# zsc/ARTalk

Hardware: AMD Instinct MI355X
Metric: motion frames/sec (25 fps clips) at batch=32 per GPU (higher is better)
Workload: dtype f32 (operands split into 2 fp16, 3 fp16 MFMA products per fp32 product, fp32 accumulate)

## Files before the change

### artalk_amd/capi.py

```python
from __future__ import annotations

import ctypes as C
import os

from .config import ARTalkConfig

_HERE = os.path.dirname(os.path.abspath(__file__))
LIB_PATH = os.environ.get("ARTALK_LIB") or os.path.join(_HERE, "libartalk_hip.so")

OK, EINVAL, EKEY, EMISSING, EHIP, ESTATE, ECAPACITY, EBUSY = 0, -1, -2, -3, -4, -5, -6, -7
DTYPE_F32, DTYPE_I64 = 0, 1

SYMBOLS = [
    "artalk_create", "artalk_destroy", "artalk_last_error", "artalk_set_tensor", "artalk_finalize_weights",
    "artalk_reserve", "artalk_workspace_bytes", "artalk_weight_bytes", "artalk_infer", "artalk_get_status", "artalk_poll_status", "artalk_last_ticket", "artalk_get_status_of", "artalk_style_encode", "artalk_stream_begin", "artalk_stream_chunk", "artalk_stream_end", "artalk_savgol", "artalk_flame_create", "artalk_flame_verts", "artalk_flame_destroy", "artalk_flame_last_error",
    "artalk_set_profiling", "artalk_get_profile", "artalk_get_kernel_sums", "artalk_set_graphs", "artalk_graph_count", "artalk_set_cu_mask", "artalk_set_audit", "artalk_get_audit", "artalk_calibrate", "artalk_reset_scales", "artalk_get_scales", "artalk_scale_sites", "artalk_get_site_scales", "artalk_set_site_scales", "artalk_set_tap", "artalk_tap_layout", "artalk_set_precision",
    "artalk_op_gemm", "artalk_op_gemm_ex", "artalk_op_gemm_bf16", "artalk_op_gemm_f16s", "artalk_op_pack_split", "artalk_op_gemm_f16s_packed", "artalk_op_release_scratch", "artalk_op_gemm_p8_plan", "artalk_op_create_masked_stream", "artalk_op_destroy_stream", "artalk_op_mfma_f32_peak", "artalk_op_layernorm", "artalk_op_attention", "artalk_op_w2v_front", "artalk_op_resample_mean", "artalk_op_pool_silu",
    "artalk_op_bsq_history",
    "artalk_sessions_reserve", "artalk_session_open", "artalk_session_step", "artalk_session_close", "artalk_session_count",
    "artalk_session_smooth", "artalk_op_savgol_stream", "artalk_op_session_smooth_check",
    "artalk_op_pack_split_ex", "artalk_op_layernorm_ex", "artalk_op_gemm_f16s_packed_ex", "artalk_op_gemm_f16s_ex", "artalk_op_attention_ex", "artalk_op_w2v_front_ex", "artalk_op_pool_silu_ex", "artalk_op_posconv_p8_ex",
    "artalk_op_bsq_history_ex", "artalk_op_ar_bits_next", "artalk_op_vq_embed", "artalk_op_ar_begin", "artalk_op_dec_input", "artalk_op_dec_finish", "artalk_op_enc_input_zero", "artalk_op_style_input", "artalk_op_add_row", "artalk_op_style_finish", "artalk_op_broadcast16", "artalk_op_session_gather", "artalk_op_session_scatter", "artalk_op_absmax",
    "artalk_op_gemm_rows", "artalk_op_layernorm_rows", "artalk_op_attention_rows", "artalk_op_gemm_rows_layout", "artalk_op_rows_dry_run",
    "artalk_op_w2v_front_rows", "artalk_op_pool_silu_rows", "artalk_op_posconv_rows",
    "artalk_op_attention_plan", "artalk_op_attention_rows_cus",
    "artalk_infer_samples", "artalk_set_tail_skip", "artalk_conv_tail_geometry", "artalk_conv_tail_class",
    "artalk_render_create", "artalk_render_mesh", "artalk_render_set_slab", "artalk_render_destroy", "artalk_render_last_error",
    "artalk_splat_create", "artalk_splat_render", "artalk_splat_set_timing", "artalk_splat_get_timing", "artalk_splat_destroy",
    "artalk_splat_last_error",
]

(ATTN_F32_64, ATTN_F32_32, ATTN_SHORT, ATTN_F16, ATTN_F16_P8, ATTN_F16_WIDE, ATTN_F16_PP, ATTN_F16_WIDE_AR,
 ATTN_F16_WIDE_AR_P8) = range(9)
ATTN_KERNELS = {
    ATTN_F32_64: "attention_kernel<64>", ATTN_F32_32: "attention_kernel<32>", ATTN_SHORT: "attention_short_kernel",
    ATTN_F16: "attention_f16_kernel<1>", ATTN_F16_P8: "attention_f16_kernel<1,1>", ATTN_F16_WIDE: "attention_f16_wide_kernel",
    ATTN_F16_PP: "attention_f16_pp_kernel", ATTN_F16_WIDE_AR: "attention_f16_wide_ar_kernel<1>",
    ATTN_F16_WIDE_AR_P8: "attention_f16_wide_ar_kernel<1,1,7,128>",
}


class ArtalkConfigStruct(C.Structure):
    _fields_ = [
        ("ar_depth", C.c_int32), ("ar_heads", C.c_int32),
        ("vae_depth", C.c_int32), ("vae_heads", C.c_int32), ("vae_hidden", C.c_int32),
        ("code_dim", C.c_int32), ("motion_dim", C.c_int32),
        ("n_levels", C.c_int32), ("patch_nums", C.c_int32 * 8),
        ("w2v_layers", C.c_int32), ("w2v_hidden", C.c_int32), ("w2v_heads", C.c_int32), ("w2v_ffn", C.c_int32),
        ("w2v_n_conv", C.c_int32), ("w2v_conv_kernel", C.c_int32 * 8), ("w2v_conv_stride", C.c_int32 * 8),
        ("w2v_conv_dim", C.c_int32),
        ("w2v_pos_kernel", C.c_int32), ("w2v_pos_groups", C.c_int32),
        ("w2v_ln_eps", C.c_float),
        ("style_dim", C.c_int32), ("style_heads", C.c_int32), ("style_layers", C.c_int32), ("style_ffn", C.c_int32),
        ("style_len", C.c_int32),
    ]


ROWMAP_IDENTITY = (2 ** 31 - 1, 0, 0)


class GemmRowsArgs(C.Structure):
    _fields_ = [
        ("mode", C.c_int32), ("M", C.c_int32), ("N", C.c_int32), ("K", C.c_int32), ("act", C.c_int32),
        ("A", C.c_void_p), ("lda", C.c_int64), ("a_elems", C.c_int64), ("a_exp", C.c_int32),
        ("W", C.c_void_p), ("ldw", C.c_int64), ("w_elems", C.c_int64),
        ("bias", C.c_void_p), ("bias_elems", C.c_int64),
        ("C", C.c_void_p), ("ldc", C.c_int64), ("c_elems", C.c_int64), ("cmap", C.c_int32 * 3),
        ("gate", C.c_void_p), ("ldg", C.c_int64), ("gate_elems", C.c_int64), ("gmap", C.c_int32 * 3),
        ("R", C.c_void_p), ("ldr", C.c_int64), ("r_elems", C.c_int64),
        ("c_p8", C.c_int32), ("c_exp", C.c_int32),
        ("force_cfg", C.c_int32), ("splitk", C.c_int32),
        ("ngrp", C.c_int32), ("grpW", C.c_int64), ("grpB", C.c_int64), ("grpC", C.c_int64),
        ("status_dev", C.c_void_p),
        ("ln_Y", C.c_void_p), ("ln_ldy", C.c_int64), ("ln_y_elems", C.c_int64),
        ("ln_scale", C.c_void_p), ("ln_shift", C.c_void_p), ("ln_ldm", C.c_int64), ("ln_mod_elems", C.c_int64), ("ln_mmap", C.c_int32 * 3),
        ("ln_eps", C.c_float), ("ln_out_p8", C.c_int32), ("ln_p8_exp", C.c_int32),
        ("used_cfg", C.POINTER(C.c_int32)), ("used_splitk", C.POINTER(C.c_int32)), ("fused_ln", C.POINTER(C.c_int32)),
        ("cus", C.c_int32),
    ]

    def __init__(self, **kw):
        super().__init__()
        self.a_exp = self.c_exp = self.ln_p8_exp = 4
        self.force_cfg, self.splitk, self.ln_eps = -1, 1, 1e-6
        for name in ("cmap", "gmap", "ln_mmap"):
            setattr(self, name, (C.c_int32 * 3)(*ROWMAP_IDENTITY))
        for k, v in kw.items():
            setattr(self, k, (C.c_int32 * 3)(*v) if k in ("cmap", "gmap", "ln_mmap") else v)


def config_struct(cfg: ARTalkConfig) -> ArtalkConfigStruct:
    w = cfg.w2v
    if w.get("feat_extract_norm", "layer") != "layer" or not w.get("do_stable_layer_norm", True) or not w.get("conv_bias", True):
        raise ValueError("only the XLS-R style wav2vec2 (layer-norm conv stack, stable layer norm, conv bias) is supported")
    if len(set(w["conv_dim"])) != 1:
        raise ValueError("conv_dim must be uniform")
    s = ArtalkConfigStruct()
    s.ar_depth, s.ar_heads = cfg.ar_depth, cfg.ar_heads
    s.vae_depth, s.vae_heads, s.vae_hidden = cfg.vae_depth, cfg.vae_heads, cfg.vae_hidden
    s.code_dim, s.motion_dim = cfg.code_dim, cfg.motion_dim
    s.n_levels = len(cfg.patch_nums)
    for i, p in enumerate(cfg.patch_nums):
        s.patch_nums[i] = p
    s.w2v_layers, s.w2v_hidden = w["num_hidden_layers"], w["hidden_size"]
    s.w2v_heads, s.w2v_ffn = w["num_attention_heads"], w["intermediate_size"]
    s.w2v_n_conv = len(w["conv_kernel"])
    for i, (k, st) in enumerate(zip(w["conv_kernel"], w["conv_stride"])):
        s.w2v_conv_kernel[i], s.w2v_conv_stride[i] = k, st
    s.w2v_conv_dim = w["conv_dim"][0]
    s.w2v_pos_kernel, s.w2v_pos_groups = w["num_conv_pos_embeddings"], w["num_conv_pos_embedding_groups"]
    s.w2v_ln_eps = w["layer_norm_eps"]
    s.style_dim, s.style_heads, s.style_layers = cfg.style_dim, cfg.style_heads, cfg.style_layers
    s.style_ffn, s.style_len = cfg.style_ffn, cfg.style_len
    return s


_lib = None


def lib() -> C.CDLL:
    global _lib
    if _lib is not None:
        return _lib
    if not os.path.exists(LIB_PATH):
        raise RuntimeError(
            f"{LIB_PATH} is missing: the HIP extension has not been built "
            "(run `python -c 'import __graft_entry__ as g; g.build()'`). There is no CPU fallback.")
    L = C.CDLL(LIB_PATH)
    vp, i32, i64, f32 = C.c_void_p, C.c_int, C.c_int64, C.c_float
    L.artalk_create.argtypes = [i32, C.POINTER(ArtalkConfigStruct), C.POINTER(vp)]
    L.artalk_create.restype = i32
    L.artalk_destroy.argtypes = [vp]
    L.artalk_destroy.restype = None
    L.artalk_last_error.argtypes = [vp]
    L.artalk_last_error.restype = C.c_char_p
    L.artalk_set_tensor.argtypes = [vp, C.c_char_p, vp, i32, i32, C.POINTER(i64)]
    L.artalk_set_tensor.restype = i32
    L.artalk_finalize_weights.argtypes = [vp]
    L.artalk_finalize_weights.restype = i32
    L.artalk_reserve.argtypes = [vp, i32, i32]
    L.artalk_reserve.restype = i32
    L.artalk_workspace_bytes.argtypes = [vp]
    L.artalk_workspace_bytes.restype = i64
    L.artalk_weight_bytes.argtypes = [vp]
    L.artalk_weight_bytes.restype = i64
    L.artalk_infer.argtypes = [vp, vp, i64, C.POINTER(i64), i32, vp, vp, vp, i64, vp, vp, vp, vp]
    L.artalk_infer.restype = i32
    if hasattr(L, "artalk_infer_samples"):
        L.artalk_infer_samples.argtypes = [vp, vp, i64, C.POINTER(i64), C.POINTER(i64), i32, vp, vp, vp, i64, vp, vp, vp, vp]
        L.artalk_infer_samples.restype = i32
        L.artalk_set_tail_skip.argtypes = [vp, i32]
        L.artalk_set_tail_skip.restype = i32
        pi = C.POINTER(i32)
        L.artalk_conv_tail_geometry.argtypes = [i64, i32, i32, pi, pi, pi, pi, pi, pi]
        L.artalk_conv_tail_geometry.restype = i32
        L.artalk_conv_tail_class.argtypes = [i64, i32]
        L.artalk_conv_tail_class.restype = i64
    L.artalk_get_status.argtypes = [vp, C.POINTER(C.c_int), vp]
    L.artalk_get_status.restype = i32
    L.artalk_poll_status.argtypes = [vp, C.POINTER(C.c_int)]
    L.artalk_poll_status.restype = i32
    L.artalk_last_ticket.argtypes = [vp]
    L.artalk_last_ticket.restype = C.c_longlong
    L.artalk_get_status_of.argtypes = [vp, C.c_longlong, C.POINTER(C.c_int)]
    L.artalk_get_status_of.restype = i32
    L.artalk_style_encode.argtypes = [vp, vp, i32, vp, vp]
    L.artalk_style_encode.restype = i32
    L.artalk_stream_begin.argtypes = [vp, i32, vp, vp, vp]
    L.artalk_stream_begin.restype = i32
    L.artalk_stream_end.argtypes = [vp]
    L.artalk_stream_end.restype = i32
    L.artalk_stream_chunk.argtypes = [vp, vp, i64, vp, i64, vp]
    L.artalk_stream_chunk.restype = i32
    if hasattr(L, "artalk_session_open"):
        L.artalk_sessions_reserve.argtypes = [vp, i32]
        L.artalk_sessions_reserve.restype = i32
        L.artalk_session_open.argtypes = [vp, i32, vp, vp, C.POINTER(i64), vp]
        L.artalk_session_open.restype = i32
        L.artalk_session_step.argtypes = [vp, C.POINTER(i64), i32, vp, i64, vp, i64, vp, vp, vp]
        L.artalk_session_step.restype = i32
        L.artalk_session_close.argtypes = [vp, C.POINTER(i64), i32]
        L.artalk_session_close.restype = i32
        L.artalk_session_count.argtypes = [vp]
        L.artalk_session_count.restype = i32
    if hasattr(L, "artalk_session_smooth"):
        pi32, pu8 = C.POINTER(i32), C.POINTER(C.c_uint8)
        L.artalk_session_smooth.argtypes = [vp, C.POINTER(i64), i32, vp, i64, pi32, pu8, vp, i64, pi32, pi32, vp]
        L.artalk_session_smooth.restype = i32
        L.artalk_op_savgol_stream.argtypes = [vp, vp, i64, pi32, pi32, pu8, vp, i64, i32, vp]
        L.artalk_op_savgol_stream.restype = i32
        L.artalk_op_session_smooth_check.argtypes = [C.POINTER(i64), C.POINTER(i64), pu8, i32, C.POINTER(i64), i32, C.POINTER(i64), i32, i32, i64,
                                                     pi32, pu8, i64, pi32, pi32, C.c_char_p, i32]
        L.artalk_op_session_smooth_check.restype = i32
    L.artalk_flame_create.argtypes = [i32, i32, i32, i32, vp, vp, vp, vp, vp, vp, f32, C.POINTER(vp)]
    L.artalk_flame_create.restype = i32
    L.artalk_flame_verts.argtypes = [vp, vp, vp, i32, vp, vp]
    L.artalk_flame_verts.restype = i32
    L.artalk_flame_destroy.argtypes = [vp]
    L.artalk_flame_destroy.restype = None
    L.artalk_flame_last_error.argtypes = [vp]
    L.artalk_flame_last_error.restype = C.c_char_p
    if hasattr(L, "artalk_render_create"):
        L.artalk_render_create.argtypes = [i32, i32, i32, vp, i32, f32, C.POINTER(vp)]
        L.artalk_render_create.restype = i32
        L.artalk_render_mesh.argtypes = [vp, vp, i32, vp, f32, vp, vp, vp, vp]
        L.artalk_render_mesh.restype = i32
        L.artalk_render_set_slab.argtypes = [vp, i32]
        L.artalk_render_set_slab.restype = i32
        L.artalk_render_destroy.argtypes = [vp]
        L.artalk_render_destroy.restype = None
        L.artalk_render_last_error.argtypes = [vp]
        L.artalk_render_last_error.restype = C.c_char_p
    if hasattr(L, "artalk_splat_create"):
        L.artalk_splat_create.argtypes = [i32, C.POINTER(vp)]
        L.artalk_splat_create.restype = i32
        L.artalk_splat_render.argtypes = [vp, i32, i32, i32, i32, vp, i64, vp, i64, vp, i64, vp, i64, vp, i64, vp, vp, i32, f32, f32, f32,
                                          vp, vp, vp, vp]
        L.artalk_splat_render.restype = i32
        L.artalk_splat_set_timing.argtypes = [vp, i32]
        L.artalk_splat_set_timing.restype = i32
        L.artalk_splat_get_timing.argtypes = [vp, C.POINTER(C.c_double), i32, C.POINTER(C.c_longlong), C.POINTER(i32)]
        L.artalk_splat_get_timing.restype = i32
        L.artalk_splat_destroy.argtypes = [vp]
        L.artalk_splat_destroy.restype = None
        L.artalk_splat_last_error.argtypes = [vp]
        L.artalk_splat_last_error.restype = C.c_char_p
    L.artalk_savgol.argtypes = [vp, vp, vp, i32, vp]
    L.artalk_savgol.restype = i32
    L.artalk_set_profiling.argtypes = [vp, i32]
    L.artalk_set_profiling.restype = i32
    L.artalk_get_profile.argtypes = [vp, C.POINTER(C.c_double), i32]
    L.artalk_get_profile.restype = i32
    if hasattr(L, "artalk_get_kernel_sums"):
        L.artalk_get_kernel_sums.argtypes = [vp, C.POINTER(C.c_double), i32]
        L.artalk_get_kernel_sums.restype = i32
    L.artalk_set_graphs.argtypes = [vp, i32]
    L.artalk_set_graphs.restype = i32
    if hasattr(L, "artalk_graph_count"):
        L.artalk_graph_count.argtypes = [vp, C.POINTER(C.c_longlong)]
        L.artalk_graph_count.restype = i32
    if hasattr(L, "artalk_set_audit"):
        L.artalk_set_audit.argtypes = [vp, i32]
        L.artalk_set_audit.restype = i32
        L.artalk_get_audit.argtypes = [vp, C.c_char_p, i32, C.POINTER(C.c_float), i32]
        L.artalk_get_audit.restype = i32
    if hasattr(L, "artalk_calibrate"):
        L.artalk_calibrate.argtypes = [vp, f32]
        L.artalk_calibrate.restype = i32
        L.artalk_reset_scales.argtypes = [vp]
        L.artalk_reset_scales.restype = i32
        L.artalk_get_scales.argtypes = [vp, C.POINTER(C.c_int), i32]
        L.artalk_get_scales.restype = i32
    if hasattr(L, "artalk_set_site_scales"):
        L.artalk_scale_sites.argtypes = [vp, C.c_char_p, i32]
        L.artalk_scale_sites.restype = i32
        L.artalk_get_site_scales.argtypes = [vp, C.POINTER(C.c_int), i32]
        L.artalk_get_site_scales.restype = i32
        L.artalk_set_site_scales.argtypes = [vp, C.POINTER(C.c_int), i32]
        L.artalk_set_site_scales.restype = i32
    L.artalk_op_gemm.argtypes = [vp, i64, vp, vp, vp, vp, vp, i32, i32, i32, i32, vp]
    L.artalk_op_gemm.restype = i32
    L.artalk_set_precision.argtypes = [vp, i32]
    L.artalk_set_precision.restype = i32
    if hasattr(L, "artalk_op_gemm_bf16"):
        L.artalk_op_gemm_bf16.argtypes = [vp, i64, vp, vp, vp, vp, vp, i32, i32, i32, i32, i32, vp]
        L.artalk_op_gemm_bf16.restype = i32
    L.artalk_op_gemm_f16s.argtypes = [vp, i64, vp, vp, vp, i32, i32, i32, i32, i32, vp]
    L.artalk_op_gemm_f16s.restype = i32
    L.artalk_op_pack_split.argtypes = [vp, vp, i64, i32, vp]
    L.artalk_op_pack_split.restype = i32
    L.artalk_op_gemm_f16s_packed.argtypes = [vp, i32, i64, vp, vp, vp, i32, i32, i32, i32, i32, vp]
    L.artalk_op_gemm_f16s_packed.restype = i32
    if hasattr(L, "artalk_set_tap"):
        L.artalk_set_tap.argtypes = [vp, vp, i32, i32]
        L.artalk_set_tap.restype = i32
        L.artalk_tap_layout.argtypes = [C.POINTER(C.c_int64), i32]
        L.artalk_tap_layout.restype = i32
        L.artalk_op_release_scratch.argtypes = []
        L.artalk_op_release_scratch.restype = i32
    L.artalk_set_cu_mask.argtypes = [vp, vp, i32]
    L.artalk_set_cu_mask.restype = i32
    L.artalk_op_create_masked_stream.argtypes = [vp, i32, C.POINTER(vp)]
    L.artalk_op_create_masked_stream.restype = i32
    L.artalk_op_destroy_stream.argtypes = [vp]
    L.artalk_op_destroy_stream.restype = i32
    L.artalk_op_gemm_p8_plan.argtypes = [i32, i32, i32, i32]
    L.artalk_op_gemm_p8_plan.restype = i32
    L.artalk_op_gemm_ex.argtypes = [vp, i64, vp, vp, vp, i32, i32, i32, i32, i32, vp]
    L.artalk_op_gemm_ex.restype = i32
    L.artalk_op_mfma_f32_peak.argtypes = [vp, i32, i32, i32, C.POINTER(C.c_double), vp]
    L.artalk_op_mfma_f32_peak.restype = i32
    L.artalk_op_layernorm.argtypes = [vp, vp, vp, vp, vp, vp, i32, i32, f32, i32, vp]
    L.artalk_op_layernorm.restype = i32
    L.artalk_op_attention.argtypes = [vp, vp, vp, vp, i32, i32, i32, i32, i32, f32, i32, vp, i32, vp]
    L.artalk_op_attention.restype = i32
    L.artalk_op_w2v_front.argtypes = [vp, i32, i32, vp, vp, vp, vp, vp, vp, vp]
    L.artalk_op_w2v_front.restype = i32
    L.artalk_op_resample_mean.argtypes = [vp, i32, i32, vp, i32, i32, i32, vp, i32, vp]
    L.artalk_op_resample_mean.restype = i32
    L.artalk_op_pool_silu.argtypes = [vp, i32, i32, i32, vp, vp]
    L.artalk_op_pool_silu.restype = i32
    L.artalk_op_bsq_history.argtypes = [vp, vp, vp, vp, i32, vp]
    L.artalk_op_bsq_history.restype = i32
    if hasattr(L, "artalk_op_pack_split_ex"):
        L.artalk_op_pack_split_ex.argtypes = [vp, vp, i64, i32, i32, vp, vp]
        L.artalk_op_pack_split_ex.restype = i32
        L.artalk_op_layernorm_ex.argtypes = [vp, vp, vp, vp, vp, vp, i32, i32, f32, i32, i32, i32, i32, vp, vp]
        L.artalk_op_layernorm_ex.restype = i32
        L.artalk_op_gemm_f16s_packed_ex.argtypes = [vp, i32, i64, vp, vp, vp, i32, i32, i32, i32, i32, i32, i32, vp, vp, vp]
        L.artalk_op_gemm_f16s_packed_ex.restype = i32
# ... 85 lines not shown
```

### artalk_amd/csrc/ar_glue.hip

```cpp
#include "common.h"
#include <cmath>
#include <mutex>
#include <set>

namespace artalk {

constexpr int T100 = 100;
constexpr int CD = 32;
constexpr int NLV = 5;
__constant__ int c_pn[NLV];
__constant__ int c_off[NLV + 1];
__constant__ int c_up_i0[4][T100];
__constant__ int c_up_i1[4][T100];
__constant__ float c_up_w1[4][T100];
__constant__ float c_hq;

static const int h_pn[NLV] = {1, 5, 25, 50, 100};

int init_ms_tables() {
    static std::mutex mu;
    static std::set<int> ready;
    int dev = -1;
    if (hipGetDevice(&dev) != hipSuccess) return -1;
    std::lock_guard<std::mutex> lock(mu);
// ... 79 lines not shown
}
void launch_ar_begin(const float* style_cond, const float* lvlpos, float* x0, float* fhat, int B, hipStream_t s) {
    ARTALK_LAUNCH(ar_begin_kernel, dim3(B), dim3(256), 0, s, style_cond, lvlpos, x0, fhat, 768);
}

constexpr int BITS_NT = 1024;
__global__ __launch_bounds__(BITS_NT) void ar_bits_kernel(const float* __restrict__ logits, uint8_t* __restrict__ bits,
                                                      float* __restrict__ fhat, float* __restrict__ nextfeat, int p, int* __restrict__ status) {
    __shared__ float hs[T100 * CD];
    __shared__ float fs[T100 * CD];
    const int b = blockIdx.x, tid = threadIdx.x;
    const int pn = c_pn[p], off = c_off[p];
    for (int idx = tid; idx < pn * CD; idx += BITS_NT) {
        const int i = idx / CD, c = idx % CD;
        const float* l = logits + ((long)b * pn + i) * (2 * CD) + 2 * c;
        const int bit = l[1] > l[0];
        if (status && !(isfinite(l[0]) && isfinite(l[1]))) atomicOr(status, 1);
        bits[((long)b * 181 + off + i) * CD + c] = (uint8_t)bit;
        hs[idx] = bit ? c_hq : -c_hq;
    }
    if (p >= NLV - 1) return;
    __syncthreads();
    float* fg = fhat + (long)b * T100 * CD;
    for (int idx = tid; idx < T100 * CD; idx += BITS_NT) {
        const int t = idx / CD, c = idx % CD;
        const float v = fg[idx] + up_lin(hs, p, t, c);
        fg[idx] = v;
        fs[idx] = v;
    }
    __syncthreads();
    const int pn2 = c_pn[p + 1];
    for (int idx = tid; idx < pn2 * CD; idx += BITS_NT)
        nextfeat[(long)b * pn2 * CD + idx] = area_pool(fs, pn2, idx / CD, idx % CD);
}
void launch_ar_bits_next(const float* logits, uint8_t* bits, float* fhat, float* nextfeat, int B, int level, hipStream_t s, int* status) {
    ARTALK_LAUNCH(ar_bits_kernel, dim3(B), dim3(BITS_NT), 0, s, logits, bits, fhat, nextfeat, level, status);
}

constexpr int VQ_TOK = 16;
__global__ __launch_bounds__(256) void vq_embed_kernel(const float* __restrict__ feat, int n, const float* __restrict__ We,
                                                       const float* __restrict__ be, const float* __restrict__ pos,
                                                       float* __restrict__ X, int xrows, int xoff,
                                                       const float* __restrict__ style_cond, const float* __restrict__ pos0, int E) {
    __shared__ float f[VQ_TOK][CD];
    const int i0 = blockIdx.x * VQ_TOK, b = blockIdx.y, tid = threadIdx.x;
    if (blockIdx.x == 0 && style_cond) {
        for (int e = tid; e < E; e += 256) X[((long)b * xrows) * E + e] = style_cond[(long)b * E + e] + pos0[e];
    }
    const int nt = min(VQ_TOK, n - i0);
    for (int idx = tid; idx < VQ_TOK * CD; idx += 256) f[idx / CD][idx % CD] = idx < nt * CD ? feat[((long)b * n + i0) * CD + idx] : 0.f;
    constexpr int EPT = 3;
    float w[EPT][CD], bias[EPT], pv[EPT][VQ_TOK];
#pragma unroll
    for (int k = 0; k < EPT; ++k) {
        const int e = tid + k * 256;
        const bool ok = e < E;
#pragma unroll
        for (int c4 = 0; c4 < CD / 4; ++c4) {
            f32x4 t = {0.f, 0.f, 0.f, 0.f};
            if (ok) t = *reinterpret_cast<const f32x4*>(We + (long)e * CD + 4 * c4);
            w[k][4 * c4] = t[0]; w[k][4 * c4 + 1] = t[1]; w[k][4 * c4 + 2] = t[2]; w[k][4 * c4 + 3] = t[3];
        }
        bias[k] = ok ? be[e] : 0.f;
#pragma unroll
        for (int t = 0; t < VQ_TOK; ++t) pv[k][t] = (ok && t < nt) ? pos[(long)(i0 + t) * E + e] : 0.f;
    }
    __syncthreads();
#pragma unroll
    for (int k = 0; k < EPT; ++k) {
        const int e = tid + k * 256;
        if (e >= E) break;
#pragma unroll
        for (int t0 = 0; t0 < VQ_TOK; t0 += 4) {
            float acc[4] = {0.f, 0.f, 0.f, 0.f};
#pragma unroll
            for (int c = 0; c < CD; ++c)
#pragma unroll
                for (int u = 0; u < 4; ++u) acc[u] = fmaf(w[k][c], f[t0 + u][c], acc[u]);
#pragma unroll
            for (int u = 0; u < 4; ++u)
                if (t0 + u < nt) X[((long)b * xrows + xoff + i0 + t0 + u) * E + e] = (acc[u] + bias[k]) + pv[k][t0 + u];
        }
    }
}
void launch_vq_embed(const float* feat, int n, const float* We, const float* be, const float* pos, float* X, int xrows,
                     int xoff, const float* style_cond, const float* pos0, int B, hipStream_t s) {
    ARTALK_LAUNCH(vq_embed_kernel, dim3((n + VQ_TOK - 1) / VQ_TOK, B), dim3(256), 0, s, feat, n, We, be, pos, X, xrows, xoff,
                       style_cond, pos0, 768);
}

__global__ __launch_bounds__(256) void dec_input_kernel(const float* __restrict__ prev_fdec, const float* __restrict__ fhat,
                                                        const uint8_t* __restrict__ bits, const float* __restrict__ dpos,
                                                        float* __restrict__ X) {
    const int b = blockIdx.x;
    for (int idx = blockIdx.y * 256 + threadIdx.x; idx < 2 * T100 * CD; idx += gridDim.y * 256) {
        const int t = idx / CD, c = idx % CD;
        float v;
        if (t < T100) {
            v = prev_fdec[(long)b * T100 * CD + idx];
        } else {
            const int tt = t - T100;
            const float h = bits[((long)b * 181 + 81 + tt) * CD + c] ? c_hq : -c_hq;
            v = fhat[(long)b * T100 * CD + tt * CD + c] + h;
        }
        X[(long)b * 2 * T100 * CD + idx] = v + dpos[idx];
    }
}
void launch_dec_input(const float* prev_fdec, const float* fhat, const uint8_t* bits, const float* dpos, float* X, int B,
                      hipStream_t s) {
    ARTALK_LAUNCH(dec_input_kernel, dim3(B, 8), dim3(256), 0, s, prev_fdec, fhat, bits, dpos, X);
}

__global__ __launch_bounds__(256) void dec_finish_kernel(const float* __restrict__ dec, const float* __restrict__ mean,
                                                         const float* __restrict__ stdv, const float* __restrict__ epos,
                                                         float* __restrict__ out, long out_bstride, int chunk,
                                                         float* __restrict__ E, int MD, int EK, int* __restrict__ status) {
    const int b = blockIdx.x;
    for (int idx = blockIdx.y * 256 + threadIdx.x; idx < T100 * EK; idx += gridDim.y * 256) {
        const int t = idx / EK, j = idx % EK;
        float e = 0.f;
        if (j < MD) {
            const float d = dec[((long)b * 2 * T100 + T100 + t) * MD + j];
            const float m = d * stdv[j] + mean[j];
            if (status && !isfinite(m)) atomicOr(status, 4);
            out[(long)b * out_bstride + ((long)chunk * T100 + t) * MD + j] = m;
            e = (m - mean[j]) / stdv[j] + epos[t * MD + j];
        }
        E[((long)b * T100 + t) * EK + j] = e;
    }
}
void launch_dec_finish(const float* dec, const float* mean, const float* stdv, const float* epos, float* out,
                       long out_bstride, int chunk, float* E, int B, hipStream_t s, int* status) {
    ARTALK_LAUNCH(dec_finish_kernel, dim3(B, 10), dim3(256), 0, s, dec, mean, stdv, epos, out, out_bstride, chunk, E, 106, 128, status);
}

__global__ __launch_bounds__(256) void enc_input_zero_kernel(const float* __restrict__ mean, const float* __restrict__ stdv,
                                                             const float* __restrict__ epos, float* __restrict__ E, int MD, int EK) {
    const int b = blockIdx.x;
    for (int idx = threadIdx.x; idx < T100 * EK; idx += 256) {
        const int t = idx / EK, j = idx % EK;
        E[((long)b * T100 + t) * EK + j] = (j < MD) ? ((0.f - mean[j]) / stdv[j] + epos[t * MD + j]) : 0.f;
    }
}
__global__ __launch_bounds__(256) void broadcast16_kernel(const uint4* __restrict__ src, uint4* __restrict__ dst, int n16) {
    uint4* d = dst + (long)blockIdx.y * n16;
    for (int i = blockIdx.x * 256 + threadIdx.x; i < n16; i += gridDim.x * 256) d[i] = src[i];
}
void launch_broadcast16(const void* src, void* dst, long bytes, int B, hipStream_t s) {
    if (B <= 0 || bytes <= 0) return;
    const int n16 = (int)(bytes / 16);
    ARTALK_LAUNCH(broadcast16_kernel, dim3((n16 + 255) / 256 < 8 ? (n16 + 255) / 256 : 8, B), dim3(256), 0, s,
                       reinterpret_cast<const uint4*>(src), reinterpret_cast<uint4*>(dst), n16);
}

void launch_enc_input_zero(const float* mean, const float* stdv, const float* epos, float* E, int B, hipStream_t s) {
    ARTALK_LAUNCH(enc_input_zero_kernel, dim3(B), dim3(256), 0, s, mean, stdv, epos, E, 106, 128);
}

__global__ __launch_bounds__(256) void session_gather_kernel(const uint4* const* __restrict__ slots, SessionRows w) {
    const uint4* __restrict__ src = slots[blockIdx.y];
    const long row = blockIdx.y;
    const int p0 = w.s16, f0 = w.s16 + w.p16, n16 = f0 + w.f16;
    for (int i = blockIdx.x * 256 + threadIdx.x; i < n16; i += gridDim.x * 256) {
        const uint4 v = src[i];
        if (i < p0) w.style[row * w.s16 + i] = v;
        else if (i < f0) w.prev_in[row * w.p16 + (i - p0)] = v;
        else w.prev_fdec[row * w.f16 + (i - f0)] = v;
    }
}
__global__ __launch_bounds__(256) void session_scatter_kernel(uint4* const* __restrict__ slots, SessionRows w, int with_style) {
    uint4* __restrict__ dst = slots[blockIdx.y];
    const long row = blockIdx.y;
    const int p0 = w.s16, f0 = w.s16 + w.p16, n16 = f0 + w.f16;
    for (int i = (with_style ? 0 : p0) + blockIdx.x * 256 + threadIdx.x; i < n16; i += gridDim.x * 256) {
        uint4 v;
        if (i < p0) v = w.style[row * w.s16 + i];
        else if (i < f0) v = w.prev_in[row * w.p16 + (i - p0)];
        else v = w.prev_fdec[row * w.f16 + (i - f0)];
        dst[i] = v;
    }
}
static inline unsigned session_pieces(const SessionRows& w) { return (unsigned)((w.s16 + w.p16 + w.f16 + 1023) / 1024); }
void launch_session_gather(const float* const* slots, const SessionRows& w, int n, hipStream_t s) {
    if (n <= 0) return;
    ARTALK_LAUNCH(session_gather_kernel, dim3(session_pieces(w), n), dim3(256), 0, s, reinterpret_cast<const uint4* const*>(slots), w);
}
void launch_session_scatter(float* const* slots, const SessionRows& w, int n, bool with_style, hipStream_t s) {
    if (n <= 0) return;
    ARTALK_LAUNCH(session_scatter_kernel, dim3(session_pieces(w), n), dim3(256), 0, s, reinterpret_cast<uint4* const*>(slots), w,
                  with_style ? 1 : 0);
}

constexpr int BSQ_NT = 1024;
__global__ __launch_bounds__(BSQ_NT) void bsq_history_kernel(const float* __restrict__ enc_out, uint8_t* __restrict__ hist_bits,
                                                          float* __restrict__ prev_fdec, float* __restrict__ msfeat, int* __restrict__ status) {
    __shared__ float resid[T100 * CD];
    __shared__ float fms[T100 * CD];
    __shared__ float qs[T100 * CD];
    __shared__ float hs[T100 * CD];
    const int b = blockIdx.x, tid = threadIdx.x;
    for (int idx = tid; idx < T100 * CD; idx += BSQ_NT) {
        resid[idx] = enc_out[(long)b * T100 * CD + idx];
        if (status && !isfinite(resid[idx])) atomicOr(status, 2);
        fms[idx] = 0.f;
    }
    __syncthreads();
    int msoff = 0;
    for (int p = 0; p < NLV; ++p) {
        const int pn = c_pn[p], off = c_off[p];
        for (int base = 0; base < pn * CD; base += BSQ_NT) {
            const int idx = base + tid;
            const bool ok = idx < pn * CD;
            const int i = ok ? idx / CD : 0, c = idx % CD;
            float x = 0.f;
            if (ok) x = (pn == T100) ? resid[idx] : area_pool(resid, pn, i, c);
            float ss = x * x;
            ss = group_sum<32>(ss);
            const float z = x / fmaxf(sqrtf(ss), 1e-12f);
            const float zhat = (z > 0.f) ? c_hq : -c_hq;
            const float q = z + (zhat - z);
            const int bit = q > 0.f;
            if (ok) {
                qs[idx] = q;
                hs[idx] = bit ? c_hq : -c_hq;
                hist_bits[((long)b * 181 + off + i) * CD + c] = (uint8_t)bit;
            }
        }
        __syncthreads();
        if (p < NLV - 1) {
            for (int idx = tid; idx < T100 * CD; idx += BSQ_NT) {
                const int t = idx / CD, c = idx % CD;
                resid[idx] -= up_lin(qs, p, t, c);
                fms[idx] += up_lin(hs, p, t, c);
            }
            __syncthreads();
            const int pn2 = c_pn[p + 1];
            for (int idx = tid; idx < pn2 * CD; idx += BSQ_NT)
                msfeat[((long)b * 180 + msoff) * CD + idx] = area_pool(fms, pn2, idx / CD, idx % CD);
            msoff += pn2;
        } else {
            for (int idx = tid; idx < T100 * CD; idx += BSQ_NT) prev_fdec[(long)b * T100 * CD + idx] = fms[idx] + hs[idx];
        }
        __syncthreads();
    }
}
void launch_bsq_history(const float* enc_out, uint8_t* hist_bits, float* prev_fdec, float* msfeat, int B, hipStream_t s, int* status) {
    ARTALK_LAUNCH(bsq_history_kernel, dim3(B), dim3(BSQ_NT), 0, s, enc_out, hist_bits, prev_fdec, msfeat, status);
}

__global__ __launch_bounds__(256) void style_input_kernel(const float* __restrict__ motion, const float* __restrict__ mean,
                                                          const float* __restrict__ stdv, float* __restrict__ X, int rows, int MD, int EK) {
    const long n = (long)rows * EK;
    for (long idx = (long)blockIdx.x * 256 + threadIdx.x; idx < n; idx += (long)gridDim.x * 256) {
        const long row = idx / EK; const int j = idx % EK;
        X[idx] = (j < MD) ? (motion[row * MD + j] - mean[j]) / stdv[j] : 0.f;
    }
}
void launch_style_input(const float* motion, const float* mean, const float* stdv, float* X, int B, hipStream_t s) {
    const int rows = B * 50;
    ARTALK_LAUNCH(style_input_kernel, dim3((rows * 128 + 255) / 256), dim3(256), 0, s, motion, mean, stdv, X, rows, 106, 128);
}

__global__ __launch_bounds__(256) void add_row_kernel(float* __restrict__ X, const float* __restrict__ v, long n, int D) {
    for (long idx = (long)blockIdx.x * 256 + threadIdx.x; idx < n; idx += (long)gridDim.x * 256) X[idx] += v[idx % D];
}
void launch_add_row(float* X, const float* v, int M, int D, hipStream_t s) {
    const long n = (long)M * D;
    ARTALK_LAUNCH(add_row_kernel, dim3((unsigned)((n + 255) / 256)), dim3(256), 0, s, X, v, n, D);
}

__global__ __launch_bounds__(256) void style_finish_kernel(const float* __restrict__ feat, const float* __restrict__ Ws,
                                                           const float* __restrict__ bs, const float* __restrict__ null_cond,
                                                           const uint8_t* __restrict__ has_style, float* __restrict__ style_cond,
                                                           int L, int S, int E, const float* __restrict__ cached, long cached_stride) {
    __shared__ float m[128];
    const int b = blockIdx.x, tid = threadIdx.x;
    const int has = has_style ? has_style[b] : 0;
    if (has != 1 && has != 2) {
        for (int e = tid; e < E; e += 256) style_cond[(long)b * E + e] = null_cond[e];
        return;
    }
    if (has == 2) {
        for (int e = tid; e < E; e += 256) style_cond[(long)b * E + e] = cached[(long)b * cached_stride + e];
        return;
    }
    if (tid < S) {
        float s = 0.f;
        for (int t = 0; t < L; ++t) s += feat[((long)b * L + t) * S + tid];
        m[tid] = s / (float)L;
    }
    __syncthreads();
    for (int e = tid; e < E; e += 256) {
        const float* w = Ws + (long)e * S;
        float acc = 0.f;
        for (int c = 0; c < S; ++c) acc = fmaf(w[c], m[c], acc);
        style_cond[(long)b * E + e] = (acc + bs[e]) * 1.1f - null_cond[e] * 0.1f;
    }
}
void launch_style_finish(const float* feat, const float* Ws, const float* bs, const float* null_cond,
                         const uint8_t* has_style, float* style_cond, int B, hipStream_t s, const float* cached, long cached_stride) {
    ARTALK_LAUNCH(style_finish_kernel, dim3(B), dim3(256), 0, s, feat, Ws, bs, null_cond, has_style, style_cond, 50, 128, 768,
                       cached, cached_stride);
}

struct SavgolCoef {
    double fir5[5], edge5[2][5];
// ... 104 lines not shown
```

### artalk_amd/csrc/calls.hip

```cpp
#include "model.h"

#include <algorithm>
#include <climits>
#include <cstring>
#include <set>
#include <string>
#include <vector>

using namespace artalk;

namespace {
int call_stream(artalk_model* m, void* stream, hipStream_t* s) {
    (void)hipSetDevice(m->device);
    if (!stream && !m->own_stream) HIPCHK(m, hipStreamCreate(&m->own_stream));
    *s = stream ? (hipStream_t)stream : m->own_stream;
    return ARTALK_OK;
}
int check_has_style(artalk_model* m, const float* style_motion_dev, const uint8_t* has_style, int B, bool* encode) {
    *encode = false;
    for (int b = 0; style_motion_dev && has_style && b < B; ++b) {
        if (has_style[b] > 2) return fail(m, ARTALK_EINVAL, "has_style entries must be 0, 1 or 2");
        *encode |= has_style[b] == 1;
    }
    return ARTALK_OK;
// ... 37 lines not shown
            *err = std::string(fn) + ": " + std::to_string(ids[i]) + " is not an open session";
            return ARTALK_EINVAL;
        }
        if (!listed.insert(ids[i]).second) { *err = std::string(fn) + ": session " + std::to_string(ids[i]) + " is listed twice"; return ARTALK_EINVAL; }
        (*st)[i] = &it->second;
    }
    return ARTALK_OK;
}

}

namespace artalk {
void smooth_span(int64_t seen, int nf, bool last, int* first, int* count) {
    const int64_t f = seen > kSavgolLag ? seen - kSavgolLag : 0;
    *first = (int)f;
    *count = (int)((last ? seen + nf : seen + nf - kSavgolLag) - f);
}
int smooth_row_range(const std::string& who, int nf, bool last, std::string* err) {
    if (nf < 0 || nf > 100) { *err = who + ": n_frames " + std::to_string(nf) + " is outside 0..100"; return ARTALK_EINVAL; }
    if (nf < 100 && !last) { *err = who + ": fewer than 100 frames (" + std::to_string(nf) + ") without `last`"; return ARTALK_EINVAL; }
    return ARTALK_OK;
}
int smooth_row_length(const std::string& who, int64_t seen, int nf, bool last, std::string* err) {
    if (seen < 0 || seen > INT_MAX - 2 * kSavgolMaxOut) { *err = who + ": frame count out of range"; return ARTALK_EINVAL; }
    if (last && seen + nf < kSavgolCarry) { *err = who + ": savgol (mode='interp') needs window_length <= T (T >= 9)"; return ARTALK_EINVAL; }
    return ARTALK_OK;
}
int smooth_stride_check(const char* fn, bool have_raw, bool need_raw, int64_t raw_stride, int64_t out_stride, int D, std::string* err) {
    if (need_raw && !have_raw) { *err = std::string(fn) + ": no raw frames given"; return ARTALK_EINVAL; }
    if (need_raw && raw_stride < 100LL * D) { *err = std::string(fn) + ": raw_stride is below 100 x " + std::to_string(D); return ARTALK_EINVAL; }
    if (out_stride < (int64_t)kSavgolMaxOut * D) { *err = std::string(fn) + ": out_stride is below 104 x " + std::to_string(D); return ARTALK_EINVAL; }
    return ARTALK_OK;
}
int smooth_check(artalk_model::Sessions& ss, const int64_t* ids, int n, bool have_raw, int64_t raw_stride, const int* n_frames,
                 const uint8_t* last, int64_t out_stride, int D, std::vector<artalk_model::Sessions::Open*>* st, std::string* err) {
    if (int rc = resolve_sessions(ss, "artalk_session_smooth", ids, n, st, err)) return rc;
    bool need_raw = false;
    for (int i = 0; i < n; ++i) {
        const int nf = n_frames ? n_frames[i] : 100;
        const bool lst = last && last[i];
        const std::string who = "artalk_session_smooth: session " + std::to_string(ids[i]);
        if (int rc = smooth_row_range(who, nf, lst, err)) return rc;
        if ((*st)[i]->smooth_done) { *err = who + " has been smoothed to its end (a `last` call was made)"; return ARTALK_ESTATE; }
        if (int rc = smooth_row_length(who, (*st)[i]->seen, nf, lst, err)) return rc;
        need_raw |= nf > 0;
    }
    return smooth_stride_check("artalk_session_smooth", have_raw, need_raw, raw_stride, out_stride, D, err);
}
}

namespace {
int stage_session_slots(artalk_model* m, hipStream_t s, artalk_model::Stage* stg, const int* slot, int n) {
    for (int i = 0; i < n; ++i) stg->slots[i] = m->sess_slot(slot[i]);
    HIPCHK(m, hipMemcpyAsync(m->ws.sess_slots, stg->slots, (size_t)n * sizeof(float*), hipMemcpyHostToDevice, s));
    return ARTALK_OK;
}

}

extern "C" {

int artalk_infer(artalk_model* m, const float* audio_dev, int64_t audio_clip_stride, const int64_t* n_chunks, int B,
                 const float* style_motion_dev, const uint8_t* has_style, float* out_motion_dev, int64_t out_clip_stride,
                 uint8_t* out_bits_dev, uint8_t* out_hist_bits_dev, float* out_w2v_dev, void* stream) {
    return artalk_infer_samples(m, audio_dev, audio_clip_stride, n_chunks, nullptr, B, style_motion_dev, has_style, out_motion_dev, out_clip_stride,
                                out_bits_dev, out_hist_bits_dev, out_w2v_dev, stream);
}

int artalk_infer_samples(artalk_model* m, const float* audio_dev, int64_t audio_clip_stride, const int64_t* n_chunks, const int64_t* n_samples,
                         int B, const float* style_motion_dev, const uint8_t* has_style, float* out_motion_dev, int64_t out_clip_stride,
                         uint8_t* out_bits_dev, uint8_t* out_hist_bits_dev, float* out_w2v_dev, void* stream) {
    if (!m || !audio_dev || !n_chunks || !out_motion_dev || B <= 0) return ARTALK_EINVAL;
    if (!m->finalized) return fail(m, ARTALK_ESTATE, "artalk_infer before artalk_finalize_weights");
    for (int b = 0; n_samples && b < B; ++b)
        if (n_chunks[b] > 0 && (n_samples[b] < 1 || n_samples[b] > n_chunks[b] * kSamplesPerChunk))
            return fail(m, ARTALK_EINVAL, "n_samples[" + std::to_string(b) + "] must be in 1 .. n_chunks * " + std::to_string(kSamplesPerChunk));
    hipStream_t s;
    if (int rc = call_stream(m, stream, &s)) return rc;
    const artalk_config& c = m->cfg;
    int64_t C = 0, maxch = n_chunks[0];
    for (int b = 0; b < B; ++b) {
        if (n_chunks[b] <= 0 || (b > 0 && n_chunks[b] > n_chunks[b - 1])) return fail(m, ARTALK_EINVAL, "n_chunks must be positive and non-increasing");
        C += n_chunks[b];
    }
    bool encode_style;
    if (int rc = check_has_style(m, style_motion_dev, has_style, B, &encode_style)) return rc;
    if (m->tap && (B > m->tap_B || maxch > m->tap_maxch)) return fail(m, ARTALK_EINVAL, "the tap buffer (artalk_set_tap) is smaller than this call");
    if (B > m->ws.maxB || C > m->ws.maxC) { if (int rc = reserve(m, B, (int)C)) return rc; }
    Workspace& w = m->ws;
    artalk_model::Stage* stg = nullptr;
    if (int rc = next_stage(m, &stg)) return rc;
    long* src = stg->src;
    std::vector<int> base((size_t)maxch + 1, 0), Bj((size_t)maxch, 0);
    {
        int idx = 0;
        for (int64_t j = 0; j < maxch; ++j) {
            base[j] = idx;
            for (int b = 0; b < B && n_chunks[b] > j; ++b) { src[idx++] = (long)b * audio_clip_stride + (long)j * kSamplesPerChunk; Bj[j]++; }
        }
        base[maxch] = idx;
    }
    std::vector<ConvPasses> passes;
    bool any_tail = false;
    if (n_samples && m->tail_skip) {
        std::vector<int> cls((size_t)C, 3);
        for (int64_t j = 0, idx = 0; j < maxch; ++j)
            for (int b = 0; b < B && n_chunks[b] > j; ++b, ++idx) {
                const int64_t v = std::min<int64_t>(n_samples[b] - j * kSamplesPerChunk, kSamplesPerChunk);
                const int64_t bound = v >= 1 ? artalk_conv_tail_class(v, kSamplesPerChunk) : 0;
                const int q = bound >= 1 && kSamplesPerChunk % 4 == 0 ? (int)(bound / (kSamplesPerChunk / 4)) : 4;
                cls[idx] = m->tail_geo[q - 1].partial ? q - 1 : 3;
            }
        const int last = m->n_conv - 1;
        for (int c0 = 0; c0 < C; c0 += w.G) {
            const int n = (int)std::min<int64_t>(w.G, C - c0);
            ConvPasses cp;
            static const int order[4] = {3, 0, 1, 2};
            int pos = 0;
            long row0 = 0;
            for (int k = 0; k < 4; ++k) {
                const int cl = order[k], off = pos;
                const artalk_model::TailGeo& tg = m->tail_geo[cl];
                const long rows = cl == 3 ? m->Ts : tg.S[last], tc = cl == 3 ? m->Tw - 1 : tg.tc;
                for (int i = 0; i < n; ++i)
                    if (cls[c0 + i] == cl) {
                        src[C + c0 + pos] = src[c0 + i];
                        src[2 * C + c0 + i] = (row0 + (pos - off) * rows) | (tc << 32);
                        ++pos;
                    }
                if (pos > off) { cp.off[cp.np] = off; cp.n[cp.np] = pos - off; cp.cls[cp.np] = cl; ++cp.np; row0 += (pos - off) * rows; }
            }
            if (cp.np == 1 && cp.cls[0] == 3) cp.np = 0;
            else { cp.perm = w.src_off + C + c0; cp.tab = w.src_off + 2 * C + c0; any_tail = true; }
            passes.push_back(cp);
        }
    }
    HIPCHK(m, hipMemcpyAsync(w.src_off, src, (any_tail ? 3 : 1) * C * sizeof(long), hipMemcpyHostToDevice, s));
    m->stream_B = 0; m->stream_scales_ended = false;
    m->ev_used = 0; m->dom_events.clear(); m->marks.clear(); m->prof_stream = s;
    struct TimerScope { bool on; TimerScope(artalk_model* x) : on(x->profiling == 3) { if (on) { x->ktimer.used = 0; x->ktimer.recs.clear(); x->ktimer.bucket = KB_OTHER; g_ktimer = &x->ktimer; } }
                        ~TimerScope() { if (on) g_ktimer = nullptr; } } timer_scope(m);
    if (int rc = begin_clips(m, s, B, style_motion_dev, has_style, encode_style, stg)) return rc;
    for (int c0 = 0, gi = 0; c0 < C; c0 += w.G, ++gi)
        run_wav2vec(m, audio_dev, c0, (int)std::min<int64_t>(w.G, C - c0), out_w2v_dev, s, !passes.empty() && passes[gi].np ? &passes[gi] : nullptr);
    if (int rc = run_init_history(m, B, s)) return rc;
    const size_t bits_row = (size_t)kNTok * c.code_dim;
    if (out_hist_bits_dev)
        HIPCHK(m, hipMemcpy2DAsync(out_hist_bits_dev, (size_t)(maxch + 1) * bits_row, w.hist_bits, bits_row, bits_row, B,
                                   hipMemcpyDeviceToDevice, s));
    stage_mark(m, s, PB_VAE);
    for (int64_t j = 0; j < maxch; ++j) {
        const int Bn = Bj[j];
        const int n_next = out_hist_bits_dev ? Bn : (j + 1 < maxch ? Bj[j + 1] : 0);
        if (int rc = chunk_step(m, s, base[j], Bn, n_next, (int)j, out_motion_dev + j * 100 * c.motion_dim, out_clip_stride)) return rc;
        if (out_bits_dev)
            HIPCHK(m, hipMemcpy2DAsync(out_bits_dev + j * bits_row, (size_t)maxch * bits_row, w.bits, bits_row, bits_row, Bn,
                                       hipMemcpyDeviceToDevice, s));
        if (out_hist_bits_dev)
            HIPCHK(m, hipMemcpy2DAsync(out_hist_bits_dev + (j + 1) * bits_row, (size_t)(maxch + 1) * bits_row, w.hist_bits, bits_row,
                                       bits_row, Bn, hipMemcpyDeviceToDevice, s));
    }
    stage_mark(m, s, PB_OTHER);
    if (int rc = publish_status(m, s)) return rc;
    if (m->sticky_error) { m->sticky_error = false; return ARTALK_ESTATE; }
    return ARTALK_OK;
}

int artalk_style_encode(artalk_model* m, const float* style_motion_dev, int n, float* out_cond_dev, void* stream) {
    if (!m || !style_motion_dev || !out_cond_dev || n <= 0) return ARTALK_EINVAL;
    if (!m->finalized) return fail(m, ARTALK_ESTATE, "artalk_style_encode before artalk_finalize_weights");
    hipStream_t s;
    if (int rc = call_stream(m, stream, &s)) return rc;
    if (m->stream_B > 0) return fail(m, ARTALK_ESTATE, "artalk_style_encode during a streaming session (it shares the workspace)");
    if (n > m->ws.maxB) { if (int rc = reserve(m, n, std::max(n, m->ws.maxC))) return rc; }
    Workspace& w = m->ws;
    HIPCHK(m, hipMemsetAsync(w.has_style, 1, n, s));
    {
        ProfilingOff quiet(m);
        run_style(m, style_motion_dev, n, s, true);
    }
    HIPCHK(m, hipMemcpyAsync(out_cond_dev, w.style_cond, (size_t)n * kE * sizeof(float), hipMemcpyDeviceToDevice, s));
    HIPCHK(m, hipGetLastError());
    return ARTALK_OK;
}

int artalk_stream_begin(artalk_model* m, int B, const float* style_motion_dev, const uint8_t* has_style, void* stream) {
    if (!m || B <= 0) return ARTALK_EINVAL;
    if (!m->finalized) return fail(m, ARTALK_ESTATE, "artalk_stream_begin before artalk_finalize_weights");
    bool encode_style;
    if (int rc = check_has_style(m, style_motion_dev, has_style, B, &encode_style)) return rc;
    hipStream_t s;
    if (int rc = call_stream(m, stream, &s)) return rc;
    if (B > m->ws.maxB || B > m->ws.maxC) { if (int rc = reserve(m, B, B)) return rc; }
    if (int rc = ensure_stage(m, m->ws.maxB, m->ws.maxC)) return rc;
    artalk_model::Stage* stg = nullptr;
    if (int rc = next_stage(m, &stg)) return rc;
    {
        ProfilingOff quiet(m);
        if (int rc = begin_clips(m, s, B, style_motion_dev, has_style, encode_style, stg)) return rc;
        if (int rc = run_init_history(m, B, s)) return rc;
    }
    m->stream_B = B; m->stream_scales_ended = false;
    if (int rc = publish_status(m, s)) return rc;
    return ARTALK_OK;
}

int artalk_stream_chunk(artalk_model* m, const float* audio_dev, int64_t chunk_stride, float* out_motion_dev, int64_t out_stride,
                        void* stream) {
    if (!m || !audio_dev || !out_motion_dev) return ARTALK_EINVAL;
    if (m->stream_B <= 0)
        return fail(m, ARTALK_ESTATE, m->stream_scales_ended ? "the site scales changed since artalk_stream_begin; begin again"
                                                             : "artalk_stream_chunk before artalk_stream_begin");
    hipStream_t s;
    if (int rc = call_stream(m, stream, &s)) return rc;
    const int B = m->stream_B;
    Workspace& w = m->ws;
    if (B > w.maxB) return fail(m, ARTALK_ESTATE, "workspace was re-reserved since artalk_stream_begin; begin again");
    artalk_model::Stage* stg = nullptr;
    if (int rc = next_stage(m, &stg)) return rc;
    for (int b = 0; b < B; ++b) stg->src[b] = (long)b * chunk_stride;
    HIPCHK(m, hipMemcpyAsync(w.src_off, stg->src, B * sizeof(long), hipMemcpyHostToDevice, s));
    HIPCHK(m, hipEventRecord(stg->done, s));
    stg->used = true;
    ProfilingOff quiet(m);
    for (int c0 = 0; c0 < B; c0 += w.G) run_wav2vec(m, audio_dev, c0, std::min(w.G, B - c0), nullptr, s);
    if (int rc = chunk_step(m, s, 0, B, B, m->tap_maxch, out_motion_dev, out_stride)) return rc;
    if (int rc = publish_status(m, s)) return rc;
    return ARTALK_OK;
}

int artalk_stream_end(artalk_model* m) {
    if (!m) return ARTALK_EINVAL;
    m->stream_B = 0; m->stream_scales_ended = false;
    return ARTALK_OK;
}

int artalk_sessions_reserve(artalk_model* m, int max_sessions) {
    if (!m || max_sessions <= 0) return ARTALK_EINVAL;
    (void)hipSetDevice(m->device);
    return grow_sessions(m, max_sessions);
}

int artalk_session_count(const artalk_model* m) { return m ? (int)m->sess.open.size() : ARTALK_EINVAL; }

int artalk_session_open(artalk_model* m, int n, const float* style_motion_dev, const uint8_t* has_style, int64_t* ids_out, void* stream) {
    if (!m || n <= 0 || !ids_out) return ARTALK_EINVAL;
    if (!m->finalized) return fail(m, ARTALK_ESTATE, "artalk_session_open before artalk_finalize_weights");
    bool encode_style;
    if (int rc = check_has_style(m, style_motion_dev, has_style, n, &encode_style)) return rc;
    hipStream_t s;
    if (int rc = call_stream(m, stream, &s)) return rc;
    artalk_model::Sessions& ss = m->sess;
    if (int rc = grow_sessions(m, (int64_t)ss.open.size() + n)) return rc;
    if (n > m->ws.maxB || n > m->ws.maxC) { if (int rc = reserve(m, n, n)) return rc; }
    if (int rc = ensure_stage(m, m->ws.maxB, m->ws.maxC)) return rc;
    std::vector<int> slot;
    for (int i = 0; i < (int)ss.owner.size() && (int)slot.size() < n; ++i)
        if (!ss.owner[i]) slot.push_back(i);
    artalk_model::Stage* stg = nullptr;
    if (int rc = next_stage(m, &stg)) return rc;
    if (int rc = stage_session_slots(m, s, stg, slot.data(), n)) return rc;
    m->stream_B = 0; m->stream_scales_ended = false;
    {
        ProfilingOff quiet(m);
        if (int rc = begin_clips(m, s, n, style_motion_dev, has_style, encode_style, stg)) return rc;
        if (int rc = run_init_history(m, n, s)) return rc;
    }
    launch_session_scatter(m->ws.sess_slots, session_rows(m), n, true, s);
    if (int rc = publish_status(m, s)) return rc;
    for (int i = 0; i < n; ++i) {
        ids_out[i] = ss.next_id++;
        ss.owner[slot[i]] = ids_out[i];
        ss.open.emplace(ids_out[i], artalk_model::Sessions::Open{slot[i]});
    }
    return ARTALK_OK;
}

int artalk_session_step(artalk_model* m, const int64_t* ids, int n, const float* audio_dev, int64_t chunk_stride, float* out_motion_dev,
                        int64_t out_stride, uint8_t* out_bits_dev, uint8_t* out_hist_bits_dev, void* stream) {
    if (!m || !ids || n <= 0 || !audio_dev || !out_motion_dev) return ARTALK_EINVAL;
    artalk_model::Sessions& ss = m->sess;
    std::vector<artalk_model::Sessions::Open*> st;
    std::string err;
    if (int rc = resolve_sessions(ss, "artalk_session_step", ids, n, &st, &err)) return fail(m, rc, err);
    std::vector<int> slot((size_t)n);
    for (int i = 0; i < n; ++i) slot[i] = st[i]->slot;
    hipStream_t s;
    if (int rc = call_stream(m, stream, &s)) return rc;
    if (n > m->ws.maxB || n > m->ws.maxC) { if (int rc = reserve(m, n, n)) return rc; }
    Workspace& w = m->ws;
    artalk_model::Stage* stg = nullptr;
    if (int rc = next_stage(m, &stg)) return rc;
    for (int b = 0; b < n; ++b) stg->src[b] = (long)b * chunk_stride;
    HIPCHK(m, hipMemcpyAsync(w.src_off, stg->src, n * sizeof(long), hipMemcpyHostToDevice, s));
    if (int rc = stage_session_slots(m, s, stg, slot.data(), n)) return rc;
    HIPCHK(m, hipEventRecord(stg->done, s));
    stg->used = true;
    m->stream_B = 0; m->stream_scales_ended = false;
    HIPCHK(m, hipMemsetAsync(w.status, 0, 4 * sizeof(int), s));
    const SessionRows rows = session_rows(m);
    ProfilingOff quiet(m);
    launch_session_gather(w.sess_slots, rows, n, s);
    for (int c0 = 0; c0 < n; c0 += w.G) run_wav2vec(m, audio_dev, c0, std::min(w.G, n - c0), nullptr, s);
    if (int rc = chunk_step(m, s, 0, n, n, m->tap_maxch, out_motion_dev, out_stride)) return rc;
    launch_session_scatter(w.sess_slots, rows, n, false, s);
    const size_t bits_n = (size_t)n * kNTok * m->cfg.code_dim;
    if (out_bits_dev) HIPCHK(m, hipMemcpyAsync(out_bits_dev, w.bits, bits_n, hipMemcpyDeviceToDevice, s));
    if (out_hist_bits_dev) HIPCHK(m, hipMemcpyAsync(out_hist_bits_dev, w.hist_bits, bits_n, hipMemcpyDeviceToDevice, s));
    if (int rc = publish_status(m, s)) return rc;
    return ARTALK_OK;
}

int artalk_session_close(artalk_model* m, const int64_t* ids, int n) {
    if (!m || !ids || n <= 0) return ARTALK_EINVAL;
    artalk_model::Sessions& ss = m->sess;
    std::set<int64_t> seen;
    for (int i = 0; i < n; ++i)
        if ((!ss.open.count(ids[i]) && !ss.ended_by_scales.count(ids[i])) || !seen.insert(ids[i]).second)
            return fail(m, ARTALK_EINVAL, "artalk_session_close: " + std::to_string(ids[i]) + " is not an open session (or is listed twice)");
    for (int i = 0; i < n; ++i) {
        const auto it = ss.open.find(ids[i]);
        if (it != ss.open.end()) { ss.owner[it->second.slot] = 0; ss.open.erase(it); }
        ss.ended_by_scales.erase(ids[i]);
    }
    return ARTALK_OK;
}

int artalk_session_smooth(artalk_model* m, const int64_t* ids, int n, const float* raw_dev, int64_t raw_stride, const int* n_frames,
                          const uint8_t* last, float* out_dev, int64_t out_stride, int* first_out, int* count_out, void* stream) {
    if (!m || !ids || n <= 0 || !out_dev || !first_out || !count_out) return ARTALK_EINVAL;
    artalk_model::Sessions& ss = m->sess;
    std::vector<artalk_model::Sessions::Open*> st;
    std::string err;
    if (int rc = smooth_check(ss, ids, n, raw_dev != nullptr, raw_stride, n_frames, last, out_stride, m->cfg.motion_dim, &st, &err)) return fail(m, rc, err);
    hipStream_t s;
    if (int rc = call_stream(m, stream, &s)) return rc;
    if (n > m->stage_cap_b) { if (int rc = ensure_stage(m, n, m->stage_cap_c)) return rc; }
    artalk_model::Stage* stg = nullptr;
    if (int rc = next_stage(m, &stg)) return rc;
    for (int i = 0; i < n; ++i) {
        stg->slots[i] = m->sess_slot(st[i]->slot);
        stg->smooth[i] = make_int4((int)st[i]->seen, n_frames ? n_frames[i] : 100, last && last[i] ? 1 : 0, 0);
    }
    float** slots_dev = static_cast<float**>(ss.smooth_tab);
    int4* meta_dev = reinterpret_cast<int4*>(slots_dev + ss.smooth_cap);
    HIPCHK(m, hipMemcpyAsync(slots_dev, stg->slots, (size_t)n * sizeof(float*), hipMemcpyHostToDevice, s));
    HIPCHK(m, hipMemcpyAsync(meta_dev, stg->smooth, (size_t)n * sizeof(int4), hipMemcpyHostToDevice, s));
    HIPCHK(m, hipEventRecord(stg->done, s));
    stg->used = true;
    launch_savgol_stream(slots_dev, meta_dev, (long)m->sess_carry_off(), raw_dev, (long)raw_stride, out_dev, (long)out_stride, n,
                         m->cfg.motion_dim, s);
    HIPCHK(m, hipGetLastError());
    for (int i = 0; i < n; ++i) {
        const int nf = n_frames ? n_frames[i] : 100;
        const bool lst = last && last[i];
        smooth_span(st[i]->seen, nf, lst, &first_out[i], &count_out[i]);
        st[i]->seen += nf;
        st[i]->smooth_done = lst;
    }
    return ARTALK_OK;
}

int artalk_savgol(artalk_model* m, const float* in_dev, float* out_dev, int T, void* stream) {
    if (!m || !in_dev || !out_dev) return ARTALK_EINVAL;
    if (T < 9) return fail(m, ARTALK_EINVAL, "savgol (mode='interp') needs window_length <= T (T >= 9)");
    (void)hipSetDevice(m->device);
    launch_savgol(in_dev, out_dev, T, m->cfg.motion_dim, (hipStream_t)stream);
    return ARTALK_OK;
}

}
```

### artalk_amd/csrc/engine.hip

```cpp
#include "model.h"

#include <hip/hip_ext.h>

#include <algorithm>
#include <cmath>
#include <cstring>
#include <string>
#include <vector>

using namespace artalk;

namespace artalk {
thread_local KernelTimer* g_ktimer = nullptr;
bool ktimer_events(hipEvent_t* e0, hipEvent_t* e1) {
    KernelTimer* t = g_ktimer;
    if (!t) return false;
    while (t->pool.size() < t->used + 2) {
        hipEvent_t e = nullptr;
        if (hipEventCreate(&e) != hipSuccess) return false;
        t->pool.push_back(e);
    }
    *e0 = t->pool[t->used]; *e1 = t->pool[t->used + 1];
    t->recs.emplace_back(t->bucket, t->used);
    t->used += 2;
    return true;
}
}

namespace {
hipEvent_t next_event(artalk_model* m, hipStream_t s, size_t* idx) {
    if (m->ev_used == m->ev_pool.size()) {
        hipEvent_t e;
        (void)hipEventCreate(&e);
        m->ev_pool.push_back(e);
    }
    *idx = m->ev_used++;
    (void)hipEventRecord(m->ev_pool[*idx], s);
    return m->ev_pool[*idx];
}
void kbucket(artalk_model* m, int b) { m->ktimer.bucket = b; }
}

namespace artalk {
void stage_mark(artalk_model* m, hipStream_t s, int bucket) {
    if (!m->profiling || m->in_graph_body) return;
    size_t i;
    next_event(m, s, &i);
    m->marks.emplace_back(bucket, i);
}
}

namespace {
void audit(artalk_model* m, const float* buf, int rows, int cols, long ld, bool is_p8, hipStream_t s, int* ex, int junk_period = 0,
           int junk_from = 0) {
    if (!m->audit || !m->audit_vals) return;
    auto st = m->site_of.find(ex);
    if (st == m->site_of.end()) { m->err = "internal: audited exponent is not in the site table"; m->sticky_error = true; return; }
    const std::string& name = m->sites[st->second].name;
    auto it = m->audit_index.find(name);
    int idx;
    if (it == m->audit_index.end()) {
        if ((int)m->audit_names.size() >= kAuditSlots) return;
        idx = (int)m->audit_names.size();
        m->audit_names.push_back(name);
        m->audit_exp.push_back(ex);
        m->audit_index.emplace(name, idx);
    } else idx = it->second;
    launch_absmax(buf, rows, cols & ~7, ld, is_p8 ? 1 : 0, m->audit_vals + idx, s, junk_period, junk_from, ex ? *ex : kActExp);
}

bool gemm(artalk_model* m, const GemmArgs& g0, hipStream_t s, const LnArgs* fuse_ln = nullptr, int plan_M = 0) {
    GemmArgs g = g0;
    const int run_M = g.M;
    if (plan_M > 0) g.M = plan_M;
    g.graph_tag = m->in_body ? 1 : 0;
    g.cus = m->n_cus;
    g.status = m->precision == 1 ? (m->view ? m->view->status : m->ws.status) : nullptr;
    if (m->precision == 1 && !g.exact) g.Wp = packed_of(m, g.W);
    if (m->precision == 2 && !g.exact) {
        g.Wb = bf16_of(m, g.W);
        if (!g.Wb || ((unsigned long long)g.Wb & 15) || (g.ldw & 7)) {
            m->err = "internal: bf16 GEMM without an aligned bf16 weight copy"; m->sticky_error = true; return false;
        }
        if (g.a_packed) { m->err = "internal: P8 activation handed to a bf16 GEMM"; m->sticky_error = true; return false; }
    }
    const Workspace& cw = m->view ? *m->view : m->ws;
    const GemmPolicy pol{m->precision, false, cw.splitk, cw.splitk_floats, m->splitk_tiles, m->splitk_target};
    GemmPlan plan = plan_gemm(g, pol, fuse_ln);
    if (plan_M > 0) {
        g.M = run_M;
        if (plan.path != GEMM_P8) g.force_cfg = plan.cfg;
        else if (gemm_p8_class(plan.cfg) == P8_BIG) {
            GemmArgs h = g;
            h.force_cfg = g0.force_cfg; h.splitk = g0.splitk; h.partial = g0.partial;
            const GemmPlan alt = plan_gemm(h, pol, fuse_ln);
            if (alt.path == GEMM_P8 && gemm_p8_class(alt.cfg) == P8_BIG && h.splitk == g.splitk) { g.force_cfg = alt.cfg; plan.cfg = alt.cfg; }
        }
    }
    if (g.a_packed && plan.path == GEMM_F32) { m->err = "internal: P8 activation handed to an fp32 GEMM"; m->sticky_error = true; return false; }
    const bool timed = m->profiling && plan.dominant && !m->in_body;
    size_t i0 = 0, i1 = 0;
    if (timed) next_event(m, s, &i0);
    run_gemm(g, plan, fuse_ln, s);
    if (timed) {
        next_event(m, s, &i1);
        m->dom_events.emplace_back(i0, gemm_flops(g));
    }
    return plan.fused_ln;
}

void tap_copy(artalk_model* m, int field, int row0, const float* src, int rows, int cols, int B, hipStream_t s) {
    if (!m->tap || m->in_graph_body || m->tap_chunk >= m->tap_maxch || B > m->tap_B) return;
    float* dst = m->tap + ((long)m->tap_chunk * m->tap_B) * TAP_SLOT + field + (long)row0 * cols;
    (void)hipMemcpy2DAsync(dst, (size_t)TAP_SLOT * 4, src, (size_t)rows * cols * 4, (size_t)rows * cols * 4, B, hipMemcpyDeviceToDevice, s);
}

enum { LF_EXACT = 1, LF_A_P8 = 2, LF_C_P8 = 4 };
void linear(artalk_model* m, const float* A, long lda, const float* W, const float* bias, float* C, long ldc, int M, int N, int K,
            int act, const float* R, hipStream_t s, int flags = 0, float* c2 = nullptr, int a_exp = kActExp, int c_exp = kActExp,
            int plan_M = 0) {
    GemmArgs g;
    g.c2 = c2; g.a_exp = a_exp; g.c_exp = c_exp;
    g.exact = flags & LF_EXACT; g.a_packed = (flags & LF_A_P8) ? 1 : 0; g.c_p8 = (flags & LF_C_P8) ? 1 : 0;
    g.A = A; g.lda = lda; g.W = W; g.ldw = K; g.bias = bias; g.C = C; g.ldc = ldc; g.M = M; g.N = N; g.K = K; g.act = act;
    g.R = R; g.ldr = ldc;
    gemm(m, g, s, nullptr, plan_M);
}

void layernorm(const float* X, float* Y, const float* w, const float* b, int M, int D, float eps, int act, hipStream_t s, int out_p8 = 0,
               int* status = nullptr, int junk_period = 0, int junk_from = 0, int p8_exp = kActExp) {
    LnArgs a;
    a.out_p8 = out_p8; a.p8_exp = p8_exp; a.status = out_p8 ? status : nullptr; a.junk_period = junk_period; a.junk_from = junk_from;
    a.X = X; a.ldx = D; a.Y = Y; a.ldy = D; a.w = w; a.b = b; a.M = M; a.D = D; a.eps = eps; a.act = act;
    launch_layernorm(a, s);
}

}

namespace artalk {

void run_wav2vec(artalk_model* m, const float* audio, int c0, int n, float* out_w2v, hipStream_t s, const ConvPasses* tail) {
    const artalk_config& c = m->cfg;
    Workspace& w = m->ws;
    const int CD = c.w2v_conv_dim, Hs = c.w2v_hidden;
    const int p8 = m->precision == 1 ? 1 : 0;
    const int AP = p8 ? LF_A_P8 : 0;
    Range r_w2v("artalk.wav2vec2");
    roctxRangePushA("artalk.wav2vec2.conv_stack");
    kbucket(m, KB_CONV);
    launch_audio_normalize(audio, tail ? tail->perm : w.src_off + c0, w.xnorm, n, kSamplesPerChunk, s);
    SiteExps& ex = m->ex;
    ConvPasses one;
    one.np = 1; one.n[0] = n; one.cls[0] = 3;
    const ConvPasses& ps = tail ? *tail : one;
    auto geo_T = [&](int p) { const artalk_model::TailGeo& tg = m->tail_geo[ps.cls[p]]; return ps.cls[p] != 3 && tg.partial ? tg.T : m->conv_T; };
    auto geo_S = [&](int p) { const artalk_model::TailGeo& tg = m->tail_geo[ps.cls[p]]; return ps.cls[p] != 3 && tg.partial ? tg.S : m->conv_S; };
    auto row0 = [&](int p, int i) { long r = 0; for (int q = 0; q < p; ++q) r += (long)ps.n[q] * geo_S(q)[i]; return r; };
    float* src = w.convA; float* dst = w.convB;
    for (int p = 0; p < ps.np; ++p) {
        const int *T = geo_T(p), *S = geo_S(p);
        float* y = src + row0(p, 0) * CD;
        launch_conv0(w.xnorm + (long)ps.off[p] * kSamplesPerChunk, kSamplesPerChunk, m->conv0_w, m->conv_b[0], m->conv_lnw[0], m->conv_lnb[0], y, ps.n[p],
                     T[0], S[0], s, p8, w.status, ex.conv[0]);
        audit(m, y, ps.n[p] * S[0], CD, CD, p8, s, &ex.conv[0], S[0], T[0]);
    }
    for (int i = 1; i < c.w2v_n_conv; ++i) {
        const int M = (int)row0(ps.np, i), plan_M = M == n * m->conv_S[i] ? 0 : n * m->conv_S[i];
        linear(m, src, (long)c.w2v_conv_stride[i] * CD, m->conv_w[i], m->conv_b[i], dst, CD, M, CD, c.w2v_conv_kernel[i] * CD,
               ACT_NONE, nullptr, s, AP, nullptr, ex.conv[i - 1], kActExp, plan_M);
        for (int p = 0; p < ps.np; p += 2) {
            const int *T = geo_T(p), *S = geo_S(p);
            float* y = dst + row0(p, i) * CD;
            const int Mp = ps.n[p] * S[i], Mq = p + 1 < ps.np ? ps.n[p + 1] * geo_S(p + 1)[i] : 0;
            LnArgs a;
            a.plan_M = plan_M;
            a.out_p8 = (p8 && i + 1 < c.w2v_n_conv) ? 1 : 0; a.p8_exp = ex.conv[i]; a.status = a.out_p8 ? w.status : nullptr;
            a.junk_period = S[i]; a.junk_from = T[i];
            if (Mq) { a.junk_row2 = Mp; a.junk_period2 = geo_S(p + 1)[i]; a.junk_from2 = geo_T(p + 1)[i]; }
            a.X = y; a.ldx = CD; a.Y = y; a.ldy = CD; a.w = m->conv_lnw[i]; a.b = m->conv_lnb[i]; a.M = Mp + Mq; a.D = CD; a.eps = 1e-5f; a.act = ACT_GELU_ERF;
            launch_layernorm(a, s);
            if (i + 1 < c.w2v_n_conv) {
                audit(m, y, Mp, CD, CD, p8, s, &ex.conv[i], S[i], T[i]);
                if (Mq) audit(m, y + (long)Mp * CD, Mq, CD, CD, p8, s, &ex.conv[i], a.junk_period2, a.junk_from2);
            }
        }
        std::swap(src, dst);
    }
    if (tail) {
        launch_conv_tail_gather(src, tail->tab, dst, n, m->Tw, m->Ts, CD, s);
        std::swap(src, dst);
    }
    stage_mark(m, s, PB_CONV);
    roctxRangePop();
    Range r_enc("artalk.wav2vec2.encoder");
    kbucket(m, KB_ENC);
    const int M = n * m->Ts;
    const int JP = m->Ts, JF = m->Tw;
    layernorm(src, dst, m->fp_lnw, m->fp_lnb, M, CD, c.w2v_ln_eps, ACT_NONE, s, p8, w.status, JP, JF, ex.fp_ln);
    audit(m, dst, M, CD, CD, p8, s, &ex.fp_ln, JP, JF);
    linear(m, dst, CD, m->fp_w, m->fp_b, w.h0, Hs, M, Hs, CD, ACT_NONE, nullptr, s, AP, nullptr, ex.fp_ln);
    audit(m, w.h0, M, Hs, Hs, false, s, &ex.posconv_in, JP, JF);
    {
        const int cg = Hs / c.w2v_pos_groups;
        GemmArgs g;
        g.A = w.h0; g.lda = Hs; g.W = m->pos_w; g.ldw = (long)cg * c.w2v_pos_kernel; g.bias = m->pos_b; g.C = w.h1; g.ldc = Hs; g.R = w.h0; g.ldr = Hs;
        g.M = M; g.act = ACT_GELU_ERF; g.a_exp = ex.posconv_in;
        if (p8 && cg == 64 && c.w2v_pos_kernel == 128 && c.w2v_pos_groups == 16 && m->Ts <= 256) {
            g.N = Hs; g.K = cg * c.w2v_pos_kernel; g.Wp = packed_of(m, m->pos_w); g.status = w.status;
            launch_posconv_p8(g, n, m->Tw, m->Ts, s);
        } else {
            g.amode = 1; g.pc_T = m->Tw; g.pc_tstride = m->Ts; g.pc_pad = c.w2v_pos_kernel / 2; g.pc_cin = cg;
            g.N = cg; g.K = cg * c.w2v_pos_kernel;
            g.batch = c.w2v_pos_groups; g.sA = cg; g.sW = (long)cg * cg * c.w2v_pos_kernel; g.sBias = cg; g.sC = cg; g.sR = cg;
            gemm(m, g, s);
        }
    }
    float* h = w.h1;
    const int nh = c.w2v_heads, hd = Hs / nh;
    for (int i = 0; i < c.w2v_layers; ++i) {
        const W2VLayer& L = m->w2v[i];
        SiteExps::W2V& E = ex.w2v[i];
        layernorm(h, w.xln, L.ln1w, L.ln1b, M, Hs, c.w2v_ln_eps, ACT_NONE, s, p8, w.status, JP, JF, E.ln1);
        audit(m, w.xln, M, Hs, Hs, p8, s, &E.ln1, JP, JF);
        linear(m, w.xln, Hs, L.qkv_w, L.qkv_b, w.qkv, 3 * Hs, M, 3 * Hs, Hs, ACT_NONE, nullptr, s, AP | (p8 ? LF_C_P8 : 0), nullptr, E.ln1, E.qkv);
        AttnArgs a;
        a.qkv_p8 = p8; a.qkv_exp = E.qkv; a.o_exp = E.attn;
        a.Q = w.qkv; a.K = w.qkv + Hs; a.V = w.qkv + 2 * Hs;
        a.ldq = a.ldk = a.ldv = 3 * Hs; a.q_bstride = a.k_bstride = a.v_bstride = (long)m->Ts * 3 * Hs;
        a.O = w.att; a.ldo = Hs; a.o_bstride = (long)m->Ts * Hs;
        a.B = n; a.H = nh; a.HD = hd; a.Lq = m->Tw; a.Lk = m->Tw; a.scale = 1.0f / std::sqrt((float)hd);
        audit(m, w.qkv, M, 3 * Hs, 3 * Hs, p8, s, &E.qkv, JP, JF);
        a.out_p8 = p8; a.split16 = p8; a.status = p8 ? w.status : nullptr; a.cus = m->n_cus;
        launch_attention(a, s);
        audit(m, w.att, M, Hs, Hs, p8, s, &E.attn, JP, JF);
        linear(m, w.att, Hs, L.out_w, L.out_b, h, Hs, M, Hs, Hs, ACT_NONE, h, s, AP, nullptr, E.attn);
        layernorm(h, w.xln, L.ln2w, L.ln2b, M, Hs, c.w2v_ln_eps, ACT_NONE, s, p8, w.status, JP, JF, E.ln2);
        audit(m, w.xln, M, Hs, Hs, p8, s, &E.ln2, JP, JF);
        linear(m, w.xln, Hs, L.ff1_w, L.ff1_b, w.ffn, c.w2v_ffn, M, c.w2v_ffn, Hs, ACT_GELU_ERF, nullptr, s, AP | (p8 ? LF_C_P8 : 0), nullptr, E.ln2, E.ffn);
        audit(m, w.ffn, M, c.w2v_ffn, c.w2v_ffn, p8, s, &E.ffn, JP, JF);
        linear(m, w.ffn, c.w2v_ffn, L.ff2_w, L.ff2_b, h, Hs, M, Hs, c.w2v_ffn, ACT_NONE, h, s, AP, nullptr, E.ffn);
    }
    layernorm(h, w.xln, m->enc_lnw, m->enc_lnb, M, Hs, c.w2v_ln_eps, ACT_NONE, s);
    if (out_w2v)
        (void)hipMemcpy2DAsync(out_w2v + (long)c0 * m->Tw * Hs, (size_t)m->Tw * Hs * 4, w.xln, (size_t)m->Ts * Hs * 4,
                               (size_t)m->Tw * Hs * 4, n, hipMemcpyDeviceToDevice, s);
    launch_pool_silu(w.xln, m->Ts, m->Tw, w.silu_cond + (long)c0 * kNTok * kCond, n, m->pn, c.n_levels, kCond, s, p8, w.status, ex.silu_cond);
    audit(m, w.silu_cond + (long)c0 * kNTok * kCond, n * kNTok, kCond, kCond, p8, s, &ex.silu_cond);
    stage_mark(m, s, PB_ENC);
}

void run_style(artalk_model* m, const float* style_motion, int B, hipStream_t s, bool encode) {
    const artalk_config& c = m->cfg;
    Workspace& w = m->ws;
    const int S = c.style_dim, L = c.style_len, M = B * L;
    Range r_style("artalk.style_encoder");
    kbucket(m, KB_STYLE);
    if (style_motion && encode) {
        launch_style_input(style_motion, m->st_mean, m->st_std, w.s_in, B, s);
        SiteExps& ex = m->ex;
        audit(m, w.s_in, M, 128, 128, false, s, &ex.style_in);
        linear(m, w.s_in, 128, m->st_proj_w, m->st_proj_b, w.s_h, S, M, S, 128, ACT_NONE, nullptr, s, 0, nullptr, ex.style_in);
        launch_add_row(w.s_h, m->st_pe, M, S, s);
        for (int i = 0; i < c.style_layers; ++i) {
            const StyleLayer& Ly = m->style[i];
            SiteExps::ST& E = ex.style[i];
            audit(m, w.s_h, M, S, S, false, s, &E.h);
            linear(m, w.s_h, S, Ly.in_w, Ly.in_b, w.s_qkv, 3 * S, M, 3 * S, S, ACT_NONE, nullptr, s, 0, nullptr, E.h);
            AttnArgs a;
            a.Q = w.s_qkv; a.K = w.s_qkv + S; a.V = w.s_qkv + 2 * S; a.ldq = a.ldk = a.ldv = 3 * S;
            a.q_bstride = a.k_bstride = a.v_bstride = (long)L * 3 * S;
            a.O = w.s_att; a.ldo = S; a.o_bstride = (long)L * S;
            a.B = B; a.H = c.style_heads; a.HD = S / c.style_heads; a.Lq = L; a.Lk = L;
            a.scale = 1.0f / std::sqrt((float)(S / c.style_heads));
            launch_attention(a, s);
            audit(m, w.s_att, M, S, S, false, s, &E.attn);
            linear(m, w.s_att, S, Ly.out_w, Ly.out_b, w.s_tmp, S, M, S, S, ACT_NONE, w.s_h, s, 0, nullptr, E.attn);
            layernorm(w.s_tmp, w.s_h, Ly.n1w, Ly.n1b, M, S, 1e-5f, ACT_NONE, s);
            audit(m, w.s_h, M, S, S, false, s, &E.h1);
            linear(m, w.s_h, S, Ly.l1_w, Ly.l1_b, w.s_ffn, c.style_ffn, M, c.style_ffn, S, ACT_GELU_ERF, nullptr, s, 0, nullptr, E.h1);
            audit(m, w.s_ffn, M, c.style_ffn, c.style_ffn, false, s, &E.ffn);
            linear(m, w.s_ffn, c.style_ffn, Ly.l2_w, Ly.l2_b, w.s_tmp, S, M, S, c.style_ffn, ACT_NONE, w.s_h, s, 0, nullptr, E.ffn);
            layernorm(w.s_tmp, w.s_h, Ly.n2w, Ly.n2b, M, S, 1e-5f, ACT_NONE, s);
        }
    }
    launch_style_finish(w.s_h, m->sc_w, m->sc_b, m->null_style, style_motion ? w.has_style : nullptr, w.style_cond, B, s,
                        style_motion, (long)L * c.motion_dim);
}

}

namespace {
void run_vae_stack(artalk_model* m, const VAESide& S, int B, int T, int split, hipStream_t s) {
    const artalk_config& c = m->cfg;
    Workspace& w = m->view ? *m->view : m->ws;
    const int H = c.vae_hidden, M = B * T, F = H * 3 / 2;
    const int p8 = m->precision == 1 ? 1 : 0;
    const int AP = p8 ? LF_A_P8 : 0;
    const int sd = &S == &m->enc ? 0 : 1;
    for (int i = 0; i < c.vae_depth; ++i) {
        const VAELayer& L = S.layers[i];
        SiteExps::VAE& E = m->ex.vae[sd][i];
        layernorm(w.vh, w.vln, L.lnw, L.lnb, M, H, 1e-5f, ACT_NONE, s, p8, w.status, 0, 0, E.ln);
        audit(m, w.vln, M, H, H, p8, s, &E.ln);
        linear(m, w.vln, H, L.qkv_w, nullptr, w.vqkv, 3 * H, M, 3 * H, H, ACT_NONE, nullptr, s, AP | (p8 ? LF_C_P8 : 0), nullptr, E.ln, E.qkv);
        AttnArgs a;
        a.qkv_p8 = p8; a.qkv_exp = E.qkv; a.o_exp = E.attn;
        a.Q = w.vqkv; a.K = w.vqkv + H; a.V = w.vqkv + 2 * H; a.ldq = a.ldk = a.ldv = 3 * H;
        a.q_bstride = a.k_bstride = a.v_bstride = (long)T * 3 * H;
        a.O = w.vatt; a.ldo = H; a.o_bstride = (long)T * H;
        a.B = B; a.H = c.vae_heads; a.HD = H / c.vae_heads; a.Lq = T; a.Lk = T;
        a.scale = 1.0f / std::sqrt((float)H);
        audit(m, w.vqkv, M, 3 * H, 3 * H, p8, s, &E.qkv);
        a.split_q = split; a.split_k = split; a.out_p8 = p8; a.split16 = p8; a.status = p8 ? w.status : nullptr; a.cus = m->n_cus;
        launch_attention(a, s);
        audit(m, w.vatt, M, H, H, p8, s, &E.attn);
        linear(m, w.vatt, H, L.out_w, L.out_b, w.vh, H, M, H, H, ACT_NONE, w.vh, s, AP, p8 ? w.vln : nullptr, E.attn, E.resid);
        audit(m, p8 ? w.vln : w.vh, M, H, H, p8, s, &E.resid);
        linear(m, p8 ? w.vln : w.vh, H, L.m1_w, L.m1_b, w.vmlp, F, M, F, H, ACT_GELU_TANH, nullptr, s, p8 ? (LF_A_P8 | LF_C_P8) : 0, nullptr, E.resid, E.mlp);
        audit(m, w.vmlp, M, F, F, p8, s, &E.mlp);
        linear(m, w.vmlp, F, L.m2_w, L.m2_b, w.vh, H, M, H, F, ACT_NONE, w.vh, s, AP, nullptr, E.mlp);
    }
}

void run_reencode(artalk_model* m, int B, hipStream_t s) {
    const artalk_config& c = m->cfg;
    Workspace& w = m->view ? *m->view : m->ws;
    const int H = c.vae_hidden, T = 100;
    Range r_re("artalk.vae.reencode_bsq");
    kbucket(m, KB_REENC);
    audit(m, w.enc_in, B * T, 128, 128, false, s, &m->ex.vae_enc_in);
    linear(m, w.enc_in, 128, m->enc.in_w, m->enc.in_b, w.vh, H, B * T, H, 128, ACT_LEAKY02, nullptr, s, 0, nullptr, m->ex.vae_enc_in);
    run_vae_stack(m, m->enc, B, T, 0, s);
    linear(m, w.vh, H, m->enc.out_w, m->enc.out_b, w.enc_out, c.code_dim, B * T, c.code_dim, H, ACT_NONE, nullptr, s, LF_EXACT);
    launch_bsq_history(w.enc_out, w.hist_bits, w.prev_fdec, w.msfeat, B, s, w.status);
    launch_vq_embed(w.msfeat, kNTok - 1, m->vq_w, m->vq_b, m->prev_lvl_pos + kE, w.prev_in, kNTok, 1, w.style_cond,
                    m->prev_lvl_pos, B, s);
}

}

namespace artalk {
int run_init_history(artalk_model* m, int B, hipStream_t s) {
    const artalk_config& c = m->cfg;
    struct Restore { artalk_model* m; ~Restore() { kbucket(m, KB_OTHER); } } restore{m};
    Workspace& w = m->ws;
    artalk_model::InitHistory& ih = m->init_hist[m->precision];
    const long nb = (long)kNTok * c.code_dim, nf = 100L * c.code_dim * 4, nm = 180L * c.code_dim * 4;
    if (!ih.valid) {
        if (!ih.bits) {
            ih.bits = dalloc<uint8_t>(m, nb); ih.fdec = dalloc<float>(m, nf / 4); ih.msfeat = dalloc<float>(m, nm / 4);
            if (!ih.bits || !ih.fdec || !ih.msfeat) return fail(m, ARTALK_EHIP, "hipMalloc failed for the initial-history cache");
            HIPCHK(m, hipDeviceSynchronize());
        }
        launch_enc_input_zero(m->vae_mean, m->vae_std, m->enc_pos, w.enc_in, 1, s);
        run_reencode(m, 1, s);
        HIPCHK(m, hipMemcpyAsync(ih.bits, w.hist_bits, nb, hipMemcpyDeviceToDevice, s));
        HIPCHK(m, hipMemcpyAsync(ih.fdec, w.prev_fdec, nf, hipMemcpyDeviceToDevice, s));
        HIPCHK(m, hipMemcpyAsync(ih.msfeat, w.msfeat, nm, hipMemcpyDeviceToDevice, s));
        int flags[4] = {0, 0, 0, 0};
        HIPCHK(m, hipMemcpyAsync(flags, w.status, sizeof(int), hipMemcpyDeviceToHost, s));
        HIPCHK(m, hipStreamSynchronize(s));
        ih.valid = flags[0] == 0;
    }
    launch_broadcast16(ih.bits, w.hist_bits, nb, B, s);
    launch_broadcast16(ih.fdec, w.prev_fdec, nf, B, s);
    launch_broadcast16(ih.msfeat, w.msfeat, nm, B, s);
    launch_vq_embed(w.msfeat, kNTok - 1, m->vq_w, m->vq_b, m->prev_lvl_pos + kE, w.prev_in, kNTok, 1, w.style_cond, m->prev_lvl_pos, B, s);
    return ARTALK_OK;
}

}

namespace {
void run_chunk_body(artalk_model* m, int B, hipStream_t s, int n_reencode = -1) {
    struct BodyScope { artalk_model* m; BodyScope(artalk_model* x) : m(x) { m->in_body = true; } ~BodyScope() { m->in_body = false; } } scope(m);
    const artalk_config& c = m->cfg;
    Workspace& w = m->view ? *m->view : m->ws;
    const long ldada = m->ada_n;
    const long cache_l = (long)w.maxB * 2 * kNTok * 3 * kE;
    const int p8 = m->precision == 1 ? 1 : 0;
    kbucket(m, KB_AR_MISC);
    tap_copy(m, TAP_PREV_IN, 0, w.prev_in, kNTok, kE, B, s);
    roctxRangePushA("artalk.ar.history_kv");
    SiteExps& ex = m->ex;
    if (p8) launch_pack_split(w.prev_in, reinterpret_cast<unsigned int*>(w.prev_in_p8), (long)B * kNTok * kE, false, s, w.status, ex.hist_tok);
    audit(m, p8 ? w.prev_in_p8 : w.prev_in, B * kNTok, kE, kE, p8, s, &ex.hist_tok);
    {
        GemmArgs g;
        g.A = p8 ? w.prev_in_p8 : w.prev_in; g.a_packed = p8; g.a_exp = ex.hist_tok;
        g.lda = kE; g.W = m->ar_qkv_w + (long)kE * kE; g.ldw = kE; g.bias = m->ar_qkv_b + kE;
        g.C = w.cache + kE; g.ldc = 3 * kE; g.cmap = rowmap(kNTok, 2 * kNTok, 0);
        g.M = B * kNTok; g.N = c.ar_depth * 2 * kE; g.K = kE;
        g.ngrp = 2 * kE; g.grpW = (long)3 * kE * kE; g.grpB = 3 * kE; g.grpC = cache_l;
        g.Wp = packed_of(m, g.W);
        if (p8 && gemm_p8_eligible(g)) {
            gemm(m, g, s);
        } else {
            for (int l = 0; l < c.ar_depth; ++l) {
                const ARLayer& L = m->ar[l];
                GemmArgs q = g;
                q.Wp = nullptr; q.ngrp = 0; q.grpW = q.grpB = q.grpC = 0;
                q.W = L.qkv_w + (long)kE * kE; q.bias = L.qkv_b + kE; q.C = w.cache + l * cache_l + kE; q.N = 2 * kE;
                gemm(m, q, s);
            }
        }
    }
    roctxRangePop();
    launch_ar_begin(w.style_cond, m->lvl_pos, w.x, w.fhat, B, s);
    static const char* const kLevelName[kMaxLv] = {"artalk.ar.scale_step0", "artalk.ar.scale_step1", "artalk.ar.scale_step2",
                                                   "artalk.ar.scale_step3", "artalk.ar.scale_step4"};
    for (int p = 0; p < c.n_levels; ++p) {
        Range r_lv(kLevelName[p]);
        kbucket(m, KB_LEVEL0 + p);
        const int pn = m->pn[p], off = m->off[p], M = B * pn;
        const RowMap amap = rowmap(pn, kNTok, off);
        auto ln_args = [&](int l, int which) {
            LnArgs n;
            n.X = w.x; n.ldx = kE; n.Y = w.xmod; n.ldy = kE; n.ldm = ldada; n.mmap = amap; n.M = M; n.D = kE; n.eps = 1e-6f;
            n.status = p8 ? w.status : nullptr;
            if (l < c.ar_depth) {
                const float* ada = w.ada + (long)l * 6 * kE;
                n.scale = ada + (2 + which) * kE; n.shift = ada + (4 + which) * kE; n.out_p8 = p8;
                n.p8_exp = which == 0 ? ex.ar[l].ln1 : ex.ar[l].ln2;
            } else {
                const float* hada = w.ada + (long)c.ar_depth * 6 * kE;
                n.scale = hada; n.shift = hada + kE; n.out_p8 = 0;
            }
            return n;
        };
        bool have_ln = false;
        for (int l = 0; l < c.ar_depth; ++l) {
            const ARLayer& L = m->ar[l];
            const float* ada = w.ada + (long)l * 6 * kE;
            float* cache = w.cache + l * cache_l;
            SiteExps::AR& E = ex.ar[l];
            if (l == 0) tap_copy(m, TAP_BLK0_IN, off, w.x, pn, kE, B, s);
            if (!have_ln) launch_layernorm(ln_args(l, 0), s);
            audit(m, w.xmod, M, kE, kE, p8, s, &E.ln1);
            GemmArgs q;
            q.A = w.xmod; q.lda = kE; q.W = L.qkv_w; q.ldw = kE; q.bias = L.qkv_b; q.C = cache; q.ldc = 3 * kE;
            q.cmap = rowmap(pn, 2 * kNTok, kNTok + off); q.M = M; q.N = 3 * kE; q.K = kE; q.a_packed = p8; q.a_exp = E.ln1;
            gemm(m, q, s);
            AttnArgs a;
            a.Q = cache + (long)(kNTok + off) * 3 * kE; a.K = cache + kE; a.V = cache + 2 * kE;
            a.ldq = a.ldk = a.ldv = 3 * kE; a.q_bstride = a.k_bstride = a.v_bstride = (long)2 * kNTok * 3 * kE;
            a.O = w.attn_out; a.ldo = kE; a.o_bstride = (long)pn * kE;
            a.B = B; a.H = c.ar_heads; a.HD = kE / c.ar_heads; a.Lq = pn; a.Lk = kNTok + off + pn; a.scale = 1.0f;
            a.l2norm = 1; a.qscale = L.qscale; a.out_p8 = p8; a.split16 = p8; a.status = p8 ? w.status : nullptr; a.o_exp = E.attn;
            launch_attention(a, s);
            audit(m, w.attn_out, M, kE, kE, p8, s, &E.attn);
            GemmArgs pj;
            pj.A = w.attn_out; pj.lda = kE; pj.W = L.proj_w; pj.ldw = kE; pj.bias = L.proj_b; pj.C = w.x; pj.ldc = kE;
            pj.gate = ada; pj.ldg = ldada; pj.gmap = amap; pj.R = w.x; pj.ldr = kE; pj.M = M; pj.N = kE; pj.K = kE; pj.a_packed = p8; pj.a_exp = E.attn;
            const LnArgs n2 = ln_args(l, 1);
            if (!gemm(m, pj, s, &n2)) launch_layernorm(n2, s);
            audit(m, w.xmod, M, kE, kE, p8, s, &E.ln2);
            linear(m, w.xmod, kE, L.ffn1_w, L.ffn1_b, w.ffn_h, 4 * kE, M, 4 * kE, kE, ACT_GELU_TANH, nullptr, s, p8 ? (LF_A_P8 | LF_C_P8) : 0, nullptr, E.ln2, E.ffn);
            audit(m, w.ffn_h, M, 4 * kE, 4 * kE, p8, s, &E.ffn);
            GemmArgs f2;
            f2.A = w.ffn_h; f2.lda = 4 * kE; f2.W = L.ffn2_w; f2.ldw = 4 * kE; f2.bias = L.ffn2_b; f2.C = w.x; f2.ldc = kE;
            f2.gate = ada + kE; f2.ldg = ldada; f2.gmap = amap; f2.R = w.x; f2.ldr = kE; f2.M = M; f2.N = kE; f2.K = 4 * kE; f2.a_packed = p8; f2.a_exp = E.ffn;
            const LnArgs nn = ln_args(l + 1, 0);
            have_ln = gemm(m, f2, s, &nn);
            if (l == 0) tap_copy(m, TAP_BLK0_OUT, off, w.x, pn, kE, B, s);
            if (l == c.ar_depth - 1) tap_copy(m, TAP_BLKL_OUT, off, w.x, pn, kE, B, s);
        }
        if (!have_ln) launch_layernorm(ln_args(c.ar_depth, 0), s);
        linear(m, w.xmod, kE, m->logits_w, m->logits_b, w.logits, 2 * c.code_dim, M, 2 * c.code_dim, kE, ACT_NONE, nullptr, s, LF_EXACT);
        tap_copy(m, TAP_LOGITS, off, w.logits, pn, 2 * c.code_dim, B, s);
        launch_ar_bits_next(w.logits, w.bits, w.fhat, w.nextfeat, B, p, s, w.status);
        if (p + 1 < c.n_levels)
            launch_vq_embed(w.nextfeat, m->pn[p + 1], m->vq_w, m->vq_b, m->lvl_pos + (long)m->off[p + 1] * kE, w.x, m->pn[p + 1], 0,
                            nullptr, nullptr, B, s);
    }
    stage_mark(m, s, PB_AR);
    const int H = c.vae_hidden;
    roctxRangePushA("artalk.vae.decode");
    kbucket(m, KB_VAE_DEC);
    launch_dec_input(w.prev_fdec, w.fhat, w.bits, m->dec_pos, w.dec_x, B, s);
    audit(m, w.dec_x, B * 200, c.code_dim, c.code_dim, false, s, &ex.vae_dec_in);
    linear(m, w.dec_x, c.code_dim, m->dec.in_w, m->dec.in_b, w.vh, H, B * 200, H, c.code_dim, ACT_LEAKY02, nullptr, s, 0, nullptr, ex.vae_dec_in);
    run_vae_stack(m, m->dec, B, 200, 100, s);
    audit(m, w.vh, B * 200, H, H, false, s, &ex.vae_dec_head);
    linear(m, w.vh, H, m->dec.out_w, m->dec.out_b, w.dec_out, c.motion_dim, B * 200, c.motion_dim, H, ACT_NONE, nullptr, s, 0, nullptr, ex.vae_dec_head);
    tap_copy(m, TAP_DEC_OUT, 0, w.dec_out, 200, c.motion_dim, B, s);
    launch_dec_finish(w.dec_out, m->vae_mean, m->vae_std, m->enc_pos, w.motion_chunk, 100L * c.motion_dim, 0, w.enc_in, B, s, w.status);
    roctxRangePop();
    if (n_reencode < 0 || n_reencode > B) n_reencode = B;
    if (n_reencode > 0) run_reencode(m, n_reencode, s);
    stage_mark(m, s, PB_VAE);
}

Workspace clip_view(const artalk_model* m, int b0, int branch) {
    Workspace v = m->ws;
    for (const ClipBuf& cb : clip_buffers(m)) {
        if (cb.f) v.*cb.f += b0 * cb.n; else v.*cb.u8 += b0 * cb.n;
    }
    v.splitk = m->ws.splitk_b[branch];
    return v;
}

int ensure_side_streams(artalk_model* m, int n) {
    if (!m->fork_ev) HIPCHK(m, hipEventCreateWithFlags(&m->fork_ev, hipEventDisableTiming));
    for (int i = 0; i < n && i < 3; ++i) {
        if (m->side_stream[i]) continue;
        if (m->cu_mask.empty()) HIPCHK(m, hipStreamCreateWithFlags(&m->side_stream[i], hipStreamNonBlocking));
        else HIPCHK(m, hipExtStreamCreateWithCUMask(&m->side_stream[i], (uint32_t)m->cu_mask.size(), m->cu_mask.data()));
        HIPCHK(m, hipEventCreateWithFlags(&m->join_ev[i], hipEventDisableTiming));
    }
    return ARTALK_OK;
}
int body_branches(const artalk_model* m, int B) {
    const int want = m->branches > 0 ? m->branches : (B >= 8 ? 2 : 1);
    return B >= 2 * want ? want : (B >= 8 ? 2 : 1);
}
bool body_uses_graphs(const artalk_model* m) { return m->use_graphs && m->profiling < 2 && !m->audit && !m->tap; }
constexpr size_t kMaxGraphs = 96;
int evict_graphs(artalk_model* m, const long long* keep, int n_keep) {
    while (m->graphs.size() >= kMaxGraphs) {
        auto victim = m->graphs.end();
        for (auto it = m->graphs.begin(); it != m->graphs.end(); ++it) {
            bool pinned = false;
            for (int i = 0; i < n_keep; ++i) pinned |= it->first == keep[i];
            if (!pinned && (victim == m->graphs.end() || it->second.last_use < victim->second.last_use)) victim = it;
        }
        if (victim == m->graphs.end()) break;
        HIPCHK(m, hipDeviceSynchronize());
        (void)hipGraphExecDestroy(victim->second.exec);
        m->graphs.erase(victim);
    }
    return ARTALK_OK;
}
struct BodyGroups { bool graphs; int n; int b0[5]; int nre[4]; long long key[4]; };
BodyGroups plan_body(const artalk_model* m, int B, int n_next) {
    BodyGroups g;
    if (n_next < 0 || n_next > B) n_next = B;
    g.graphs = body_uses_graphs(m) && B <= 4095;
    const bool whole = m->audit || m->tap || m->profiling == 2 || (body_uses_graphs(m) && !g.graphs);
    g.n = whole ? 1 : body_branches(m, B);
    for (int h = 0; h <= g.n; ++h) g.b0[h] = (int)((long)B * h / g.n);
    for (int h = 0; h < g.n; ++h) {
        const int gsz = g.b0[h + 1] - g.b0[h];
        const int need = std::max(0, std::min(n_next - g.b0[h], gsz));
        g.nre[h] = g.graphs ? std::min(gsz, (need + 7) / 8 * 8) : need;
        g.key[h] = ((long long)(((B * 8 + g.n) * 4 + h) * 3 + m->precision)) * 4096 + g.nre[h];
    }
    return g;
}
int run_body(artalk_model* m, int B, hipStream_t s, int n_next) {
    const BodyGroups g = plan_body(m, B, n_next);
    const bool fork = g.n > 1 && m->profiling != 3;
    if (fork) { if (int rc = ensure_side_streams(m, g.n - 1)) return rc; }
    hipStream_t st[4] = {s, s, s, s};
    for (int h = 1; fork && h < g.n; ++h) st[h] = m->side_stream[h - 1];
    Workspace views[4];
    for (int h = 0; h < g.n; ++h) views[h] = clip_view(m, g.b0[h], h);
    auto launch_group = [&](int h) { m->view = &views[h]; run_chunk_body(m, g.b0[h + 1] - g.b0[h], st[h], g.nre[h]); m->view = nullptr; };
    for (int h = 0; g.graphs && h < g.n; ++h) {
        auto hit = m->graphs.find(g.key[h]);
        if (hit != m->graphs.end()) { hit->second.last_use = ++m->graph_clock; continue; }
        if (int rc = evict_graphs(m, g.key, g.n)) return rc;
        hipGraph_t graph = nullptr;
        hipGraphExec_t exec = nullptr;
        HIPCHK(m, hipStreamBeginCapture(st[h], hipStreamCaptureModeThreadLocal));
        m->in_graph_body = true;
        launch_group(h);
        m->in_graph_body = false;
        HIPCHK(m, hipStreamEndCapture(st[h], &graph));
        HIPCHK(m, hipGraphInstantiate(&exec, graph, nullptr, nullptr, 0));
        (void)hipGraphDestroy(graph);
        m->graphs.emplace(g.key[h], artalk_model::GraphEntry{exec, ++m->graph_clock});
        ++m->graph_captures;
    }
    if (fork) {
        HIPCHK(m, hipEventRecord(m->fork_ev, s));
        for (int h = 1; h < g.n; ++h) HIPCHK(m, hipStreamWaitEvent(st[h], m->fork_ev, 0));
    }
    for (int h = 0; h < g.n; ++h) {
        if (g.graphs) HIPCHK(m, hipGraphLaunch(m->graphs[g.key[h]].exec, st[h]));
        else launch_group(h);
    }
    for (int h = 1; fork && h < g.n; ++h) {
        HIPCHK(m, hipEventRecord(m->join_ev[h - 1], st[h]));
        HIPCHK(m, hipStreamWaitEvent(s, m->join_ev[h - 1], 0));
    }
    return ARTALK_OK;
}

}

namespace artalk {
int begin_clips(artalk_model* m, hipStream_t s, int B, const float* style_motion_dev, const uint8_t* has_style, bool encode_style,
                artalk_model::Stage* stg) {
    Workspace& w = m->ws;
    if (!has_style) style_motion_dev = nullptr;
    if (style_motion_dev) {
        std::memcpy(stg->has, has_style, (size_t)B);
        HIPCHK(m, hipMemcpyAsync(w.has_style, stg->has, B, hipMemcpyHostToDevice, s));
    }
    HIPCHK(m, hipEventRecord(stg->done, s));
    stg->used = true;
    HIPCHK(m, hipMemsetAsync(w.status, 0, 4 * sizeof(int), s));
    stage_mark(m, s, PB_OTHER);
    run_style(m, style_motion_dev, B, s, encode_style);
    stage_mark(m, s, PB_STYLE);
    return ARTALK_OK;
}
int chunk_step(artalk_model* m, hipStream_t s, int cond_row0, int Bn, int n_next, int tap_chunk, float* out_motion_dev, int64_t out_stride) {
    Workspace& w = m->ws;
    m->tap_chunk = tap_chunk;
    roctxRangePushA("artalk.ar.adaln_table");
    kbucket(m, KB_ADA);
    linear(m, w.silu_cond + (long)cond_row0 * kNTok * kCond, kCond, m->ada_w, m->ada_b, w.ada, m->ada_n, Bn * kNTok, m->ada_n, kCond,
           ACT_NONE, nullptr, s, m->precision == 1 ? LF_A_P8 : 0, nullptr, m->ex.silu_cond);
    roctxRangePop();
    stage_mark(m, s, PB_ADA);
    if (body_uses_graphs(m)) {
        Range r_body("artalk.body.graph");
        if (int rc = run_body(m, Bn, s, n_next)) return rc;
        stage_mark(m, s, PB_AR);
    } else {
        if (int rc = run_body(m, Bn, s, n_next)) return rc;
    }
    const size_t mrow = (size_t)100 * m->cfg.motion_dim * 4;
    HIPCHK(m, hipMemcpy2DAsync(out_motion_dev, (size_t)out_stride * 4, w.motion_chunk, mrow, mrow, Bn, hipMemcpyDeviceToDevice, s));
    return ARTALK_OK;
}

}
```

### artalk_amd/csrc/gemm_f16s.hip

```cpp
#include <algorithm>
#include <cmath>
#include <cstdlib>
#include <type_traits>
#include "common.h"
#include "gemm_tile.h"

namespace artalk {

typedef _Float16 f16x4 __attribute__((ext_vector_type(4)));
typedef unsigned int u32x4 __attribute__((ext_vector_type(4)));
typedef unsigned int u32x2 __attribute__((ext_vector_type(2)));

__device__ __forceinline__ void split_f32x4(const f32x4 x, const float scale, u32x2& hi, u32x2& lo) {
    f16x4 h, l;
#pragma unroll
    for (int e = 0; e < 4; ++e) { _Float16 a, b; split_f16(x[e] * scale, a, b); h[e] = a; l[e] = b; }
    hi = __builtin_bit_cast(u32x2, h);
    lo = __builtin_bit_cast(u32x2, l);
}
__device__ __forceinline__ int p8_lds_offset(int c) { return (c & 1) * 64 + (c >> 1) * 16; }

__global__ __launch_bounds__(256) void pack_split_kernel(const float* __restrict__ w, unsigned int* __restrict__ out, long n, float scale,
                                                         int* __restrict__ status, unsigned int maxbits) {
    for (long i = ((long)blockIdx.x * 256 + threadIdx.x) * 8; i < n; i += (long)gridDim.x * 2048) {
        const f32x4 a = *reinterpret_cast<const f32x4*>(w + i), b = *reinterpret_cast<const f32x4*>(w + i + 4);
        if (status) {
            p8_guard(status, a[0], a[1], a[2], a[3], maxbits);
            p8_guard(status, b[0], b[1], b[2], b[3], maxbits);
        }
        u32x2 h0, l0, h1, l1;
        split_f32x4(a, scale, h0, l0);
        split_f32x4(b, scale, h1, l1);
        u32x4 hi = {h0[0], h0[1], h1[0], h1[1]}, lo = {l0[0], l0[1], l1[0], l1[1]};
        *reinterpret_cast<u32x4*>(out + i) = hi;
        *reinterpret_cast<u32x4*>(out + i + 4) = lo;
    }
}
void launch_pack_split(const float* w, unsigned int* out, long n, bool is_weight, hipStream_t s, int* status, int p8_exp) {
    if (n <= 0) return;
    if (is_weight) status = nullptr;
    const long blocks = (n / 8 + 255) / 256;
    ARTALK_LAUNCH(pack_split_kernel, dim3((unsigned)(blocks < 8192 ? blocks : 8192)), dim3(256), 0, s, w, out, n, is_weight ? kWScale : p8_scale_of(p8_exp), status, p8_maxbits_of(p8_exp));
}

template <int BM, int BN, int WM, int WN, int APK, int TAG, int AMODE = 0>
__global__ __launch_bounds__(256, 2) void gemm_f16s_kernel(const GemmArgs g) {
    constexpr int BK = 32;
    constexpr int ROWB = 144;
    constexpr int TM = BM / WM / 32, TN = BN / WN / 32;
    constexpr int A_LD = BM / 32, B_LD = BN / 32;
    extern __shared__ __attribute__((aligned(16))) unsigned char smem_h[];
    unsigned char* As = smem_h;
    unsigned char* Bs = smem_h + 2 * BM * ROWB;

    const int tid = threadIdx.x;
    const int tiles_n = (g.N + BN - 1) / BN, tiles_m = (g.M + BM - 1) / BM;
    int tm, tn;
    tile_order(gridDim.x, blockIdx.x, tiles_m, tiles_n, (BM >= 128) ? 4 : 8, tm, tn);
    const int m0 = tm * BM, n0 = tn * BN;
    const int z = blockIdx.z;
    const float* __restrict__ A = g.A + z * g.sA;
    const unsigned int* __restrict__ Wp = g.Wp + z * g.sW;

    u32x4 ra[A_LD];
    u32x4 rb[B_LD];
    const int lrow = tid >> 3, lc4 = (tid & 7) * 4;

    auto gload = [&](int kt) {
        const int k = kt * BK + lc4;
#pragma unroll
        for (int i = 0; i < A_LD; ++i) {
            const int gm = m0 + lrow + i * 32;
            u32x4 v = {0u, 0u, 0u, 0u};
            if (gm < g.M) {
                if (AMODE == 0) {
                    v = *reinterpret_cast<const u32x4*>(A + (long)gm * g.lda + k);
                } else {
                    long off;
                    if (window_src(g, gm, k, off)) v = *reinterpret_cast<const u32x4*>(A + off);
                }
            }
            ra[i] = v;
        }
#pragma unroll
        for (int i = 0; i < B_LD; ++i) {
            const int gn = n0 + lrow + i * 32;
            u32x4 v = {0u, 0u, 0u, 0u};
            if (gn < g.N) v = *reinterpret_cast<const u32x4*>(Wp + (long)gn * g.ldw + k);
            rb[i] = v;
        }
    };
    auto lstore = [&](int buf) {
#pragma unroll
        for (int i = 0; i < A_LD; ++i) {
            unsigned char* p = As + (buf * BM + lrow + i * 32) * ROWB;
            if (APK) {
                *reinterpret_cast<u32x4*>(p + p8_lds_offset(tid & 7)) = ra[i];
            } else {
                u32x2 hi, lo;
                {
                    const f32x4 av = __builtin_bit_cast(f32x4, ra[i]);
                    p8_guard(g.status, av[0], av[1], av[2], av[3], p8_maxbits_of(g.a_exp));
                }
                split_f32x4(__builtin_bit_cast(f32x4, ra[i]), p8_scale_of(g.a_exp), hi, lo);
                *reinterpret_cast<u32x2*>(p + lc4 * 2) = hi;
                *reinterpret_cast<u32x2*>(p + lc4 * 2 + 64) = lo;
            }
        }
#pragma unroll
        for (int i = 0; i < B_LD; ++i) {
            *reinterpret_cast<u32x4*>(Bs + (buf * BN + lrow + i * 32) * ROWB + p8_lds_offset(tid & 7)) = rb[i];
        }
    };

    const int wave = tid >> 6, lane = tid & 63;
    const int wm = wave / WN, wn = wave % WN;
    const int r = lane & 31, h = lane >> 5;

    f32x16 acc[TM][TN];
    zero_acc(acc);

    int kt0, nkt;
    k_range(g.K / BK, blockIdx.y, g.splitk, kt0, nkt);
    const int nk = kt0 + nkt;
    gload(kt0);
    lstore(0);
    __syncthreads();
    for (int kt = kt0; kt < nk; ++kt) {
        const int buf = (kt - kt0) & 1;
        if (kt + 1 < nk) gload(kt + 1);
        const unsigned char* as = As + (buf * BM + wm * (BM / WM) + r) * ROWB + h * 16;
        const unsigned char* bs = Bs + (buf * BN + wn * (BN / WN) + r) * ROWB + h * 16;
#pragma unroll
        for (int kb = 0; kb < 2; ++kb) {
            f16x8 ah[TM], al[TM], bh[TN], bl[TN];
#pragma unroll
            for (int i = 0; i < TM; ++i) {
                ah[i] = *reinterpret_cast<const f16x8*>(as + i * 32 * ROWB + kb * 32);
                al[i] = *reinterpret_cast<const f16x8*>(as + i * 32 * ROWB + kb * 32 + 64);
            }
#pragma unroll
            for (int j = 0; j < TN; ++j) {
                bh[j] = *reinterpret_cast<const f16x8*>(bs + j * 32 * ROWB + kb * 32);
                bl[j] = *reinterpret_cast<const f16x8*>(bs + j * 32 * ROWB + kb * 32 + 64);
            }
#pragma unroll
            for (int i = 0; i < TM; ++i)
#pragma unroll
                for (int j = 0; j < TN; ++j) {
                    acc[i][j] = __builtin_amdgcn_mfma_f32_32x32x16_f16(bh[j], ah[i], acc[i][j], 0, 0, 0);
                    acc[i][j] = __builtin_amdgcn_mfma_f32_32x32x16_f16(bl[j], ah[i], acc[i][j], 0, 0, 0);
                    acc[i][j] = __builtin_amdgcn_mfma_f32_32x32x16_f16(bh[j], al[i], acc[i][j], 0, 0, 0);
                }
        }
        if (kt + 1 < nk) lstore(buf ^ 1);
        __syncthreads();
    }

    if (g.splitk > 1) {
        scale_acc(acc, p8_out_scale_of(g.a_exp));
        float* __restrict__ P = g.partial + (long)blockIdx.y * g.M * g.N;
#pragma unroll
        for (int i = 0; i < TM; ++i)
#pragma unroll
            for (int j = 0; j < TN; ++j) partial_tile32(g, P, m0 + wm * (BM / WM) + i * 32 + r, n0 + wn * (BN / WN) + j * 32, h, acc[i][j]);
        return;
    }
    const EpiCtx epi = make_epi(g, g.bias ? g.bias + z * g.sBias : nullptr, g.C + z * g.sC, g.R ? g.R + z * g.sR : nullptr);
    epilogue_tiles<true, true, TM, TN>(g, epi, m0 + wm * (BM / WM) + r, n0 + wn * (BN / WN), h, acc, p8_out_scale_of(g.a_exp));
}

template <int U, int N, class F>
__device__ __forceinline__ void static_for(F&& f) {
    if constexpr (U < N) {
        f(std::integral_constant<int, U>{});
        static_for<U + 1, N>(f);
    }
}
template <int TM, bool RES, int TAG = 0>
__global__ __launch_bounds__(512, 1) void gemm_p8_big_kernel(const GemmArgs g) {
    constexpr int BM = 64 * TM, BN = 256, BK = 32;
    constexpr int STAGE_BYTES = (BM + BN) * 128;
    constexpr int NDMA = TM + 4;
    constexpr int NSUB = 2 * TM;
    constexpr int BIAS_OFF = 2 * STAGE_BYTES;
    extern __shared__ __attribute__((aligned(16))) unsigned char smem_p8[];

    const int tid = threadIdx.x;
    const int wave = __builtin_amdgcn_readfirstlane(tid >> 6);
    const int tiles_n = (g.N + BN - 1) / BN, tiles_m = (g.M + BM - 1) / BM;
    const int ntiles = tiles_n * tiles_m;
    const int wm = wave >> 2, wn = wave & 3;
    const int nk = g.K / BK;
    int lane = tid & 63, r, h, prow, pchunk;
    unsigned a_off[2], w_off[2];
// ... 1162 lines not shown
```

### artalk_amd/csrc/kernels.h

```cpp
#pragma once
#include <hip/hip_runtime.h>
#include <climits>
#include <cstdint>

#include <hip/hip_ext.h>
#include <utility>
#include <vector>

namespace artalk {

struct KernelTimer {
    int bucket = 0;
    std::vector<hipEvent_t> pool; size_t used = 0;
    std::vector<std::pair<int, size_t>> recs;
};
extern thread_local KernelTimer* g_ktimer;
bool ktimer_events(hipEvent_t* e0, hipEvent_t* e1);
#define ARTALK_LAUNCH(kernel, grid, block, lds, stream, ...)                                                          \
    do {                                                                                                              \
        hipEvent_t kt_e0_ = nullptr, kt_e1_ = nullptr;                                                                \
        if (artalk::g_ktimer && artalk::ktimer_events(&kt_e0_, &kt_e1_))                                              \
            hipExtLaunchKernelGGL(kernel, grid, block, lds, stream, kt_e0_, kt_e1_, 0, __VA_ARGS__);                  \
        else                                                                                                          \
            hipLaunchKernelGGL(kernel, grid, block, lds, stream, __VA_ARGS__);                                        \
    } while (0)

struct RowMap {
    int rpb;
    int bstride;
    int off;
};
static inline RowMap rowmap_identity() { return RowMap{INT_MAX, 0, 0}; }
static inline RowMap rowmap(int rows_per_batch, int batch_stride_rows, int row_off) {
    return RowMap{rows_per_batch, batch_stride_rows, row_off};
}

enum Act { ACT_NONE = 0, ACT_GELU_ERF = 1, ACT_GELU_TANH = 2, ACT_LEAKY02 = 3 };
constexpr int kActExp = 4;

struct GemmArgs {
    const float* A = nullptr; long lda = 0;
    const float* W = nullptr; long ldw = 0;
    const unsigned int* Wp = nullptr;
    const void* Wb = nullptr;
    int c_p8 = 0;
    int a_packed = 0;
    int a_exp = 4, c_exp = 4;
    int exact = 0;
    const float* bias = nullptr;
    float* C = nullptr; long ldc = 0; RowMap cmap = {INT_MAX, 0, 0};
    float* c2 = nullptr;
    const float* gate = nullptr; long ldg = 0; RowMap gmap = {INT_MAX, 0, 0};
    const float* R = nullptr; long ldr = 0;
    int M = 0, N = 0, K = 0;
    int act = ACT_NONE;
    int batch = 1; long sA = 0, sW = 0, sBias = 0, sC = 0, sR = 0;
    int amode = 0; int pc_T = 0, pc_tstride = 0, pc_pad = 0, pc_cin = 0;
    int splitk = 1; float* partial = nullptr;
    int ngrp = 0; long grpW = 0, grpB = 0, grpC = 0;
    int res_lds = 0;
    int w_nt = 0;
    int cus = 0;
    int force_cfg = -1;
    int graph_tag = 0;
    int* status = nullptr;
};
void launch_gemm(const GemmArgs& g, hipStream_t s);
void launch_splitk_reduce(const GemmArgs& g, hipStream_t s);
struct LnArgs;
bool splitk_reduce_ln_eligible(const GemmArgs& g, const LnArgs& ln);
void launch_splitk_reduce_ln(const GemmArgs& g, const LnArgs& ln, hipStream_t s);
int gemm_config(const GemmArgs& g);
int gemm_tile_count(const GemmArgs& g);
void launch_pack_split(const float* w, unsigned int* out, long n, bool is_weight, hipStream_t s, int* status = nullptr, int p8_exp = kActExp);
bool gemm_p8_eligible(const GemmArgs& g);
void gemm_p8_prepare();
void launch_gemm_bf16(const GemmArgs& g, hipStream_t s);
int gemm_bf16_config(const GemmArgs& g);
int gemm_bf16_tile_count(const GemmArgs& g);
void launch_pack_bf16(const float* in, void* out, long n, hipStream_t s);

struct GemmPolicy {
    int precision = 0;
    bool reg_staged = false;
    float* slabs = nullptr; int64_t slab_floats = 0;
    int splitk_tiles = 0, splitk_target = 0;
};
enum GemmPath { GEMM_F32 = 0, GEMM_F16S = 1, GEMM_P8 = 2, GEMM_BF16 = 3 };
enum P8Class { P8_NONE = 0, P8_BIG, P8_GROUPS, P8_SMALL };
int gemm_p8_class(int cfg);
struct GemmPlan {
    int path = GEMM_F32;
    int cfg = -1;
    bool c2_fused = false;
    bool dominant = false;
    bool fused_ln = false;
};
GemmPlan plan_gemm(GemmArgs& g, const GemmPolicy& p, const LnArgs* fuse_ln);
void run_gemm(const GemmArgs& g, const GemmPlan& plan, const LnArgs* fuse_ln, hipStream_t s);
void launch_posconv_p8(const GemmArgs& g, int n_chunks, int T, int Ts, hipStream_t s);
static inline double gemm_flops(const GemmArgs& g) { return 2.0 * g.M * (double)g.N * g.K * g.batch; }

struct LnArgs {
    const float* X = nullptr; long ldx = 0;
    float* Y = nullptr; long ldy = 0;
    const float* w = nullptr; const float* b = nullptr;
    const float* scale = nullptr; const float* shift = nullptr;
    long ldm = 0; RowMap mmap = {INT_MAX, 0, 0};
    int M = 0, D = 0; float eps = 1e-5f; int act = ACT_NONE;
    int out_p8 = 0;
    int p8_exp = 4;
    int* status = nullptr;
    int junk_period = 0, junk_from = 0;
    int junk_row2 = 0, junk_period2 = 0, junk_from2 = 0;
    int plan_M = 0;
};
void launch_layernorm(const LnArgs& a, hipStream_t s);
struct AttnArgs {
    const float* Q = nullptr; long ldq = 0, q_bstride = 0;
    const float* K = nullptr; long ldk = 0, k_bstride = 0;
    const float* V = nullptr; long ldv = 0, v_bstride = 0;
    float* O = nullptr; long ldo = 0, o_bstride = 0;
    int B = 0, H = 0, HD = 64, Lq = 0, Lk = 0;
    float scale = 1.f;
    int l2norm = 0; const float* qscale = nullptr;
    int split_q = 0, split_k = 0;
    int out_p8 = 0;
    int split16 = 0;
    int qkv_p8 = 0;
    int qkv_exp = 4, o_exp = 4;
    int* status = nullptr;
    int cus = 0;
};
enum AttnKernel {
    ATTN_NONE = -1,
    ATTN_F32_64 = 0,
    ATTN_F32_32 = 1,
    ATTN_SHORT = 2,
    ATTN_F16 = 3,
    ATTN_F16_P8 = 4,
    ATTN_F16_WIDE = 5,
    ATTN_F16_PP = 6,
    ATTN_F16_WIDE_AR = 7,
    ATTN_F16_WIDE_AR_P8 = 8,
};
AttnKernel plan_attention(const AttnArgs& a, int n_cu);
AttnKernel launch_attention(const AttnArgs& a, hipStream_t s);
void attention_prepare();

void launch_audio_normalize(const float* audio, const long* src_off, float* xnorm, int n_chunks, int n, hipStream_t s);
void launch_conv0(const float* xnorm, int n, const float* w , const float* bias, const float* lnw,
                  const float* lnb, float* Y, int n_chunks, int T, int row_stride, hipStream_t s, int out_p8 = 0, int* status = nullptr, int p8_exp = kActExp);
void launch_conv_tail_gather(const float* X, const long* tab, float* Y, int n_chunks, int Tw, int Ts, int D, hipStream_t s);
void launch_pool_silu(const float* X, int x_tstride, int T, float* Y, int n_chunks, const int* patch_nums, int n_lvls,
                      int D, hipStream_t s, int out_p8 = 0, int* status = nullptr, int p8_exp = kActExp);

void launch_ar_bits_next(const float* logits, uint8_t* bits, float* fhat, float* nextfeat, int B, int level, hipStream_t s,
                         int* status = nullptr);
void launch_vq_embed(const float* feat, int n, const float* We, const float* be, const float* pos, float* X, int xrows,
                     int xoff, const float* style_cond, const float* pos0, int B, hipStream_t s);
void launch_ar_begin(const float* style_cond, const float* lvlpos, float* x0, float* fhat, int B, hipStream_t s);
void launch_dec_input(const float* prev_fdec, const float* fhat, const uint8_t* bits, const float* dpos, float* X,
                      int B, hipStream_t s);
void launch_dec_finish(const float* dec , const float* mean, const float* stdv, const float* epos,
                       float* out, long out_bstride, int chunk, float* E, int B, hipStream_t s, int* status = nullptr);
void launch_enc_input_zero(const float* mean, const float* stdv, const float* epos, float* E, int B, hipStream_t s);
void launch_broadcast16(const void* src, void* dst, long bytes, int B, hipStream_t s);
struct SessionRows {
    uint4* style; uint4* prev_in; uint4* prev_fdec;
    int s16, p16, f16;
};
void launch_session_gather(const float* const* slots, const SessionRows& w, int n, hipStream_t s);
void launch_session_scatter(float* const* slots, const SessionRows& w, int n, bool with_style, hipStream_t s);
void launch_bsq_history(const float* enc_out, uint8_t* hist_bits, float* prev_fdec, float* msfeat, int B, hipStream_t s,
                        int* status = nullptr);
void launch_style_input(const float* motion, const float* mean, const float* stdv, float* X, int B, hipStream_t s);
void launch_style_finish(const float* feat , const float* Ws, const float* bs, const float* null_cond,
                         const uint8_t* has_style, float* style_cond, int B, hipStream_t s, const float* cached = nullptr,
                         long cached_stride = 0);
void launch_add_row(float* X, const float* v, int M, int D, hipStream_t s);
void launch_savgol(const float* in, float* out, int T, int D, hipStream_t s);
constexpr int kSavgolLag = 4, kSavgolCarry = 9, kSavgolMaxOut = 104;
void launch_savgol_stream(float* const* slots, const int4* meta, long carry_off, const float* raw, long raw_stride, float* out,
                          long out_stride, int n, int D, hipStream_t s);

double launch_mfma_f32_peak(float* out, int blocks, int iters, int nacc, hipStream_t s);
void launch_resample_mean(const float* x, int nch, int n, const float* taps, int orig, int nw, int width, float* out, int n_out,
                          hipStream_t s);
void launch_flame_pose(const float* pose, float* rot, float* feat, int T, int ldf, hipStream_t s);
void launch_flame_joints(const float* vs, const float* jreg, float* J, int T, int V, hipStream_t s);
void launch_flame_skin(const float* vposed, const float* rot, const float* J, const int* parents, const float* weights, float* out,
                       int T, int V, float scale, hipStream_t s);
void launch_absmax(const float* buf, int rows, int cols, long ld, int is_p8, unsigned int* slot, hipStream_t s, int junk_period = 0,
                   int junk_from = 0, int p8_exp = kActExp);
int init_ms_tables();

}
```

### artalk_amd/csrc/model.h

```cpp
#pragma once
#include "kernels.h"
#include "../../include/artalk_hip.h"

#include <rocprofiler-sdk-roctx/roctx.h>

#include <cstdint>
#include <map>
#include <set>
#include <string>
#include <vector>

namespace artalk {

enum { KB_STYLE = 0, KB_CONV = 1, KB_ENC = 2, KB_ADA = 3, KB_AR_MISC = 4, KB_LEVEL0 = 5, KB_VAE_DEC = 10, KB_REENC = 11, KB_OTHER = 12, KB_N = 13 };
enum { PB_STYLE = 0, PB_CONV = 1, PB_ENC = 2, PB_ADA = 3, PB_AR = 4, PB_VAE = 5, PB_OTHER = 6 };

constexpr int kSamplesPerChunk = 64000;
constexpr int kE = 768;
constexpr int kCond = 1024;
constexpr int kNTok = 181;
constexpr int kMaxLv = 5;
constexpr int kAuditSlots = 1024;

struct Range {
    explicit Range(const char* name) { roctxRangePushA(name); }
    ~Range() { roctxRangePop(); }
    Range(const Range&) = delete;
    Range& operator=(const Range&) = delete;
};

enum SlotKind { SK_DIRECT, SK_PADK, SK_CONV, SK_HOST, SK_IGNORE };

struct Slot {
    std::vector<int64_t> shape;
    int dtype = ARTALK_DTYPE_F32;
    SlotKind kind = SK_DIRECT;
    float* dst = nullptr;
    int64_t pad_to = 0;
    bool set = false;
    std::vector<float> host;
    std::vector<int64_t> host_i64;
    int64_t numel() const { int64_t n = 1; for (auto d : shape) n *= d; return n; }
};

struct W2VLayer { float *qkv_w, *qkv_b, *out_w, *out_b, *ln1w, *ln1b, *ln2w, *ln2b, *ff1_w, *ff1_b, *ff2_w, *ff2_b; };
struct ARLayer { float *qkv_w, *qkv_b, *proj_w, *proj_b, *ffn1_w, *ffn1_b, *ffn2_w, *ffn2_b, *qscale; };
struct VAELayer { float *lnw, *lnb, *qkv_w, *out_w, *out_b, *m1_w, *m1_b, *m2_w, *m2_b; };
struct VAESide { float *in_w, *in_b, *out_w, *out_b; std::vector<VAELayer> layers; };
struct StyleLayer { float *in_w, *in_b, *out_w, *out_b, *l1_w, *l1_b, *l2_w, *l2_b, *n1w, *n1b, *n2w, *n2b; };

struct SiteExps {
    int conv[8]; int fp_ln, posconv_in;
    struct W2V { int ln1, qkv, attn, ln2, ffn; } w2v[64];
    int silu_cond, hist_tok;
    struct AR { int ln1, attn, ln2, ffn; } ar[32];
    struct VAE { int ln, qkv, attn, resid, mlp; } vae[2][16];
    int vae_enc_in, vae_dec_in, vae_dec_head;
    int style_in; struct ST { int h, attn, h1, ffn; } style[8];
    SiteExps() { int* p = reinterpret_cast<int*>(this); for (size_t i = 0; i < sizeof(SiteExps) / sizeof(int); ++i) p[i] = kActExp; }
};

struct Workspace {
    int maxB = 0, maxC = 0, G = 0;
    long* src_off = nullptr; float *xnorm = nullptr, *convA = nullptr, *convB = nullptr;
    float *h0 = nullptr, *h1 = nullptr, *xln = nullptr, *qkv = nullptr, *att = nullptr, *ffn = nullptr;
    float* silu_cond = nullptr;
    float *ada = nullptr, *style_cond = nullptr, *prev_in = nullptr, *prev_in_p8 = nullptr, *cache = nullptr;
    float *x = nullptr, *xmod = nullptr, *attn_out = nullptr, *ffn_h = nullptr, *logits = nullptr;
    float *fhat = nullptr, *nextfeat = nullptr;
    float* splitk = nullptr; int64_t splitk_floats = 0;
    float* splitk_b[4] = {nullptr, nullptr, nullptr, nullptr};
    uint8_t *bits = nullptr, *hist_bits = nullptr, *has_style = nullptr;
    int* status = nullptr;
    float** sess_slots = nullptr;
    float *prev_fdec = nullptr, *msfeat = nullptr, *dec_x = nullptr, *vh = nullptr, *vln = nullptr, *vqkv = nullptr;
    float *vatt = nullptr, *vmlp = nullptr, *dec_out = nullptr, *enc_in = nullptr, *enc_out = nullptr, *motion_chunk = nullptr;
    float *s_in = nullptr, *s_h = nullptr, *s_qkv = nullptr, *s_att = nullptr, *s_ffn = nullptr, *s_tmp = nullptr;
    int64_t bytes = 0;
};

struct ClipBuf { float* Workspace::*f; uint8_t* Workspace::*u8; int64_t n; };

struct ConvPasses { int np = 0; int off[4]{}, n[4]{}, cls[4]{}; const long* perm = nullptr; const long* tab = nullptr; };

enum { TAP_BLK0_IN = 0, TAP_BLK0_OUT = kNTok * kE, TAP_BLKL_OUT = 2 * kNTok * kE, TAP_PREV_IN = 3 * kNTok * kE,
       TAP_LOGITS = 4 * kNTok * kE, TAP_DEC_OUT = 4 * kNTok * kE + kNTok * 64, TAP_SLOT = 4 * kNTok * kE + kNTok * 64 + 200 * 106 };

constexpr int64_t slot_carry_off(int code_dim) { return kE + (int64_t)kNTok * kE + 100LL * code_dim; }
constexpr int kOpCodeDim = 32, kOpMotionDim = 106;

}

using namespace artalk;

struct artalk_model {
    artalk_config cfg{};
    int device = 0;
    std::string err;
    bool finalized = false;
    std::map<std::string, Slot> slots;
    std::vector<void*> allocs;
    std::vector<void*> ws_allocs;
    int64_t weight_bytes = 0;
    struct PackRange { const float* base; int64_t n; unsigned int* packed; uint16_t* bf16; };
    std::vector<PackRange> wranges;
    int precision = 0;
    bool have_bf16 = false;
    int splitk_tiles = 192, splitk_target = 384;
    bool audit = false;
    unsigned int* audit_vals = nullptr;
    std::vector<std::string> audit_names;
    std::map<std::string, int> audit_index;
    std::vector<int*> audit_exp;
    SiteExps ex;
    int scales_changed = 0;
    struct Site { std::string name; int* ex; };
    std::vector<Site> sites;
    std::map<const int*, int> site_of;
    bool stream_scales_ended = false;
    struct InitHistory { uint8_t* bits = nullptr; float *fdec = nullptr, *msfeat = nullptr; bool valid = false; } init_hist[3];
    void invalidate_init_hist() { for (auto& ih : init_hist) ih.valid = false; }
    float* tap = nullptr; int tap_B = 0, tap_maxch = 0, tap_chunk = 0;
    std::vector<uint32_t> cu_mask;
    int n_cus = 0;
    int stream_B = 0;
    static constexpr int kSessBlock = 32;
    struct Sessions {
        std::vector<float*> blocks;
        std::vector<int64_t> owner;
        struct Open { int slot = 0; int64_t seen = 0; bool smooth_done = false; };
        std::map<int64_t, Open> open;
        std::set<int64_t> ended_by_scales;
        int64_t next_id = 1;
        void* smooth_tab = nullptr; int64_t smooth_cap = 0;
    } sess;
    int64_t sess_carry_off() const { return slot_carry_off(cfg.code_dim); }
    int64_t sess_slot_floats() const { return sess_carry_off() + (kSavgolCarry * (int64_t)cfg.motion_dim + 3) / 4 * 4; }
    float* sess_slot(int i) const { return sess.blocks[i / kSessBlock] + (int64_t)(i % kSessBlock) * sess_slot_floats(); }
    Workspace* view = nullptr;
    bool sticky_error = false;
    int n_conv = 0; int conv_T[8]{}; int conv_S[8]{};
    int Tw = 0, Ts = 0;
    struct TailGeo { bool partial = false; int tc = 0; int T[8]{}, S[8]{}; } tail_geo[4];
    bool tail_skip = true;
    int ada_n = 0;
    int pn[kMaxLv]{}, off[kMaxLv + 1]{};
    float *conv0_w = nullptr, *conv_b[8]{}, *conv_lnw[8]{}, *conv_lnb[8]{}, *conv_w[8]{};
    float *fp_lnw = nullptr, *fp_lnb = nullptr, *fp_w = nullptr, *fp_b = nullptr;
    float *pos_w = nullptr, *pos_b = nullptr, *enc_lnw = nullptr, *enc_lnb = nullptr;
    std::vector<W2VLayer> w2v;
    float *ada_w = nullptr, *ada_b = nullptr;
    float *ar_qkv_w = nullptr, *ar_qkv_b = nullptr;
    std::vector<ARLayer> ar;
    float *logits_w = nullptr, *logits_b = nullptr, *vq_w = nullptr, *vq_b = nullptr, *sc_w = nullptr, *sc_b = nullptr;
    float *null_style = nullptr, *lvl_pos = nullptr, *prev_lvl_pos = nullptr;
    float *enc_pos = nullptr, *dec_pos = nullptr, *vae_mean = nullptr, *vae_std = nullptr;
    VAESide enc, dec;
    float *st_mean = nullptr, *st_std = nullptr, *st_pe = nullptr, *st_proj_w = nullptr, *st_proj_b = nullptr;
    std::vector<StyleLayer> style;
    Workspace ws;
    int profiling = 0;
    KernelTimer ktimer;
    bool use_graphs = true;
    bool in_graph_body = false;
    bool in_body = false;
    std::vector<hipEvent_t> ev_pool; size_t ev_used = 0;
    std::vector<std::pair<size_t, double>> dom_events;
    std::vector<std::pair<int, size_t>> marks;
    hipStream_t prof_stream = nullptr;
    hipStream_t side_stream[3] = {nullptr, nullptr, nullptr};
    hipEvent_t fork_ev = nullptr, join_ev[3] = {nullptr, nullptr, nullptr};
    int branches = 0;
    hipStream_t own_stream = nullptr;
    struct GraphEntry { hipGraphExec_t exec = nullptr; long long last_use = 0; };
    std::map<long long, GraphEntry> graphs;
    long long graph_clock = 0, graph_captures = 0;
    static constexpr int kStageSlots = 4;
    struct Stage { long* src = nullptr; uint8_t* has = nullptr; float** slots = nullptr; int4* smooth = nullptr; hipEvent_t done = nullptr; bool used = false; };
    Stage stage[kStageSlots];
    int stage_cap_c = 0, stage_cap_b = 0, stage_next = 0;
    static constexpr int kStatusSlots = 4;
    int* h_status = nullptr; hipEvent_t status_ev[kStatusSlots] = {nullptr, nullptr, nullptr, nullptr}; bool status_pending = false;
    long long ticket = 0;
};

#define HIPCHK(m, call)                                                                         \
    do {                                                                                        \
        hipError_t e_ = (call);                                                                 \
        if (e_ != hipSuccess) {                                                                 \
            (m)->err = std::string(#call) + ": " + hipGetErrorString(e_);                       \
            return ARTALK_EHIP;                                                                 \
        }                                                                                       \
    } while (0)

namespace artalk {

inline int fail(artalk_model* m, int code, const std::string& msg) { m->err = msg; return code; }
struct ProfilingOff {
    artalk_model* m; int saved;
    explicit ProfilingOff(artalk_model* x) : m(x), saved(x->profiling) { m->profiling = 0; }
    ~ProfilingOff() { m->profiling = saved; }
    ProfilingOff(const ProfilingOff&) = delete;
    ProfilingOff& operator=(const ProfilingOff&) = delete;
};

template <typename T>
T* dalloc_in(std::vector<void*>& pool, int64_t n) {
    void* p = nullptr;
    if (n <= 0) n = 1;
    if (hipMalloc(&p, n * sizeof(T)) != hipSuccess) { pool.push_back(nullptr); return nullptr; }
    (void)hipMemset(p, 0, n * sizeof(T));
    pool.push_back(p);
    return reinterpret_cast<T*>(p);
}
template <typename T>
T* dalloc(artalk_model* m, int64_t n) { return dalloc_in<T>(m->allocs, n); }


void stage_mark(artalk_model* m, hipStream_t s, int bucket);
void run_wav2vec(artalk_model* m, const float* audio, int c0, int n, float* out_w2v, hipStream_t s, const ConvPasses* tail = nullptr);
void run_style(artalk_model* m, const float* style_motion, int B, hipStream_t s, bool encode = true);
int run_init_history(artalk_model* m, int B, hipStream_t s);
int begin_clips(artalk_model* m, hipStream_t s, int B, const float* style_motion_dev, const uint8_t* has_style, bool encode_style,
                artalk_model::Stage* stg);
int chunk_step(artalk_model* m, hipStream_t s, int cond_row0, int Bn, int n_next, int tap_chunk, float* out_motion_dev, int64_t out_stride);
const unsigned int* packed_of(const artalk_model* m, const float* w);
const void* bf16_of(const artalk_model* m, const float* w);
int ensure_stage(artalk_model* m, int maxB, int maxC);
int next_stage(artalk_model* m, artalk_model::Stage** out);
int publish_status(artalk_model* m, hipStream_t s);
std::vector<ClipBuf> clip_buffers(const artalk_model* m);
int reserve(artalk_model* m, int maxB, int maxC);
void smooth_span(int64_t seen, int nf, bool last, int* first, int* count);
int smooth_row_range(const std::string& who, int nf, bool last, std::string* err);
int smooth_row_length(const std::string& who, int64_t seen, int nf, bool last, std::string* err);
int smooth_stride_check(const char* fn, bool have_raw, bool need_raw, int64_t raw_stride, int64_t out_stride, int D, std::string* err);
int smooth_check(artalk_model::Sessions& ss, const int64_t* ids, int n, bool have_raw, int64_t raw_stride, const int* n_frames,
                 const uint8_t* last, int64_t out_stride, int D, std::vector<artalk_model::Sessions::Open*>* st, std::string* err);

}
```

### artalk_amd/csrc/model.hip

```cpp
#include "model.h"

#include <algorithm>
#include <cmath>
#include <cstring>
#include <string>
#include <vector>

using namespace artalk;

namespace {
thread_local std::string g_create_error;

float* walloc(artalk_model* m, int64_t n) {
    m->weight_bytes += n * 4;
    float* p = dalloc<float>(m, n);
    m->wranges.push_back({p, n, nullptr, nullptr});
    return p;
}

}

namespace artalk {
const unsigned int* packed_of(const artalk_model* m, const float* w) {
    for (const auto& r : m->wranges)
// ... 459 lines not shown
    if (m->fork_ev) (void)hipEventDestroy(m->fork_ev);
    free_stage(m);
    for (auto& st : m->stage) if (st.done) (void)hipEventDestroy(st.done);
    if (m->h_status) (void)hipHostFree(m->h_status);
    for (auto& e : m->status_ev) if (e) (void)hipEventDestroy(e);
    for (void* p : m->allocs) if (p) (void)hipFree(p);
    for (void* p : m->ws_allocs) if (p) (void)hipFree(p);
    for (float* p : m->sess.blocks) if (p) (void)hipFree(p);
    if (m->sess.smooth_tab) (void)hipFree(m->sess.smooth_tab);
    delete m;
}

int artalk_set_tensor(artalk_model* m, const char* key, const void* host_ptr, int dtype, int ndim, const int64_t* shape) {
    if (!m || !key || !host_ptr || !shape) return ARTALK_EINVAL;
    if (m->finalized) return fail(m, ARTALK_ESTATE, "weights are final after artalk_finalize_weights (derived layouts and packed copies exist); create a new model");
    auto it = m->slots.find(key);
    if (it == m->slots.end()) return fail(m, ARTALK_EKEY, std::string("Unexpected key in state_dict: ") + key);
    Slot& s = it->second;
    bool same = (int)s.shape.size() == ndim && dtype == s.dtype;
    for (int i = 0; same && i < ndim; ++i) same = s.shape[i] == shape[i];
    if (!same) return fail(m, ARTALK_EINVAL, std::string("size mismatch for ") + key);
    (void)hipSetDevice(m->device);
    const int64_t n = s.numel();
    if (dtype == ARTALK_DTYPE_I64) {
        s.host_i64.assign((const int64_t*)host_ptr, (const int64_t*)host_ptr + n);
        s.set = true;
        return ARTALK_OK;
    }
    const float* src = (const float*)host_ptr;
    if (s.kind == SK_HOST || n <= 4096) s.host.assign(src, src + n);
    int rc = ARTALK_OK;
    switch (s.kind) {
        case SK_DIRECT: rc = upload(m, s.dst, src, n); break;
        case SK_PADK: {
            const int64_t o = s.shape[0], in = s.shape[1];
            std::vector<float> t((size_t)o * s.pad_to, 0.f);
            for (int64_t r = 0; r < o; ++r) std::memcpy(&t[r * s.pad_to], src + r * in, in * sizeof(float));
            rc = upload(m, s.dst, t.data(), (int64_t)t.size());
            break;
        }
        case SK_CONV: {
            const int64_t o = s.shape[0], ci = s.shape[1], k = s.shape[2];
            std::vector<float> t((size_t)n);
            for (int64_t a = 0; a < o; ++a)
                for (int64_t b = 0; b < ci; ++b)
                    for (int64_t d = 0; d < k; ++d) t[(a * k + d) * ci + b] = src[(a * ci + b) * k + d];
            rc = upload(m, s.dst, t.data(), n);
            break;
        }
        default: break;
    }
    if (rc == ARTALK_OK) s.set = true;
    return rc;
}

int artalk_finalize_weights(artalk_model* m) {
    if (!m) return ARTALK_EINVAL;
    (void)hipSetDevice(m->device);
    std::string missing;
    int nmiss = 0;
    for (auto& kv : m->slots)
        if (!kv.second.set) { if (nmiss++ < 8) missing += (missing.empty() ? "" : ", ") + kv.first; }
    if (nmiss) return fail(m, ARTALK_EMISSING, "Missing key(s) in state_dict: " + missing + (nmiss > 8 ? ", ..." : ""));
    const artalk_config& c = m->cfg;
    {
        const Slot& li = m->slots["lvl_idx"]; const Slot& le = m->slots["lvl_embed.weight"];
        const Slot& pe = m->slots["pos_embed"]; const Slot& ppe = m->slots["prev_pos_embed"];
        std::vector<float> a((size_t)kNTok * kE), b((size_t)kNTok * kE);
        int tok = 0;
        for (int p = 0; p < c.n_levels; ++p)
            for (int i = 0; i < c.patch_nums[p]; ++i, ++tok)
                if (li.host_i64[tok] != p) return fail(m, ARTALK_EINVAL, "lvl_idx does not match V_PATCH_NUMS");
        for (int t = 0; t < kNTok; ++t)
            for (int e = 0; e < kE; ++e) {
                const float lv = le.host[(size_t)li.host_i64[t] * kE + e];
                a[(size_t)t * kE + e] = lv + pe.host[(size_t)t * kE + e];
                b[(size_t)t * kE + e] = lv + ppe.host[(size_t)t * kE + e];
            }
        if (int rc = upload(m, m->lvl_pos, a.data(), (int64_t)a.size())) return rc;
        if (int rc = upload(m, m->prev_lvl_pos, b.data(), (int64_t)b.size())) return rc;
        const Slot& mk = m->slots["attn_bias_for_masking"];
        for (int q = 0; q < kNTok; ++q)
            for (int k = 0; k < 2 * kNTok; ++k) {
                const float v = mk.host[(size_t)q * 2 * kNTok + k];
                const bool vis = k < kNTok || li.host_i64[q] >= li.host_i64[k - kNTok];
                if (vis ? (v != 0.f) : !(std::isinf(v) && v < 0)) return fail(m, ARTALK_EINVAL, "attn_bias_for_masking is not the level-causal mask");
            }
        const Slot& vm = m->slots["basic_vae.attn_mask"];
        for (int q = 0; q < 200; ++q)
            for (int k = 0; k < 200; ++k) {
                const float v = vm.host[(size_t)q * 200 + k];
                const bool vis = !(q < 100 && k >= 100);
                if (vis ? (v != 0.f) : !(std::isinf(v) && v < 0)) return fail(m, ARTALK_EINVAL, "basic_vae.attn_mask is not the expected mask");
            }
    }
    for (int i = 0; i < c.ar_depth; ++i) {
        const Slot& sm = m->slots["attn_blocks." + std::to_string(i) + ".attn.scale_mul_1H11"];
        std::vector<float> q(c.ar_heads);
        for (int h = 0; h < c.ar_heads; ++h) q[h] = std::exp(std::min(sm.host[h], (float)std::log(100.0)));
        if (int rc = upload(m, m->ar[i].qscale, q.data(), c.ar_heads)) return rc;
    }
    {
        const Slot& pe = m->slots["style_encoder.PE.pe"];
        if (int rc = upload(m, m->st_pe, pe.host.data() + (size_t)c.style_len * c.style_dim, c.style_dim)) return rc;
    }
    {
        const std::string pc = "audio_encoder.encoder.pos_conv_embed.conv.parametrizations.weight.";
        const Slot& g = m->slots[pc + "original0"]; const Slot& v = m->slots[pc + "original1"];
        const int64_t O = v.shape[0], I = v.shape[1], K = v.shape[2];
        std::vector<double> nrm(K, 0.0);
        for (int64_t o = 0; o < O; ++o)
            for (int64_t i = 0; i < I; ++i)
                for (int64_t k = 0; k < K; ++k) { const double x = v.host[(o * I + i) * K + k]; nrm[k] += x * x; }
        std::vector<float> t((size_t)O * I * K);
        for (int64_t k = 0; k < K; ++k) {
            const float nk = (float)std::sqrt(nrm[k]);
            for (int64_t o = 0; o < O; ++o)
                for (int64_t i = 0; i < I; ++i) t[(o * K + k) * I + i] = v.host[(o * I + i) * K + k] * (g.host[k] / nk);
        }
        if (int rc = upload(m, m->pos_w, t.data(), (int64_t)t.size())) return rc;
    }
    for (auto& kv : m->slots) { std::vector<float>().swap(kv.second.host); }
    for (auto& r : m->wranges) {
        if (r.n < 1024 || r.packed) continue;
        r.packed = dalloc<unsigned int>(m, r.n);
        if (!r.packed) return fail(m, ARTALK_EHIP, "hipMalloc failed for packed weights");
        launch_pack_split(r.base, r.packed, r.n, true, nullptr);
    }
    HIPCHK(m, hipDeviceSynchronize());
    if (m->precision == 2) { if (int rc = ensure_bf16_copy(m)) return rc; }
    m->finalized = true;
    return ARTALK_OK;
}

int artalk_reserve(artalk_model* m, int max_batch, int max_total_chunks) {
    if (!m || max_batch <= 0 || max_total_chunks < max_batch) return ARTALK_EINVAL;
    (void)hipSetDevice(m->device);
    return reserve(m, max_batch, max_total_chunks);
}
int64_t artalk_workspace_bytes(const artalk_model* m) { return m ? m->ws.bytes : 0; }
int64_t artalk_weight_bytes(const artalk_model* m) { return m ? m->weight_bytes : 0; }

int artalk_set_profiling(artalk_model* m, int level) { if (!m || level < 0 || level > 3) return ARTALK_EINVAL; m->profiling = level; return ARTALK_OK; }
int artalk_set_precision(artalk_model* m, int mode) {
    if (!m || mode < 0 || mode > 2) return ARTALK_EINVAL;
    if (mode == 2 && m->finalized) {
        (void)hipSetDevice(m->device);
        if (int rc = ensure_bf16_copy(m)) return rc;
    }
    m->precision = mode;
    return ARTALK_OK;
}
int artalk_set_tail_skip(artalk_model* m, int on) { if (!m) return ARTALK_EINVAL; m->tail_skip = on != 0; return ARTALK_OK; }
int artalk_set_graphs(artalk_model* m, int enable) {
    if (!m) return ARTALK_EINVAL;
    m->use_graphs = (enable & 0xff) != 0;
    const int br = (enable >> 8) & 0xff;
    if (br >= 0 && br <= 4) m->branches = br; else return ARTALK_EINVAL;
    if ((enable >> 16) & 0xffff) {
        m->splitk_tiles = ((enable >> 16) & 0xff) * 16; m->splitk_target = ((enable >> 24) & 0xff) * 16;
    }
    (void)hipSetDevice(m->device); (void)hipDeviceSynchronize();
    drop_graphs(m);
    m->invalidate_init_hist();
    return ARTALK_OK;
}
int artalk_graph_count(const artalk_model* m, long long* captures) {
    if (!m) return ARTALK_EINVAL;
    if (captures) *captures = m->graph_captures;
    return (int)m->graphs.size();
}

int artalk_set_audit(artalk_model* m, int enable) {
    if (!m) return ARTALK_EINVAL;
    (void)hipSetDevice(m->device);
    if (enable && !m->audit_vals) {
        HIPCHK(m, hipMalloc(reinterpret_cast<void**>(&m->audit_vals), kAuditSlots * sizeof(unsigned int)));
        m->allocs.push_back(m->audit_vals);
    }
    if (enable) {
        HIPCHK(m, hipDeviceSynchronize());
        HIPCHK(m, hipMemset(m->audit_vals, 0, kAuditSlots * sizeof(unsigned int)));
        m->audit_names.clear(); m->audit_index.clear(); m->audit_exp.clear();
    }
    m->audit = enable != 0;
    return ARTALK_OK;
}
int artalk_calibrate(artalk_model* m, float headroom) {
    if (!m || !(headroom >= 1.0f)) return ARTALK_EINVAL;
    if (!m->audit_vals || m->audit_names.empty()) { m->err = "artalk_calibrate: no audit data (artalk_set_audit(1), then artalk_infer in f32 mode)"; return ARTALK_ESTATE; }
    (void)hipSetDevice(m->device);
    if (hipDeviceSynchronize() != hipSuccess) return ARTALK_EHIP;
    const int n = (int)m->audit_names.size();
    std::vector<unsigned int> bits((size_t)n);
    if (hipMemcpy(bits.data(), m->audit_vals, n * sizeof(unsigned int), hipMemcpyDeviceToHost) != hipSuccess) return ARTALK_EHIP;
    SiteExps next = m->ex;
    int* const base = reinterpret_cast<int*>(&m->ex);
    int* const nbase = reinterpret_cast<int*>(&next);
    for (int i = 0; i < n; ++i) {
        if (!m->audit_exp[i]) continue;
        int* ex = nbase + (m->audit_exp[i] - base);
        float mx;
        std::memcpy(&mx, &bits[i], sizeof(float));
        if (!std::isfinite(mx)) { m->err = "artalk_calibrate: site " + m->audit_names[i] + " is not finite (calibrate in f32 mode)"; return ARTALK_EINVAL; }
        if (mx <= 0.f) continue;
        int e = *ex;
        while (e > -8 && (double)mx * std::ldexp(1.0, e) * headroom > 65504.0) --e;
        if ((double)mx * std::ldexp(1.0, e) > 65504.0) { m->err = "artalk_calibrate: site " + m->audit_names[i] + " exceeds every supported scale"; return ARTALK_EINVAL; }
        *ex = e;
    }
    return commit_scales(m, next);
}
int artalk_reset_scales(artalk_model* m) {
    if (!m) return ARTALK_EINVAL;
    (void)hipSetDevice(m->device); (void)hipDeviceSynchronize();
    if (m->scales_changed) end_sessions_by_scales(m);
    m->ex = SiteExps();
    m->scales_changed = 0;
    drop_graphs(m);
    m->invalidate_init_hist();
    return ARTALK_OK;
}
int artalk_get_scales(artalk_model* m, int* exps, int max_n) {
    if (!m || !exps || max_n <= 0) return ARTALK_EINVAL;
    const int n = std::min<int>((int)m->audit_names.size(), max_n);
    for (int i = 0; i < n; ++i) exps[i] = m->audit_exp[i] ? *m->audit_exp[i] : kActExp;
    return n;
}
int artalk_scale_sites(const artalk_model* m, char* names_buf, int buf_len) {
    if (!m) return ARTALK_EINVAL;
    const int n = (int)m->sites.size();
    if (!names_buf) return n;
    int need = 0;
    for (const auto& st : m->sites) need += (int)st.name.size() + 1;
    if (buf_len < need) { const_cast<artalk_model*>(m)->err = "artalk_scale_sites: names need " + std::to_string(need) + " bytes"; return ARTALK_EINVAL; }
    int pos = 0;
    for (const auto& st : m->sites) { std::memcpy(names_buf + pos, st.name.c_str(), st.name.size() + 1); pos += (int)st.name.size() + 1; }
    return n;
}
int artalk_get_site_scales(artalk_model* m, int* exps, int n) {
    if (!m || !exps) return ARTALK_EINVAL;
    if (n != (int)m->sites.size()) return fail(m, ARTALK_EINVAL, "artalk_get_site_scales: n must equal the site count " + std::to_string(m->sites.size()));
    for (int i = 0; i < n; ++i) exps[i] = *m->sites[i].ex;
    return ARTALK_OK;
}
int artalk_set_site_scales(artalk_model* m, const int* exps, int n) {
    if (!m || !exps) return ARTALK_EINVAL;
    if (n != (int)m->sites.size()) return fail(m, ARTALK_EINVAL, "artalk_set_site_scales: n must equal the site count " + std::to_string(m->sites.size()));
    for (int i = 0; i < n; ++i)
        if (exps[i] < -8 || exps[i] > kActExp)
            return fail(m, ARTALK_EINVAL, "artalk_set_site_scales: exponent " + std::to_string(exps[i]) + " of site " + m->sites[i].name + " is outside [-8, 4]");
    SiteExps next = m->ex;
    int* const base = reinterpret_cast<int*>(&m->ex);
    int* const nbase = reinterpret_cast<int*>(&next);
    for (int i = 0; i < n; ++i) nbase[m->sites[i].ex - base] = exps[i];
    return commit_scales(m, next);
}
int artalk_get_audit(artalk_model* m, char* names_buf, int buf_len, float* values, int max_n) {
    if (!m || !names_buf || !values || buf_len <= 0 || max_n <= 0) return ARTALK_EINVAL;
    if (!m->audit_vals) return 0;
    (void)hipSetDevice(m->device);
    if (hipDeviceSynchronize() != hipSuccess) return ARTALK_EHIP;
    const int n = std::min<int>((int)m->audit_names.size(), max_n);
    std::vector<unsigned int> bits((size_t)std::max(n, 1));
    if (n && hipMemcpy(bits.data(), m->audit_vals, n * sizeof(unsigned int), hipMemcpyDeviceToHost) != hipSuccess) return ARTALK_EHIP;
    int pos = 0, written = 0;
    for (int i = 0; i < n; ++i) {
        const std::string& nm = m->audit_names[i];
        if (pos + (int)nm.size() + 1 > buf_len) break;
        std::memcpy(names_buf + pos, nm.c_str(), nm.size() + 1);
        pos += (int)nm.size() + 1;
        std::memcpy(&values[i], &bits[i], sizeof(float));
        ++written;
    }
    return written;
}

int artalk_set_tap(artalk_model* m, float* tap_dev, int max_batch, int max_chunks) {
    if (!m || max_batch < 0 || max_chunks < 0) return ARTALK_EINVAL;
    (void)hipSetDevice(m->device); (void)hipDeviceSynchronize();
    m->tap = tap_dev; m->tap_B = tap_dev ? max_batch : 0; m->tap_maxch = tap_dev ? max_chunks : 0; m->tap_chunk = 0;
    return ARTALK_OK;
}
int artalk_tap_layout(int64_t* out, int n) {
    if (!out || n < 7) return ARTALK_EINVAL;
    const int64_t v[7] = {TAP_BLK0_IN, TAP_BLK0_OUT, TAP_BLKL_OUT, TAP_PREV_IN, TAP_LOGITS, TAP_DEC_OUT, TAP_SLOT};
    for (int i = 0; i < 7; ++i) out[i] = v[i];
    return ARTALK_OK;
}

int artalk_set_cu_mask(artalk_model* m, const uint32_t* mask, int n_words) {
    if (!m || n_words < 0 || (n_words > 0 && !mask)) return ARTALK_EINVAL;
    (void)hipSetDevice(m->device); (void)hipDeviceSynchronize();
    m->cu_mask.assign(mask, mask + n_words);
    int n = 0;
    for (uint32_t w : m->cu_mask) n += __builtin_popcount(w);
    if (n_words > 0 && n < 8) { m->cu_mask.clear(); m->n_cus = 0; return fail(m, ARTALK_EINVAL, "a CU partition needs at least 8 compute units"); }
    int dev_cus = 0;
    if (hipDeviceGetAttribute(&dev_cus, hipDeviceAttributeMultiprocessorCount, m->device) == hipSuccess && dev_cus > 0) n = std::min(n, dev_cus);
    m->n_cus = n;
    for (int i = 0; i < 3; ++i) {
        if (m->side_stream[i]) { (void)hipStreamDestroy(m->side_stream[i]); m->side_stream[i] = nullptr; }
        if (m->join_ev[i]) { (void)hipEventDestroy(m->join_ev[i]); m->join_ev[i] = nullptr; }
    }
    drop_graphs(m);
    m->invalidate_init_hist();
// ... 72 lines not shown
```

### artalk_amd/model.py

```python
from __future__ import annotations

import ctypes as C
import math
from typing import List, Optional, Sequence

import numpy as np
import torch

from . import capi
from .config import ARTalkConfig

SCALES_FORMAT = "artalk-site-scales/1"
SCALE_EXP_MIN, SCALE_EXP_MAX = -8, 4


def check_scales(sites, names: Sequence[str]) -> List[int]:
    if not isinstance(sites, dict):
        raise ValueError("site scales must be a {site name: exponent} dict")
    missing = [n for n in names if n not in sites]
    extra = [n for n in sites if n not in set(names)]
    if missing or extra:
        raise ValueError("the site scales do not match this model's site table ({} missing, e.g. {}; {} extra, e.g. {}): they belong to "
                         "another architecture".format(len(missing), missing[:3], len(extra), extra[:3]))
    exps = []
# ... 170 lines not shown
        return self

    def reserve(self, max_batch: int, max_total_chunks: int):
        rc = capi.lib().artalk_reserve(self._h, int(max_batch), int(max_total_chunks))
        if rc != capi.OK:
            raise RuntimeError("artalk_reserve failed: " + self._err())
        self._reserved = (int(max_batch), int(max_total_chunks))

    def status(self, wait: bool = True) -> Optional[int]:
        f = C.c_int(0)
        if wait:
            rc = capi.lib().artalk_get_status(self._h, C.byref(f), None)
        else:
            rc = capi.lib().artalk_poll_status(self._h, C.byref(f))
            if rc == capi.EBUSY:
                return None
        if rc != capi.OK:
            raise RuntimeError("artalk status query failed: " + self._err())
        return int(f.value)

    _status = status

    def last_ticket(self) -> int:
        return int(capi.lib().artalk_last_ticket(self._h))

    def status_of(self, ticket: int) -> int:
        f = C.c_int(0)
        if capi.lib().artalk_get_status_of(self._h, C.c_longlong(ticket), C.byref(f)) != capi.OK:
            raise RuntimeError("artalk status query failed: " + self._err())
        return int(f.value)

    def calibrate(self, audios, style_motions=None, headroom: float = 4.0) -> int:
        L = capi.lib()
        prec, chk = self._precision, self.check_finite
        try:
            self.set_precision("f32")
            self.check_finite = False
            if L.artalk_set_audit(self._h, 1) != capi.OK:
                raise RuntimeError("artalk_set_audit failed: " + self._err())
            self.inference_batch(audios, style_motions, check=False)
            changed = int(L.artalk_calibrate(self._h, C.c_float(float(headroom))))
            if changed < 0:
                raise RuntimeError("artalk_calibrate failed: " + self._err())
        finally:
            L.artalk_set_audit(self._h, 0)
            self.check_finite = chk
            self.set_precision(prec)
        self._style_cache = {}
        self._sync_sessions()
        self._calibrations = getattr(self, "_calibrations", 0) + 1
        self._headroom = float(headroom)
        return changed

    def _site_names(self) -> List[str]:
        if getattr(self, "_site_table", None) is None:
            L = capi.lib()
            n = int(L.artalk_scale_sites(self._h, None, 0))
            if n < 0:
                raise RuntimeError("artalk_scale_sites failed: " + self._err())
            buf = C.create_string_buffer(n * 64 + 1024)
            if L.artalk_scale_sites(self._h, buf, len(buf)) != n:
                raise RuntimeError("artalk_scale_sites failed: " + self._err())
            self._site_table = [x.decode() for x in buf.raw.split(b"\0")[:n]]
        return self._site_table

    def _read_site_exps(self) -> List[int]:
        names = self._site_names()
        arr = (C.c_int * len(names))()
        if capi.lib().artalk_get_site_scales(self._h, arr, len(names)) != capi.OK:
            raise RuntimeError("artalk_get_site_scales failed: " + self._err())
        return [int(v) for v in arr]

    def _write_site_exps(self, exps: Sequence[int]) -> int:
        arr = (C.c_int * len(exps))(*exps)
        changed = int(capi.lib().artalk_set_site_scales(self._h, arr, len(exps)))
        if changed < 0:
            raise RuntimeError("artalk_set_site_scales failed: " + self._err())
        return changed

    def scales(self) -> dict:
        if not self._loaded:
            raise RuntimeError("load_state_dict must be called before scales")
        return dict(zip(self._site_names(), self._read_site_exps()))

    def load_scales(self, src) -> int:
        if not self._loaded:
            raise RuntimeError("load_state_dict must be called before load_scales")
        headroom = None
        if isinstance(src, dict):
            sites = src
        else:
            doc = read_scales_file(src)
            sites, headroom = doc["sites"], doc.get("headroom")
        exps = check_scales(sites, self._site_names())
        changed = self._write_site_exps(exps)
        if changed:
            self._n_streams = 0
            self._style_cache = {}
            self._sync_sessions()
        if not isinstance(src, dict) or changed:
            self._headroom = headroom
        return changed

    def save_scales(self, path):
        import dataclasses
        import json
        doc = {"format": SCALES_FORMAT, "sites": self.scales(), "config": dataclasses.asdict(self.cfg), "headroom": self._headroom}
        with open(path, "w") as f:
            json.dump(doc, f, indent=1)

    def reset_scales(self):
        if capi.lib().artalk_reset_scales(self._h) != capi.OK:
            raise RuntimeError("artalk_reset_scales failed: " + self._err())
        self._headroom = None
        self._sync_sessions()

    def _trip_to_f32(self, what: str):
        import warnings
        warnings.warn(f"artalk_amd: non-finite result in f16x3 mode ({what}); re-running in f32 mode and staying there "
                      "(set_precision('f16x3') switches back)")
        self.set_precision("f32")
        self._latched_f32 = True

    def workspace_bytes(self):
        return int(capi.lib().artalk_workspace_bytes(self._h))

    def weight_bytes(self):
        return int(capi.lib().artalk_weight_bytes(self._h))

    def set_profiling(self, level: int):
        capi.lib().artalk_set_profiling(self._h, int(level))

    def set_precision(self, mode):
        names = {0: "f32", 1: "f16x3", 2: "bf16"}
        code = {"f32": 0, "f16x3": 1, "bf16": 2}.get(mode, mode)
        if code not in names:
            raise ValueError(f"precision mode must be 'f32', 'f16x3' or 'bf16' (got {mode!r})")
        code = int(code)
        self._precision = names[code]
        self._latched_f32 = False
        if self._h is not None and self._loaded:
            rc = capi.lib().artalk_set_precision(self._h, int(code))
            if rc == capi.EINVAL:
                raise ValueError("precision mode must be 'f32', 'f16x3' or 'bf16'")
            if rc != capi.OK:
                raise RuntimeError(f"artalk_set_precision({code}) failed ({rc}): {self._err()}")

    def set_graphs(self, on: bool, branches: int = 0, splitk_tiles: int = 0, splitk_target: int = 0):
        capi.lib().artalk_set_graphs(self._h, int(bool(on)) | (int(branches) << 8) | ((splitk_tiles // 16) << 16) | ((splitk_target // 16) << 24))

    def set_tail_skip(self, on: bool):
        if capi.lib().artalk_set_tail_skip(self._h, int(bool(on))) != capi.OK:
            raise RuntimeError("artalk_set_tail_skip failed")

    def graph_count(self):
        n = C.c_longlong(0)
        held = capi.lib().artalk_graph_count(self._h, C.byref(n))
        return int(held), int(n.value)

    def set_cu_mask(self, words: Optional[Sequence[int]]):
        if not self._loaded:
            raise RuntimeError("load_state_dict must be called before set_cu_mask")
        L = capi.lib()
        self.stream_end()
        with torch.cuda.device(self._device):
            torch.cuda.synchronize()
            old = getattr(self, "_masked_handle", None)
            if old is not None:
                self._stream = None
                L.artalk_op_destroy_stream(C.c_void_p(old))
                self._masked_handle = None
            if words is None:
                if L.artalk_set_cu_mask(self._h, None, 0) != capi.OK:
                    raise RuntimeError("artalk_set_cu_mask failed: " + self._err())
                self._stream = None
                return
            arr = (C.c_uint32 * len(words))(*[int(w) & 0xFFFFFFFF for w in words])
            if L.artalk_set_cu_mask(self._h, C.cast(arr, C.c_void_p), len(words)) != capi.OK:
                raise RuntimeError("artalk_set_cu_mask failed: " + self._err())
            out = C.c_void_p()
            if L.artalk_op_create_masked_stream(C.cast(arr, C.c_void_p), len(words), C.byref(out)) != capi.OK:
                raise RuntimeError("hipExtStreamCreateWithCUMask failed")
            self._masked_handle = out.value
            self._stream = torch.cuda.ExternalStream(out.value, device=self._device)

    def get_profile(self):
        out = (C.c_double * 10)()
        rc = capi.lib().artalk_get_profile(self._h, out, 10)
        if rc != capi.OK:
            raise RuntimeError("artalk_get_profile failed: " + self._err())
        keys = ["style_ms", "w2v_conv_ms", "w2v_encoder_ms", "ada_ms", "ar_ms", "vae_ms", "total_ms",
                "dom_launches", "dom_ms", "dom_flop"]
        return dict(zip(keys, list(out)))

    def get_kernel_sums(self):
        out = (C.c_double * 14)()
        if capi.lib().artalk_get_kernel_sums(self._h, out, 14) != capi.OK:
            raise RuntimeError("artalk_get_kernel_sums failed: " + self._err())
        keys = ["style", "w2v_conv", "w2v_encoder", "ada", "ar_history_kv", "level0", "level1", "level2", "level3", "level4", "vae_decode",
                "reencode", "other", "kernels"]
        return dict(zip(keys, list(out)))

    def _style_key(self, s: torch.Tensor):
        if not s.is_cuda:
            return ("host", hash(s.detach().to(torch.float32).contiguous().numpy().tobytes()), self._precision)
        return ("dev", s.data_ptr(), s._version, tuple(s.stride()), s.dtype, str(s.device), self._precision)

    def _style_rows(self, style_motions, order, B):
        if style_motions is None or not any(s is not None for s in style_motions):
            return None, None
        dev = self._device
        L, D = self.cfg.style_len, self.cfg.motion_dim
        style_t = torch.zeros(B, L, D, dtype=torch.float32, device=dev)
        has = (C.c_uint8 * B)()
        keys = {}
        for pos, i in enumerate(order):
            s = style_motions[i]
            if s is None:
                continue
            assert tuple(s.shape) == (L, D), f"Invalid style_motion shape: {tuple(s.shape)}."
            if self.style_cache_size > 0:
                keys[pos] = self._style_key(s)
            else:
                style_t[pos] = s.to(device=dev, dtype=torch.float32)
                has[pos] = 1
        if keys:
            new = {}
            for pos, k in keys.items():
                if k not in self._style_cache and k not in new:
                    new[k] = style_motions[order[pos]]
            if new:
                clips = torch.stack([v.to(device=dev, dtype=torch.float32) for v in new.values()])
                cond = torch.empty(len(new), self.cfg.embed_dim, dtype=torch.float32, device=dev)
                self._stream.wait_stream(torch.cuda.current_stream())
                rc = capi.lib().artalk_style_encode(self._h, capi.ptr(clips), len(new), capi.ptr(cond), C.c_void_p(self._stream.cuda_stream))
                if rc != capi.OK:
                    raise RuntimeError("artalk_style_encode failed: " + self._err())
                torch.cuda.current_stream().wait_stream(self._stream)
                clips.record_stream(self._stream)
                cond.record_stream(self._stream)
                for j, (k, v) in enumerate(new.items()):
                    self._style_cache[k] = (v, cond[j])
                while len(self._style_cache) > self.style_cache_size:
                    self._style_cache.pop(next(iter(self._style_cache)))
            flat = style_t.view(B, L * D)
            for pos, k in keys.items():
                hit = self._style_cache.get(k) or (None, None)
                if hit[1] is None:
                    style_t[pos] = style_motions[order[pos]].to(device=dev, dtype=torch.float32)
                    has[pos] = 1
                else:
                    flat[pos, :self.cfg.embed_dim] = hit[1]
                    has[pos] = 2
        return style_t, has

    @torch.no_grad()
    def stream_begin(self, n_streams: int, style_motions: Optional[Sequence[Optional[torch.Tensor]]] = None):
        if not self._loaded:
            raise RuntimeError("load_state_dict must be called before inference")
        dev = self._device
        with torch.cuda.device(dev):
            if self._stream is None:
                self._stream = torch.cuda.Stream(device=dev)
            caller = torch.cuda.current_stream()
            self._stream.wait_stream(caller)
            self.stream_end()
            style_t, has = self._style_rows(style_motions, list(range(n_streams)), n_streams)
            self._stream.wait_stream(caller)
            rc = capi.lib().artalk_stream_begin(self._h, int(n_streams), capi.ptr(style_t),
                                                C.cast(has, C.c_void_p) if has is not None else None, C.c_void_p(self._stream.cuda_stream))
            caller.wait_stream(self._stream)
            if style_t is not None:
                style_t.record_stream(self._stream)
        if rc != capi.OK:
            raise RuntimeError("artalk_stream_begin failed: " + self._err())
        self._n_streams = int(n_streams)
        self._stream_style = style_motions
        self._stream_fed = [0] * self._n_streams

    @torch.no_grad()
    def stream_chunk(self, audio_chunks: torch.Tensor, n_valid: Optional[Sequence[int]] = None):
        B = getattr(self, "_n_streams", 0)
        if B <= 0:
            raise RuntimeError("stream_chunk before stream_begin")
        assert audio_chunks.shape == (B, self.cfg.samples_per_chunk), f"expected ({B}, {self.cfg.samples_per_chunk}) samples"
        dev = self._device
        with torch.cuda.device(dev):
            x = audio_chunks.to(device=dev, dtype=torch.float32).contiguous()
            out = torch.empty(B, 100, self.cfg.motion_dim, dtype=torch.float32, device=dev)
            caller = torch.cuda.current_stream()
            self._stream.wait_stream(caller)
            rc = capi.lib().artalk_stream_chunk(self._h, capi.ptr(x), x.stride(0), capi.ptr(out), out.stride(0),
                                                C.c_void_p(self._stream.cuda_stream))
            caller.wait_stream(self._stream)
            x.record_stream(self._stream)
            out.record_stream(self._stream)
        if rc != capi.OK:
            raise RuntimeError("artalk_stream_chunk failed: " + self._err())
        if self._precision == "f16x3" and self.check_finite and self.status() != 0:
            self.stream_end()
            if self.auto_calibrate:
                try:
                    changed = self.calibrate([x[b] for b in range(B)], self._stream_style)
                except RuntimeError:
                    changed = 0
                if changed > 0:
# ... 339 lines not shown
```

### include/artalk_hip.h

```cpp
#ifndef ARTALK_HIP_H
#define ARTALK_HIP_H

#include <stdint.h>

#ifdef __cplusplus
extern "C" {
#endif

#define ARTALK_OK 0
#define ARTALK_EINVAL (-1)
#define ARTALK_EKEY (-2)
#define ARTALK_EMISSING (-3)
#define ARTALK_EHIP (-4)
#define ARTALK_ESTATE (-5)
#define ARTALK_ECAPACITY (-6)
#define ARTALK_EBUSY (-7)

#define ARTALK_DTYPE_F32 0
#define ARTALK_DTYPE_I64 1

typedef struct artalk_model artalk_model;

typedef struct artalk_config {
    int32_t ar_depth, ar_heads;
    int32_t vae_depth, vae_heads, vae_hidden;
    int32_t code_dim, motion_dim;
    int32_t n_levels; int32_t patch_nums[8];
    int32_t w2v_layers, w2v_hidden, w2v_heads, w2v_ffn;
    int32_t w2v_n_conv; int32_t w2v_conv_kernel[8]; int32_t w2v_conv_stride[8]; int32_t w2v_conv_dim;
    int32_t w2v_pos_kernel, w2v_pos_groups;
    float w2v_ln_eps;
    int32_t style_dim, style_heads, style_layers, style_ffn, style_len;
} artalk_config;

int artalk_create(int device_id, const artalk_config* cfg, artalk_model** out);
void artalk_destroy(artalk_model* m);
const char* artalk_last_error(const artalk_model* m);

int artalk_set_tensor(artalk_model* m, const char* key, const void* host_ptr, int dtype, int ndim, const int64_t* shape);
int artalk_finalize_weights(artalk_model* m);

int artalk_reserve(artalk_model* m, int max_batch, int max_total_chunks);
int64_t artalk_workspace_bytes(const artalk_model* m);
int64_t artalk_weight_bytes(const artalk_model* m);

int artalk_infer(artalk_model* m, const float* audio_dev, int64_t audio_clip_stride, const int64_t* n_chunks, int B,
                 const float* style_motion_dev, const uint8_t* has_style, float* out_motion_dev, int64_t out_clip_stride,
                 uint8_t* out_bits_dev, uint8_t* out_hist_bits_dev, float* out_w2v_dev, void* stream);

int artalk_infer_samples(artalk_model* m, const float* audio_dev, int64_t audio_clip_stride, const int64_t* n_chunks,
                         const int64_t* n_samples, int B, const float* style_motion_dev, const uint8_t* has_style, float* out_motion_dev,
                         int64_t out_clip_stride, uint8_t* out_bits_dev, uint8_t* out_hist_bits_dev, float* out_w2v_dev, void* stream);
int artalk_set_tail_skip(artalk_model* m, int on);
int artalk_conv_tail_geometry(int64_t valid, int samples_per_chunk, int n_conv, const int* kernel, const int* stride, int* t_const,
                              int* Tp, int* Sp, int* samples_read);
int64_t artalk_conv_tail_class(int64_t valid, int samples_per_chunk);

int artalk_style_encode(artalk_model* m, const float* style_motion_dev, int n, float* out_cond_dev, void* stream);

int artalk_stream_end(artalk_model* m);
int artalk_stream_begin(artalk_model* m, int B, const float* style_motion_dev, const uint8_t* has_style, void* stream);
int artalk_stream_chunk(artalk_model* m, const float* audio_dev, int64_t chunk_stride, float* out_motion_dev, int64_t out_stride,
                        void* stream);

int artalk_sessions_reserve(artalk_model* m, int max_sessions);
int artalk_session_open(artalk_model* m, int n, const float* style_motion_dev, const uint8_t* has_style, int64_t* ids_out, void* stream);
int artalk_session_step(artalk_model* m, const int64_t* ids, int n, const float* audio_dev, int64_t chunk_stride, float* out_motion_dev,
                        int64_t out_stride, uint8_t* out_bits_dev, uint8_t* out_hist_bits_dev, void* stream);
int artalk_session_close(artalk_model* m, const int64_t* ids, int n);
int artalk_session_count(const artalk_model* m);
int artalk_session_smooth(artalk_model* m, const int64_t* ids, int n, const float* raw_dev, int64_t raw_stride, const int* n_frames,
                          const uint8_t* last, float* out_dev, int64_t out_stride, int* first_out, int* count_out, void* stream);

typedef struct artalk_flame artalk_flame;
int artalk_flame_create(int device_id, int V, int NB, int P, const float* v_template, const float* shapedirs, const float* posedirs_t,
                        const float* J_regressor, const int32_t* parents, const float* lbs_weights, float scale, artalk_flame** out);
int artalk_flame_verts(artalk_flame* f, const float* betas_dev, const float* full_pose_dev, int T, float* out_dev, void* stream);
void artalk_flame_destroy(artalk_flame* f);
const char* artalk_flame_last_error(const artalk_flame* f);

typedef struct artalk_mesh_renderer artalk_mesh_renderer;
int artalk_render_create(int device_id, int V, int F, const int32_t* faces_host, int image_size, float scale, artalk_mesh_renderer** out);
int artalk_render_mesh(artalk_mesh_renderer* r, const float* verts_dev, int T, const float* transform_3x4_host_or_null, float focal_or_0,
                       float* rgb_dev, float* alpha_dev, int32_t* pix_to_face_dev_or_null, void* stream);
int artalk_render_set_slab(artalk_mesh_renderer* r, int frames);
void artalk_render_destroy(artalk_mesh_renderer* r);
const char* artalk_render_last_error(const artalk_mesh_renderer* r);

typedef struct artalk_splat artalk_splat;
int artalk_splat_create(int device_id, artalk_splat** out);
int artalk_splat_render(artalk_splat* s, int N, int T, int H, int W, const float* means_dev, int64_t means_stride, const float* colors_dev,
                        int64_t colors_stride, const float* opacities_dev, int64_t opacities_stride, const float* scales_dev,
                        int64_t scales_stride, const float* rotations_dev, int64_t rotations_stride, const float* view_host,
                        const float* proj_host, int n_cams, float tanfovx, float tanfovy, float scale_modifier, const float* bg_dev_or_null,
                        float* out_dev, int32_t* radii_dev, void* stream);
int artalk_splat_set_timing(artalk_splat* s, int enable);
int artalk_splat_get_timing(const artalk_splat* s, double* stage_ms, int n, long long* pairs, int* frames);
void artalk_splat_destroy(artalk_splat* s);
const char* artalk_splat_last_error(const artalk_splat* s);

int artalk_get_status(artalk_model* m, int* flags, void* stream);
int artalk_poll_status(artalk_model* m, int* flags);
long long artalk_last_ticket(artalk_model* m);
int artalk_get_status_of(artalk_model* m, long long ticket, int* flags);

int artalk_savgol(artalk_model* m, const float* in_dev, float* out_dev, int T, void* stream);

int artalk_set_profiling(artalk_model* m, int level);
int artalk_get_profile(artalk_model* m, double* out, int n);
int artalk_get_kernel_sums(artalk_model* m, double* out, int n);
int artalk_set_precision(artalk_model* m, int mode);
int artalk_set_graphs(artalk_model* m, int enable);
int artalk_graph_count(const artalk_model* m, long long* captures);
int artalk_set_audit(artalk_model* m, int enable);
int artalk_get_audit(artalk_model* m, char* names_buf, int buf_len, float* values, int max_n);
int artalk_calibrate(artalk_model* m, float headroom);
int artalk_reset_scales(artalk_model* m);
int artalk_get_scales(artalk_model* m, int* exps, int max_n);
int artalk_scale_sites(const artalk_model* m, char* names_buf, int buf_len);
int artalk_get_site_scales(artalk_model* m, int* exps, int n);
int artalk_set_site_scales(artalk_model* m, const int* exps, int n);
int artalk_set_tap(artalk_model* m, float* tap_dev, int max_batch, int max_chunks);
int artalk_tap_layout(int64_t* out, int n);
int artalk_set_cu_mask(artalk_model* m, const uint32_t* mask, int n_words);

int artalk_op_gemm(const float* A, int64_t lda, const float* W, const float* bias, const float* gate, const float* R,
                   float* C, int M, int N, int K, int act, void* stream);
int artalk_op_gemm_ex(const float* A, int64_t lda, const float* W, const float* bias, float* C, int M, int N, int K, int act,
                      int force_cfg, void* stream);
int artalk_op_mfma_f32_peak(float* out_dev, int blocks, int iters, int nacc, double* flops, void* stream);
int artalk_op_gemm_f16s(const float* A, int64_t lda, const float* W, const float* bias, float* C, int M, int N, int K, int act,
                        int force_cfg, void* stream);
int artalk_op_gemm_bf16(const float* A, int64_t lda, const float* W, const float* bias, const float* gate, const float* R, float* C,
                        int M, int N, int K, int act, int force_cfg, void* stream);
int artalk_op_pack_split(const float* in, void* out_u32, int64_t n, int is_weight, void* stream);
int artalk_op_gemm_f16s_packed(const void* A, int a_packed, int64_t lda, const void* Wp, const float* bias, float* C, int M, int N,
                               int K, int act, int force_cfg, void* stream);
int artalk_op_release_scratch(void);
int artalk_op_gemm_p8_plan(int M, int N, int K, int residual);
int artalk_op_create_masked_stream(const uint32_t* mask, int n_words, void** out_stream);
int artalk_op_destroy_stream(void* stream);
int artalk_op_layernorm(const float* X, float* Y, const float* w, const float* b, const float* scale, const float* shift,
                        int M, int D, float eps, int act, void* stream);
int artalk_op_attention(const float* Q, const float* K, const float* V, float* O, int B, int H, int HD, int Lq, int Lk,
                        float scale, int l2norm, const float* qscale, int split, void* stream);
int artalk_op_w2v_front(const float* audio, int C, int n, const float* w, const float* bias, const float* lnw,
                        const float* lnb, float* xnorm_out, float* Y, void* stream);
int artalk_op_resample_mean(const float* x, int nch, int n, const float* taps, int orig, int nw, int width, float* out, int n_out,
                            void* stream);
int artalk_op_pool_silu(const float* X, int C, int T, int D, float* Y, void* stream);
int artalk_op_pack_split_ex(const float* in, void* out_u32, int64_t n, int is_weight, int p8_exp, int* status_dev, void* stream);
int artalk_op_layernorm_ex(const float* X, float* Y, const float* w, const float* b, const float* scale, const float* shift,
                           int M, int D, float eps, int act, int p8_exp, int junk_period, int junk_from, int* status_dev, void* stream);
int artalk_op_gemm_f16s_packed_ex(const void* A, int a_packed, int64_t lda, const void* Wp, const float* bias, float* C, int M, int N,
                                  int K, int act, int force_cfg, int a_exp, int c_exp, void* c2_u32, int* status_dev, void* stream);
int artalk_op_gemm_f16s_ex(const float* A, int64_t lda, const float* W, const float* bias, float* C, int M, int N, int K, int act,
                           int force_cfg, int a_exp, int* status_dev, void* stream);
int artalk_op_attention_ex(const float* Q, const float* K, const float* V, float* O, int B, int H, int HD, int Lq, int Lk,
                           float scale, int l2norm, const float* qscale, int split, int qkv_exp, int o_exp, int out_p8,
                           int* status_dev, void* stream);
int artalk_op_w2v_front_ex(const float* audio, int C, int n, const float* w, const float* bias, const float* lnw,
                           const float* lnb, float* xnorm_out, float* Y, int out_p8, int p8_exp, int* status_dev, void* stream);
int artalk_op_pool_silu_ex(const float* X, int C, int T, int D, float* Y, int out_p8, int p8_exp, int* status_dev, void* stream);
int artalk_op_posconv_p8_ex(const float* X, const void* Wp, const float* bias, const float* R, float* C, int n_chunks, int T, int Ts,
                            int act, int a_exp, int* status_dev, void* stream);
int artalk_op_bsq_history(const float* enc_out, uint8_t* hist_bits, float* prev_fdec, float* msfeat, int B, void* stream);
int artalk_op_bsq_history_ex(const float* enc_out, uint8_t* hist_bits, float* prev_fdec, float* msfeat, int B, int* status_dev,
                             void* stream);
int artalk_op_ar_bits_next(const float* logits, uint8_t* bits, float* fhat, float* nextfeat, int B, int level, int* status_dev,
                           void* stream);
int artalk_op_vq_embed(const float* feat, int n, const float* We, const float* be, const float* pos, float* X, int xrows, int xoff,
                       const float* style_cond, const float* pos0, int B, void* stream);
int artalk_op_ar_begin(const float* style_cond, const float* lvlpos, float* x0, float* fhat, int B, void* stream);
int artalk_op_dec_input(const float* prev_fdec, const float* fhat, const uint8_t* bits, const float* dpos, float* X, int B, void* stream);
int artalk_op_dec_finish(const float* dec, const float* mean, const float* std_, const float* epos, float* out, int64_t out_bstride,
                         int chunk, float* E, int B, int* status_dev, void* stream);
int artalk_op_enc_input_zero(const float* mean, const float* std_, const float* epos, float* E, int B, void* stream);
int artalk_op_style_input(const float* motion, const float* mean, const float* std_, float* X, int B, void* stream);
int artalk_op_add_row(float* X, const float* v, int M, int D, void* stream);
int artalk_op_style_finish(const float* feat, const float* Ws, const float* bs, const float* null_cond, const uint8_t* has_style,
                           float* style_cond, int B, const float* cached, int64_t cached_stride, void* stream);
int artalk_op_broadcast16(const void* src, void* dst, int64_t bytes, int B, void* stream);
int artalk_op_session_gather(const float* const* slots_dev, float* style, float* prev_in, float* prev_fdec, int s16, int p16, int f16, int n,
                             void* stream);
int artalk_op_session_scatter(float* const* slots_dev, const float* style, const float* prev_in, const float* prev_fdec, int s16, int p16,
                              int f16, int n, int with_style, void* stream);
int artalk_op_savgol_stream(float* const* slots_dev, const float* raw, int64_t raw_stride, const int* seen, const int* n_frames,
                            const uint8_t* last, float* out, int64_t out_stride, int n, void* stream);
int artalk_op_session_smooth_check(const int64_t* open_ids, const int64_t* open_seen, const uint8_t* open_done, int n_open,
                                   const int64_t* ended_ids, int n_ended, const int64_t* ids, int n, int have_raw, int64_t raw_stride,
                                   const int* n_frames, const uint8_t* last, int64_t out_stride, int* first_out, int* count_out, char* msg,
                                   int msg_len);
int artalk_op_absmax(const float* buf, int rows, int cols, int64_t ld, int is_p8, int p8_exp, int junk_period, int junk_from,
                     unsigned int* slot_dev, void* stream);
typedef struct artalk_op_gemm_rows_args {
    int32_t mode, M, N, K, act;
    const void* A; int64_t lda, a_elems; int32_t a_exp;
    const float* W; int64_t ldw, w_elems;
    const float* bias; int64_t bias_elems;
    void* C; int64_t ldc, c_elems; int32_t cmap[3];
    const float* gate; int64_t ldg, gate_elems; int32_t gmap[3];
    const float* R; int64_t ldr, r_elems;
    int32_t c_p8, c_exp;
    int32_t force_cfg, splitk;
    int32_t ngrp; int64_t grpW, grpB, grpC;
    int32_t* status_dev;
// ... 47 lines not shown
```

Measured before the change: 103,900.

## Cache initial-history K/V projections and broadcast them on the first chunk

On the first chunk every clip starts from the same initial history tokens, so the history K/V projection GEMM for all but the first row gives identical output per clip. The change computes those shared K/V rows once per precision and GEMM plan, keeps them in a small LRU cache, and on first chunks runs the GEMM only for the one per-clip row before broadcasting the cached rows into each clip's cache slot. It adds extra device memory, a first-time fill that needs host syncs, and epoch/precision marks to invalidate the cache. Results may differ slightly from the original path because of plan/split-k differences, which the cache key tries to guard against.

```diff
diff --git a/artalk_amd/capi.py b/artalk_amd/capi.py
--- a/artalk_amd/capi.py
+++ b/artalk_amd/capi.py
@@ -24,7 +24,7 @@
     "artalk_op_gemm_rows", "artalk_op_layernorm_rows", "artalk_op_attention_rows", "artalk_op_gemm_rows_layout", "artalk_op_rows_dry_run",
     "artalk_op_w2v_front_rows", "artalk_op_pool_silu_rows", "artalk_op_posconv_rows",
     "artalk_op_attention_plan", "artalk_op_attention_rows_cus",
-    "artalk_infer_samples", "artalk_set_tail_skip", "artalk_conv_tail_geometry", "artalk_conv_tail_class",
+    "artalk_infer_samples", "artalk_set_tail_skip", "artalk_set_init_kv_cache", "artalk_conv_tail_geometry", "artalk_conv_tail_class",
     "artalk_render_create", "artalk_render_mesh", "artalk_render_set_slab", "artalk_render_destroy", "artalk_render_last_error",
     "artalk_splat_create", "artalk_splat_render", "artalk_splat_set_timing", "artalk_splat_get_timing", "artalk_splat_destroy",
     "artalk_splat_last_error",
@@ -156,6 +156,9 @@
         L.artalk_conv_tail_geometry.restype = i32
         L.artalk_conv_tail_class.argtypes = [i64, i32]
         L.artalk_conv_tail_class.restype = i64
+    if hasattr(L, "artalk_set_init_kv_cache"):
+        L.artalk_set_init_kv_cache.argtypes = [vp, i32]
+        L.artalk_set_init_kv_cache.restype = i32
     L.artalk_get_status.argtypes = [vp, C.POINTER(C.c_int), vp]
     L.artalk_get_status.restype = i32
     L.artalk_poll_status.argtypes = [vp, C.POINTER(C.c_int)]
diff --git a/artalk_amd/csrc/ar_glue.hip b/artalk_amd/csrc/ar_glue.hip
--- a/artalk_amd/csrc/ar_glue.hip
+++ b/artalk_amd/csrc/ar_glue.hip
@@ -255,6 +255,23 @@
     ARTALK_LAUNCH(broadcast16_kernel, dim3((n16 + 255) / 256 < 8 ? (n16 + 255) / 256 : 8, B), dim3(256), 0, s,
                        reinterpret_cast<const uint4*>(src), reinterpret_cast<uint4*>(dst), n16);
 }
+constexpr int BR_ROWS = 12;
+__global__ __launch_bounds__(256) void broadcast_rows16_kernel(const uint4* __restrict__ src, uint4* __restrict__ dst, int rows, int c16,
+                                                               long dst_layer16, long dst_clip16, long dst_row16) {
+    const int r0 = blockIdx.x * BR_ROWS, nr = min(BR_ROWS, rows - r0);
+    const uint4* sp = src + ((long)blockIdx.z * rows + r0) * c16;
+    uint4* dp = dst + (long)blockIdx.z * dst_layer16 + (long)blockIdx.y * dst_clip16 + (long)r0 * dst_row16;
+    for (int i = threadIdx.x; i < nr * c16; i += 256) {
+        const int r = i / c16, c = i - r * c16;
+        dp[(long)r * dst_row16 + c] = sp[i];
+    }
+}
+void launch_broadcast_rows16(const float* src, float* dst, int L, int rows, int cols, long dst_layer, long dst_clip, long dst_row, int B,
+                             hipStream_t s) {
+    if (L <= 0 || rows <= 0 || cols <= 0 || B <= 0) return;
+    ARTALK_LAUNCH(broadcast_rows16_kernel, dim3((rows + BR_ROWS - 1) / BR_ROWS, B, L), dim3(256), 0, s, reinterpret_cast<const uint4*>(src),
+                  reinterpret_cast<uint4*>(dst), rows, cols / 4, dst_layer / 4, dst_clip / 4, dst_row / 4);
+}
 
 void launch_enc_input_zero(const float* mean, const float* stdv, const float* epos, float* E, int B, hipStream_t s) {
     ARTALK_LAUNCH(enc_input_zero_kernel, dim3(B), dim3(256), 0, s, mean, stdv, epos, E, 106, 128);
diff --git a/artalk_amd/csrc/calls.hip b/artalk_amd/csrc/calls.hip
--- a/artalk_amd/csrc/calls.hip
+++ b/artalk_amd/csrc/calls.hip
@@ -213,7 +213,7 @@
     for (int64_t j = 0; j < maxch; ++j) {
         const int Bn = Bj[j];
         const int n_next = out_hist_bits_dev ? Bn : (j + 1 < maxch ? Bj[j + 1] : 0);
-        if (int rc = chunk_step(m, s, base[j], Bn, n_next, (int)j, out_motion_dev + j * 100 * c.motion_dim, out_clip_stride)) return rc;
+        if (int rc = chunk_step(m, s, base[j], Bn, n_next, (int)j, out_motion_dev + j * 100 * c.motion_dim, out_clip_stride, j == 0)) return rc;
         if (out_bits_dev)
             HIPCHK(m, hipMemcpy2DAsync(out_bits_dev + j * bits_row, (size_t)maxch * bits_row, w.bits, bits_row, bits_row, Bn,
                                        hipMemcpyDeviceToDevice, s));
@@ -262,6 +262,7 @@
         if (int rc = run_init_history(m, B, s)) return rc;
     }
     m->stream_B = B; m->stream_scales_ended = false;
+    m->stream_init = m->mark_init();
     if (int rc = publish_status(m, s)) return rc;
     return ARTALK_OK;
 }
@@ -285,7 +286,9 @@
     stg->used = true;
     ProfilingOff quiet(m);
     for (int c0 = 0; c0 < B; c0 += w.G) run_wav2vec(m, audio_dev, c0, std::min(w.G, B - c0), nullptr, s);
-    if (int rc = chunk_step(m, s, 0, B, B, m->tap_maxch, out_motion_dev, out_stride)) return rc;
+    const bool first = m->on_init_history(m->stream_init);
+    m->stream_init = artalk_model::InitMark();
+    if (int rc = chunk_step(m, s, 0, B, B, m->tap_maxch, out_motion_dev, out_stride, first)) return rc;
     if (int rc = publish_status(m, s)) return rc;
     return ARTALK_OK;
 }
@@ -332,7 +335,9 @@
     for (int i = 0; i < n; ++i) {
         ids_out[i] = ss.next_id++;
         ss.owner[slot[i]] = ids_out[i];
-        ss.open.emplace(ids_out[i], artalk_model::Sessions::Open{slot[i]});
+        artalk_model::Sessions::Open o;
+        o.slot = slot[i]; o.init = m->mark_init();
+        ss.open.emplace(ids_out[i], o);
     }
     return ARTALK_OK;
 }
@@ -363,7 +368,9 @@
     ProfilingOff quiet(m);
     launch_session_gather(w.sess_slots, rows, n, s);
     for (int c0 = 0; c0 < n; c0 += w.G) run_wav2vec(m, audio_dev, c0, std::min(w.G, n - c0), nullptr, s);
-    if (int rc = chunk_step(m, s, 0, n, n, m->tap_maxch, out_motion_dev, out_stride)) return rc;
+    bool first = true;
+    for (int i = 0; i < n; ++i) { first &= m->on_init_history(st[i]->init); st[i]->init = artalk_model::InitMark(); }
+    if (int rc = chunk_step(m, s, 0, n, n, m->tap_maxch, out_motion_dev, out_stride, first)) return rc;
     launch_session_scatter(w.sess_slots, rows, n, false, s);
     const size_t bits_n = (size_t)n * kNTok * m->cfg.code_dim;
     if (out_bits_dev) HIPCHK(m, hipMemcpyAsync(out_bits_dev, w.bits, bits_n, hipMemcpyDeviceToDevice, s));
diff --git a/artalk_amd/csrc/engine.hip b/artalk_amd/csrc/engine.hip
--- a/artalk_amd/csrc/engine.hip
+++ b/artalk_amd/csrc/engine.hip
@@ -69,8 +69,8 @@
     launch_absmax(buf, rows, cols & ~7, ld, is_p8 ? 1 : 0, m->audit_vals + idx, s, junk_period, junk_from, ex ? *ex : kActExp);
 }
 
-bool gemm(artalk_model* m, const GemmArgs& g0, hipStream_t s, const LnArgs* fuse_ln = nullptr, int plan_M = 0) {
-    GemmArgs g = g0;
+bool plan_of(artalk_model* m, const GemmArgs& g0, const LnArgs* fuse_ln, int plan_M, GemmArgs& g, GemmPlan& plan) {
+    g = g0;
     const int run_M = g.M;
     if (plan_M > 0) g.M = plan_M;
     g.graph_tag = m->in_body ? 1 : 0;
@@ -86,7 +86,7 @@
     }
     const Workspace& cw = m->view ? *m->view : m->ws;
     const GemmPolicy pol{m->precision, false, cw.splitk, cw.splitk_floats, m->splitk_tiles, m->splitk_target};
-    GemmPlan plan = plan_gemm(g, pol, fuse_ln);
+    plan = plan_gemm(g, pol, fuse_ln);
     if (plan_M > 0) {
         g.M = run_M;
         if (plan.path != GEMM_P8) g.force_cfg = plan.cfg;
@@ -98,6 +98,12 @@
         }
     }
     if (g.a_packed && plan.path == GEMM_F32) { m->err = "internal: P8 activation handed to an fp32 GEMM"; m->sticky_error = true; return false; }
+    return true;
+}
+bool gemm(artalk_model* m, const GemmArgs& g0, hipStream_t s, const LnArgs* fuse_ln = nullptr, int plan_M = 0) {
+    GemmArgs g;
+    GemmPlan plan;
+    if (!plan_of(m, g0, fuse_ln, plan_M, g, plan)) return false;
     const bool timed = m->profiling && plan.dominant && !m->in_body;
     size_t i0 = 0, i1 = 0;
     if (timed) next_event(m, s, &i0);
@@ -345,11 +351,13 @@
     struct Restore { artalk_model* m; ~Restore() { kbucket(m, KB_OTHER); } } restore{m};
     Workspace& w = m->ws;
     artalk_model::InitHistory& ih = m->init_hist[m->precision];
-    const long nb = (long)kNTok * c.code_dim, nf = 100L * c.code_dim * 4, nm = 180L * c.code_dim * 4;
+    const long nb = (long)kNTok * c.code_dim, nf = 100L * c.code_dim * 4, nm = 180L * c.code_dim * 4, nt = (long)kNTok * kE * 4;
     if (!ih.valid) {
         if (!ih.bits) {
             ih.bits = dalloc<uint8_t>(m, nb); ih.fdec = dalloc<float>(m, nf / 4); ih.msfeat = dalloc<float>(m, nm / 4);
-            if (!ih.bits || !ih.fdec || !ih.msfeat) return fail(m, ARTALK_EHIP, "hipMalloc failed for the initial-history cache");
+            ih.tok = dalloc<float>(m, nt / 4); ih.tok_p8 = m->precision == 1 ? dalloc<float>(m, nt / 4) : nullptr;
+            if (!ih.bits || !ih.fdec || !ih.msfeat || !ih.tok || (m->precision == 1 && !ih.tok_p8))
+                return fail(m, ARTALK_EHIP, "hipMalloc failed for the initial-history cache");
             HIPCHK(m, hipDeviceSynchronize());
         }
         launch_enc_input_zero(m->vae_mean, m->vae_std, m->enc_pos, w.enc_in, 1, s);
@@ -357,6 +365,9 @@
         HIPCHK(m, hipMemcpyAsync(ih.bits, w.hist_bits, nb, hipMemcpyDeviceToDevice, s));
         HIPCHK(m, hipMemcpyAsync(ih.fdec, w.prev_fdec, nf, hipMemcpyDeviceToDevice, s));
         HIPCHK(m, hipMemcpyAsync(ih.msfeat, w.msfeat, nm, hipMemcpyDeviceToDevice, s));
+        HIPCHK(m, hipMemcpyAsync(ih.tok, w.prev_in, nt, hipMemcpyDeviceToDevice, s));
+        if (ih.tok_p8)
+            launch_pack_split(ih.tok + kE, reinterpret_cast<unsigned int*>(ih.tok_p8 + kE), (long)(kNTok - 1) * kE, false, s, w.status, m->ex.hist_tok);
         int flags[4] = {0, 0, 0, 0};
         HIPCHK(m, hipMemcpyAsync(flags, w.status, sizeof(int), hipMemcpyDeviceToHost, s));
         HIPCHK(m, hipStreamSynchronize(s));
@@ -372,40 +383,118 @@
 }
 
 namespace {
-void run_chunk_body(artalk_model* m, int B, hipStream_t s, int n_reencode = -1) {
-    struct BodyScope { artalk_model* m; BodyScope(artalk_model* x) : m(x) { m->in_body = true; } ~BodyScope() { m->in_body = false; } } scope(m);
+struct HistKVRows { const float* A; long lda; int M, plan_rows; float* C; long ldc; RowMap cmap; long layer_stride; };
+void hist_kv_gemm(artalk_model* m, const HistKVRows& r, hipStream_t s, artalk_model::InitKVKey* key) {
+    const artalk_config& c = m->cfg;
+    const int p8 = m->precision == 1 ? 1 : 0;
+    const int plan_M = r.plan_rows != r.M ? r.plan_rows : 0;
+    GemmArgs g;
+    g.A = r.A; g.a_packed = p8; g.a_exp = m->ex.hist_tok;
+    g.lda = r.lda; g.W = m->ar_qkv_w + (long)kE * kE; g.ldw = kE; g.bias = m->ar_qkv_b + kE;
+    g.C = r.C; g.ldc = r.ldc; g.cmap = r.cmap;
+    g.M = r.M; g.N = c.ar_depth * 2 * kE; g.K = kE;
+    g.ngrp = 2 * kE; g.grpW = (long)3 * kE * kE; g.grpB = 3 * kE; g.grpC = r.layer_stride;
+    g.Wp = packed_of(m, g.W);
+    GemmArgs whole = g;
+    whole.M = r.plan_rows;
+    const bool grouped = p8 && gemm_p8_eligible(whole);
+    auto layer = [&](int l) {
+        const ARLayer& L = m->ar[l];
+        GemmArgs q = g;
+        q.Wp = nullptr; q.ngrp = 0; q.grpW = q.grpB = q.grpC = 0;
+        q.W = L.qkv_w + (long)kE * kE; q.bias = L.qkv_b + kE; q.C = r.C + l * r.layer_stride; q.N = 2 * kE;
+        return q;
+    };
+    if (key) {
+        GemmArgs f;
+        *key = artalk_model::InitKVKey();
+        key->precision = m->precision; key->grouped = grouped;
+        if (plan_of(m, grouped ? g : layer(0), nullptr, plan_M, f, key->plan)) key->splitk = f.splitk;
+        else key->precision = -1;
+        return;
+    }
+    if (grouped) { gemm(m, g, s, nullptr, plan_M); return; }
+    for (int l = 0; l < c.ar_depth; ++l) gemm(m, layer(l), s, nullptr, plan_M);
+}
+
+const float* ensure_init_kv(artalk_model* m, int gB, hipStream_t s, int* rc) {
+    *rc = ARTALK_OK;
+    const artalk_config& c = m->cfg;
+    artalk_model::InitHistory& ih = m->init_hist[m->precision];
+    if (!m->init_kv_on || !ih.valid || !ih.tok) return nullptr;
+    const int p8 = m->precision == 1 ? 1 : 0;
+    const Workspace& w = m->ws;
+    const long cache_l = (long)w.maxB * 2 * kNTok * 3 * kE, kv_l = (long)(kNTok - 1) * 2 * kE;
+    artalk_model::InitKVKey key;
+    hist_kv_gemm(m, HistKVRows{p8 ? w.prev_in_p8 : w.prev_in, kE, gB * kNTok, gB * kNTok, w.cache + kE, 3 * kE, rowmap(kNTok, 2 * kNTok, 0), cache_l}, s, &key);
+    if (key.precision < 0) return nullptr;
+    const long long now = ++m->init_kv_clock;
+    for (auto& e : m->init_kv)
+        if (e.valid && e.key == key) { e.last_use = now; return e.kv; }
+    artalk_model::InitKV* slot = nullptr;
+    for (auto& e : m->init_kv)
+        if (!e.valid) { slot = &e; break; }
+    for (auto& e : m->init_kv)
+        if (e.valid && (!slot || (slot->valid && e.last_use < slot->last_use))) slot = &e;
+    auto hipfail = [&](hipError_t e) { m->err = std::string("initial-history K/V cache: ") + hipGetErrorString(e); *rc = ARTALK_EHIP; return (const float*)nullptr; };
+    if (hipError_t e = hipDeviceSynchronize()) return hipfail(e);
+    slot->valid = false;
+    if (!slot->kv) {
+        slot->kv = dalloc<float>(m, c.ar_depth * kv_l);
+        if (!slot->kv) { *rc = fail(m, ARTALK_EHIP, "hipMalloc failed for the initial-history K/V cache"); return nullptr; }
+        if (hipError_t e = hipDeviceSynchronize()) return hipfail(e);
+    }
+    {
+        struct FillScope { artalk_model* m; bool was; Workspace* view; FillScope(artalk_model* x) : m(x), was(x->in_body), view(x->view) { m->in_body = true; m->view = nullptr; }
+                           ~FillScope() { m->in_body = was; m->view = view; } } scope(m);
+        kbucket(m, KB_AR_MISC);
+        hist_kv_gemm(m, HistKVRows{(p8 ? ih.tok_p8 : ih.tok) + kE, kE, kNTok - 1, gB * kNTok, slot->kv, 2 * kE, rowmap_identity(), kv_l}, s, nullptr);
+    }
+    int flags[4] = {0, 0, 0, 0};
+    if (hipError_t e = hipMemcpyAsync(flags, w.status, sizeof(int), hipMemcpyDeviceToHost, s)) return hipfail(e);
+    if (hipError_t e = hipStreamSynchronize(s)) return hipfail(e);
+    if (flags[0] != 0) return nullptr;
+    slot->valid = true; slot->key = key; slot->last_use = now;
+    return slot->kv;
+}
+
+struct BodyScope { artalk_model* m; BodyScope(artalk_model* x) : m(x) { m->in_body = true; } ~BodyScope() { m->in_body = false; } };
+void run_history_kv(artalk_model* m, int B, hipStream_t s, const float* init_kv) {
+    BodyScope scope(m);
     const artalk_config& c = m->cfg;
     Workspace& w = m->view ? *m->view : m->ws;
-    const long ldada = m->ada_n;
     const long cache_l = (long)w.maxB * 2 * kNTok * 3 * kE;
     const int p8 = m->precision == 1 ? 1 : 0;
     kbucket(m, KB_AR_MISC);
     tap_copy(m, TAP_PREV_IN, 0, w.prev_in, kNTok, kE, B, s);
     roctxRangePushA("artalk.ar.history_kv");
     SiteExps& ex = m->ex;
-    if (p8) launch_pack_split(w.prev_in, reinterpret_cast<unsigned int*>(w.prev_in_p8), (long)B * kNTok * kE, false, s, w.status, ex.hist_tok);
-    audit(m, p8 ? w.prev_in_p8 : w.prev_in, B * kNTok, kE, kE, p8, s, &ex.hist_tok);
-    {
-        GemmArgs g;
-        g.A = p8 ? w.prev_in_p8 : w.prev_in; g.a_packed = p8; g.a_exp = ex.hist_tok;
-        g.lda = kE; g.W = m->ar_qkv_w + (long)kE * kE; g.ldw = kE; g.bias = m->ar_qkv_b + kE;
-        g.C = w.cache + kE; g.ldc = 3 * kE; g.cmap = rowmap(kNTok, 2 * kNTok, 0);
-        g.M = B * kNTok; g.N = c.ar_depth * 2 * kE; g.K = kE;
-        g.ngrp = 2 * kE; g.grpW = (long)3 * kE * kE; g.grpB = 3 * kE; g.grpC = cache_l;
-        g.Wp = packed_of(m, g.W);
-        if (p8 && gemm_p8_eligible(g)) {
-            gemm(m, g, s);
-        } else {
-            for (int l = 0; l < c.ar_depth; ++l) {
-                const ARLayer& L = m->ar[l];
-                GemmArgs q = g;
-                q.Wp = nullptr; q.ngrp = 0; q.grpW = q.grpB = q.grpC = 0;
-                q.W = L.qkv_w + (long)kE * kE; q.bias = L.qkv_b + kE; q.C = w.cache + l * cache_l + kE; q.N = 2 * kE;
-                gemm(m, q, s);
-            }
-        }
+    const float* prev = p8 ? w.prev_in_p8 : w.prev_in;
+    float* const kv0 = w.cache + kE;
+    const long kv_row = 3 * kE, kv_clip = 2L * kNTok * kv_row;
+    if (!init_kv) {
+        if (p8) launch_pack_split(w.prev_in, reinterpret_cast<unsigned int*>(w.prev_in_p8), (long)B * kNTok * kE, false, s, w.status, ex.hist_tok);
+        audit(m, prev, B * kNTok, kE, kE, p8, s, &ex.hist_tok);
+        hist_kv_gemm(m, HistKVRows{prev, kE, B * kNTok, B * kNTok, kv0, kv_row, rowmap(kNTok, 2 * kNTok, 0), cache_l}, s, nullptr);
+    } else {
+        if (p8) launch_pack_split_rows(w.prev_in, reinterpret_cast<unsigned int*>(w.prev_in_p8), B, kE, (long)kNTok * kE, s, w.status, ex.hist_tok);
+        const artalk_model::InitHistory& ih = m->init_hist[m->precision];
+        audit(m, prev, B, kE, (long)kNTok * kE, p8, s, &ex.hist_tok);
+        audit(m, (p8 ? ih.tok_p8 : ih.tok) + kE, kNTok - 1, kE, kE, p8, s, &ex.hist_tok);
+        hist_kv_gemm(m, HistKVRows{prev, (long)kNTok * kE, B, B * kNTok, kv0, kv_row, rowmap(1, 2 * kNTok, 0), cache_l}, s, nullptr);
+        launch_broadcast_rows16(init_kv, kv0 + kv_row, c.ar_depth, kNTok - 1, 2 * kE, cache_l, kv_clip, kv_row, B, s);
     }
     roctxRangePop();
+}
+
+void run_chunk_body(artalk_model* m, int B, hipStream_t s, int n_reencode = -1) {
+    BodyScope scope(m);
+    const artalk_config& c = m->cfg;
+    Workspace& w = m->view ? *m->view : m->ws;
+    const long ldada = m->ada_n;
+    const long cache_l = (long)w.maxB * 2 * kNTok * 3 * kE;
+    const int p8 = m->precision == 1 ? 1 : 0;
+    SiteExps& ex = m->ex;
     launch_ar_begin(w.style_cond, m->lvl_pos, w.x, w.fhat, B, s);
     static const char* const kLevelName[kMaxLv] = {"artalk.ar.scale_step0", "artalk.ar.scale_step1", "artalk.ar.scale_step2",
                                                    "artalk.ar.scale_step3", "artalk.ar.scale_step4"};
@@ -547,14 +636,21 @@
     }
     return g;
 }
-int run_body(artalk_model* m, int B, hipStream_t s, int n_next) {
+int run_body(artalk_model* m, int B, hipStream_t s, int n_next, bool init_history) {
     const BodyGroups g = plan_body(m, B, n_next);
+    const float* init_kv[4] = {nullptr, nullptr, nullptr, nullptr};
+    for (int h = 0; init_history && h < g.n; ++h) {
+        int rc = ARTALK_OK;
+        init_kv[h] = ensure_init_kv(m, g.b0[h + 1] - g.b0[h], s, &rc);
+        if (rc) return rc;
+    }
     const bool fork = g.n > 1 && m->profiling != 3;
     if (fork) { if (int rc = ensure_side_streams(m, g.n - 1)) return rc; }
     hipStream_t st[4] = {s, s, s, s};
     for (int h = 1; fork && h < g.n; ++h) st[h] = m->side_stream[h - 1];
     Workspace views[4];
     for (int h = 0; h < g.n; ++h) views[h] = clip_view(m, g.b0[h], h);
+    auto launch_history = [&](int h) { m->view = &views[h]; run_history_kv(m, g.b0[h + 1] - g.b0[h], st[h], init_kv[h]); m->view = nullptr; };
     auto launch_group = [&](int h) { m->view = &views[h]; run_chunk_body(m, g.b0[h + 1] - g.b0[h], st[h], g.nre[h]); m->view = nullptr; };
     for (int h = 0; g.graphs && h < g.n; ++h) {
         auto hit = m->graphs.find(g.key[h]);
@@ -577,6 +673,7 @@
         for (int h = 1; h < g.n; ++h) HIPCHK(m, hipStreamWaitEvent(st[h], m->fork_ev, 0));
     }
     for (int h = 0; h < g.n; ++h) {
+        launch_history(h);
         if (g.graphs) HIPCHK(m, hipGraphLaunch(m->graphs[g.key[h]].exec, st[h]));
         else launch_group(h);
     }
@@ -606,7 +703,8 @@
     stage_mark(m, s, PB_STYLE);
     return ARTALK_OK;
 }
-int chunk_step(artalk_model* m, hipStream_t s, int cond_row0, int Bn, int n_next, int tap_chunk, float* out_motion_dev, int64_t out_stride) {
+int chunk_step(artalk_model* m, hipStream_t s, int cond_row0, int Bn, int n_next, int tap_chunk, float* out_motion_dev, int64_t out_stride,
+               bool init_history) {
     Workspace& w = m->ws;
     m->tap_chunk = tap_chunk;
     roctxRangePushA("artalk.ar.adaln_table");
@@ -617,10 +715,10 @@
     stage_mark(m, s, PB_ADA);
     if (body_uses_graphs(m)) {
         Range r_body("artalk.body.graph");
-        if (int rc = run_body(m, Bn, s, n_next)) return rc;
+        if (int rc = run_body(m, Bn, s, n_next, init_history)) return rc;
         stage_mark(m, s, PB_AR);
     } else {
-        if (int rc = run_body(m, Bn, s, n_next)) return rc;
+        if (int rc = run_body(m, Bn, s, n_next, init_history)) return rc;
     }
     const size_t mrow = (size_t)100 * m->cfg.motion_dim * 4;
     HIPCHK(m, hipMemcpy2DAsync(out_motion_dev, (size_t)out_stride * 4, w.motion_chunk, mrow, mrow, Bn, hipMemcpyDeviceToDevice, s));
diff --git a/artalk_amd/csrc/gemm_f16s.hip b/artalk_amd/csrc/gemm_f16s.hip
--- a/artalk_amd/csrc/gemm_f16s.hip
+++ b/artalk_amd/csrc/gemm_f16s.hip
@@ -41,6 +41,29 @@
     if (is_weight) status = nullptr;
     const long blocks = (n / 8 + 255) / 256;
     ARTALK_LAUNCH(pack_split_kernel, dim3((unsigned)(blocks < 8192 ? blocks : 8192)), dim3(256), 0, s, w, out, n, is_weight ? kWScale : p8_scale_of(p8_exp), status, p8_maxbits_of(p8_exp));
+}
+__global__ __launch_bounds__(256) void pack_split_rows_kernel(const float* __restrict__ w, unsigned int* __restrict__ out, int cols, long ld,
+                                                              float scale, int* __restrict__ status, unsigned int maxbits) {
+    const long row = (long)blockIdx.y * ld;
+    for (int i = (blockIdx.x * 256 + threadIdx.x) * 8; i < cols; i += gridDim.x * 2048) {
+        const f32x4 a = *reinterpret_cast<const f32x4*>(w + row + i), b = *reinterpret_cast<const f32x4*>(w + row + i + 4);
+        if (status) {
+            p8_guard(status, a[0], a[1], a[2], a[3], maxbits);
+            p8_guard(status, b[0], b[1], b[2], b[3], maxbits);
+        }
+        u32x2 h0, l0, h1, l1;
+        split_f32x4(a, scale, h0, l0);
+        split_f32x4(b, scale, h1, l1);
+        u32x4 hi = {h0[0], h0[1], h1[0], h1[1]}, lo = {l0[0], l0[1], l1[0], l1[1]};
+        *reinterpret_cast<u32x4*>(out + row + i) = hi;
+        *reinterpret_cast<u32x4*>(out + row + i + 4) = lo;
+    }
+}
+void launch_pack_split_rows(const float* w, unsigned int* out, int rows, int cols, long ld, hipStream_t s, int* status, int p8_exp) {
+    if (rows <= 0 || cols <= 0) return;
+    const int blocks = (cols / 8 + 255) / 256;
+    ARTALK_LAUNCH(pack_split_rows_kernel, dim3((unsigned)(blocks < 8 ? blocks : 8), (unsigned)rows), dim3(256), 0, s, w, out, cols, ld,
+                  p8_scale_of(p8_exp), status, p8_maxbits_of(p8_exp));
 }
 
 template <int BM, int BN, int WM, int WN, int APK, int TAG, int AMODE = 0>
diff --git a/artalk_amd/csrc/kernels.h b/artalk_amd/csrc/kernels.h
--- a/artalk_amd/csrc/kernels.h
+++ b/artalk_amd/csrc/kernels.h
@@ -73,6 +73,7 @@
 int gemm_config(const GemmArgs& g);
 int gemm_tile_count(const GemmArgs& g);
 void launch_pack_split(const float* w, unsigned int* out, long n, bool is_weight, hipStream_t s, int* status = nullptr, int p8_exp = kActExp);
+void launch_pack_split_rows(const float* w, unsigned int* out, int rows, int cols, long ld, hipStream_t s, int* status = nullptr, int p8_exp = kActExp);
 bool gemm_p8_eligible(const GemmArgs& g);
 void gemm_p8_prepare();
 void launch_gemm_bf16(const GemmArgs& g, hipStream_t s);
@@ -166,6 +167,8 @@
                        float* out, long out_bstride, int chunk, float* E, int B, hipStream_t s, int* status = nullptr);
 void launch_enc_input_zero(const float* mean, const float* stdv, const float* epos, float* E, int B, hipStream_t s);
 void launch_broadcast16(const void* src, void* dst, long bytes, int B, hipStream_t s);
+void launch_broadcast_rows16(const float* src, float* dst, int L, int rows, int cols, long dst_layer, long dst_clip, long dst_row, int B,
+                             hipStream_t s);
 struct SessionRows {
     uint4* style; uint4* prev_in; uint4* prev_fdec;
     int s16, p16, f16;
diff --git a/artalk_amd/csrc/model.h b/artalk_amd/csrc/model.h
--- a/artalk_amd/csrc/model.h
+++ b/artalk_amd/csrc/model.h
@@ -118,17 +118,33 @@
     std::vector<Site> sites;
     std::map<const int*, int> site_of;
     bool stream_scales_ended = false;
-    struct InitHistory { uint8_t* bits = nullptr; float *fdec = nullptr, *msfeat = nullptr; bool valid = false; } init_hist[3];
-    void invalidate_init_hist() { for (auto& ih : init_hist) ih.valid = false; }
+    struct InitHistory { uint8_t* bits = nullptr; float *fdec = nullptr, *msfeat = nullptr, *tok = nullptr, *tok_p8 = nullptr; bool valid = false; } init_hist[3];
+    struct InitKVKey {
+        int precision = 0, grouped = 0, splitk = 1; GemmPlan plan;
+        bool operator==(const InitKVKey& o) const {
+            return precision == o.precision && grouped == o.grouped && splitk == o.splitk && plan.path == o.plan.path && plan.cfg == o.plan.cfg &&
+                   plan.c2_fused == o.plan.c2_fused && plan.dominant == o.plan.dominant && plan.fused_ln == o.plan.fused_ln;
+        }
+    };
+    static constexpr int kInitKV = 4;
+    struct InitKV { float* kv = nullptr; bool valid = false; InitKVKey key; long long last_use = 0; } init_kv[kInitKV];
+    long long init_kv_clock = 0;
+    bool init_kv_on = true;
+    long long init_epoch = 0;
+    void invalidate_init_hist() { for (auto& ih : init_hist) ih.valid = false; for (auto& e : init_kv) e.valid = false; ++init_epoch; }
     float* tap = nullptr; int tap_B = 0, tap_maxch = 0, tap_chunk = 0;
     std::vector<uint32_t> cu_mask;
     int n_cus = 0;
     int stream_B = 0;
+    struct InitMark { int precision = -1; long long epoch = -1; };
+    InitMark mark_init() const { return InitMark{precision, init_epoch}; }
+    bool on_init_history(const InitMark& k) const { return k.precision == precision && k.epoch == init_epoch; }
+    InitMark stream_init;
     static constexpr int kSessBlock = 32;
     struct Sessions {
         std::vector<float*> blocks;
         std::vector<int64_t> owner;
-        struct Open { int slot = 0; int64_t seen = 0; bool smooth_done = false; };
+        struct Open { int slot = 0; int64_t seen = 0; bool smooth_done = false; InitMark init; };
         std::map<int64_t, Open> open;
         std::set<int64_t> ended_by_scales;
         int64_t next_id = 1;
@@ -223,7 +239,8 @@
 int run_init_history(artalk_model* m, int B, hipStream_t s);
 int begin_clips(artalk_model* m, hipStream_t s, int B, const float* style_motion_dev, const uint8_t* has_style, bool encode_style,
                 artalk_model::Stage* stg);
-int chunk_step(artalk_model* m, hipStream_t s, int cond_row0, int Bn, int n_next, int tap_chunk, float* out_motion_dev, int64_t out_stride);
+int chunk_step(artalk_model* m, hipStream_t s, int cond_row0, int Bn, int n_next, int tap_chunk, float* out_motion_dev, int64_t out_stride,
+               bool init_history = false);
 const unsigned int* packed_of(const artalk_model* m, const float* w);
 const void* bf16_of(const artalk_model* m, const float* w);
 int ensure_stage(artalk_model* m, int maxB, int maxC);
diff --git a/artalk_amd/csrc/model.hip b/artalk_amd/csrc/model.hip
--- a/artalk_amd/csrc/model.hip
+++ b/artalk_amd/csrc/model.hip
@@ -635,6 +635,14 @@
     return ARTALK_OK;
 }
 int artalk_set_tail_skip(artalk_model* m, int on) { if (!m) return ARTALK_EINVAL; m->tail_skip = on != 0; return ARTALK_OK; }
+int artalk_set_init_kv_cache(artalk_model* m, int on) {
+    if (!m) return ARTALK_EINVAL;
+    if (m->init_kv_on == (on != 0)) return ARTALK_OK;
+    (void)hipSetDevice(m->device); (void)hipDeviceSynchronize();
+    m->init_kv_on = on != 0;
+    drop_graphs(m);
+    return ARTALK_OK;
+}
 int artalk_set_graphs(artalk_model* m, int enable) {
     if (!m) return ARTALK_EINVAL;
     m->use_graphs = (enable & 0xff) != 0;
diff --git a/artalk_amd/model.py b/artalk_amd/model.py
--- a/artalk_amd/model.py
+++ b/artalk_amd/model.py
@@ -346,6 +346,10 @@
     def set_tail_skip(self, on: bool):
         if capi.lib().artalk_set_tail_skip(self._h, int(bool(on))) != capi.OK:
             raise RuntimeError("artalk_set_tail_skip failed")
+
+    def set_init_kv_cache(self, on: bool):
+        if capi.lib().artalk_set_init_kv_cache(self._h, int(bool(on))) != capi.OK:
+            raise RuntimeError("artalk_set_init_kv_cache failed")
 
     def graph_count(self):
         n = C.c_longlong(0)
diff --git a/include/artalk_hip.h b/include/artalk_hip.h
--- a/include/artalk_hip.h
+++ b/include/artalk_hip.h
@@ -52,6 +52,7 @@
                          const int64_t* n_samples, int B, const float* style_motion_dev, const uint8_t* has_style, float* out_motion_dev,
                          int64_t out_clip_stride, uint8_t* out_bits_dev, uint8_t* out_hist_bits_dev, float* out_w2v_dev, void* stream);
 int artalk_set_tail_skip(artalk_model* m, int on);
+int artalk_set_init_kv_cache(artalk_model* m, int on);
 int artalk_conv_tail_geometry(int64_t valid, int samples_per_chunk, int n_conv, const int* kernel, const int* stride, int* t_const,
                               int* Tp, int* Sp, int* samples_read);
 int64_t artalk_conv_tail_class(int64_t valid, int samples_per_chunk);
```

Measured after the change: 104,600, median of 6. About the same (+0.6%).
